# MGI-tech-bioinformatics/SuperPlus

Hardware: AMD Instinct MI355X
Metric: k-mers/s (DF createDict stage: trim + canonical k-mer count + solid filter + spectrum + adjacency) (higher is better)
Workload: dtype u64

## Files before the change

include/dfk.h:

```cpp
#ifndef DFK_H
#define DFK_H
#include <stddef.h>
#include <stdint.h>
#ifdef __cplusplus
extern "C" {
#endif

#define DFK_ABI_VERSION 3
#define DFK_MAX_MIN_BC 8u

enum {
    DFK_OK            = 0,
    DFK_E_ARG         = -1,
    DFK_E_NODEVICE    = -2,
    DFK_E_HIP         = -3,
    DFK_E_NOMEM       = -4,
    DFK_E_INPUT       = -5,
    DFK_E_STATE       = -6,
    DFK_E_NOGOOD      = -7
};

typedef struct dfk_config {
    uint32_t abi_version;
    uint32_t K;
    uint32_t min_qual;
    uint32_t min_freq;
    uint32_t min_bc;
    int32_t  device;
    int64_t  ign_bc_below;
    uint64_t hbm_budget_bytes;
    uint32_t minimizer_len;
    uint32_t flags;
    uint64_t inst_per_item;
    uint64_t reserved[4];
} dfk_config;

#define DFK_F_KEEP_PRE_ADJ   1u
#define DFK_F_KEEP_INPUTS    2u
#define DFK_F_MARK_BADS 4u

typedef struct dfk_entry32 {
    uint64_t w0, w1;
    uint32_t edge_id;
    uint32_t count_ctx;
    int32_t  bc;
    uint32_t pad;
} dfk_entry32;

typedef struct dfk_stats {
    uint64_t n_reads;
    uint64_t n_inst;
    uint64_t n_records;
    uint64_t n_buckets;
    uint64_t n_items;
    uint64_t n_overflow_items;
    uint64_t n_distinct;
    uint64_t n_solid;
    uint64_t adj_probes;
    float ms_upload, ms_trim, ms_part_count, ms_part_scatter, ms_count, ms_fallback, ms_adjacency, ms_total;
    uint64_t hbm_bytes_peak;
    uint64_t reserved[8];
} dfk_stats;

typedef struct dfk_ctx dfk_ctx;

int         dfk_create(const dfk_config* cfg, dfk_ctx** out);
void        dfk_destroy(dfk_ctx* ctx);
const char* dfk_last_error(void);
int         dfk_abi_version(void);

int dfk_qual_hist(dfk_ctx* ctx, uint32_t max_len, int64_t* hist);

int dfk_hint_file_range(dfk_ctx* ctx, const void* base, uint64_t bytes, int fd, uint64_t file_off);

int dfk_count(dfk_ctx* ctx,
              const uint8_t* packed_bases, const uint64_t* base_off, const uint32_t* read_len,
              const uint8_t* pq_bytes, const uint64_t* pq_off, const int32_t* bc,
              uint64_t n_reads);
int dfk_count_bci(dfk_ctx* ctx,
              const uint8_t* packed_bases, const uint64_t* base_off, const uint32_t* read_len,
              const uint8_t* pq_bytes, const uint64_t* pq_off, const int64_t* bci, uint64_t n_bci,
              uint64_t n_reads);

int dfk_count_device(dfk_ctx* ctx,
              const void* d_packed_bases, uint64_t packed_bytes, const void* d_base_off,
              const void* d_read_len, const void* d_pq_bytes, uint64_t pq_nbytes,
              const void* d_pq_off, const void* d_bc, uint64_t n_reads);

int dfk_good_lens(dfk_ctx* ctx, uint32_t* out, uint64_t cap);

int dfk_spectrum(dfk_ctx* ctx, const int64_t** hist, uint64_t* nbins);
int dfk_spectrum_json(dfk_ctx* ctx, char* out, uint64_t cap, uint64_t* need);

int dfk_solid_count(dfk_ctx* ctx, uint64_t* n);
int dfk_solid_fetch(dfk_ctx* ctx, dfk_entry32* out, uint64_t cap, int pre_adjacency);
int dfk_solid_fetch_unsorted(dfk_ctx* ctx, dfk_entry32* out, uint64_t cap, int pre_adjacency);

int dfk_solid_digest(dfk_ctx* ctx, int pre_adjacency, uint64_t* digest );

#define DFK_KVEC_PRE_ADJ 1
#define DFK_KVEC_SORTED  2
int dfk_write_kvec(dfk_ctx* ctx, const char* path, int flags);
int dfk_write_kvec_part(dfk_ctx* ctx, const char* path, int flags, uint64_t first_entry, uint64_t total_entries);

int dfk_get_stats(dfk_ctx* ctx, dfk_stats* out);

int dfk_graph_build(dfk_ctx* ctx);
int dfk_graph_stats(dfk_ctx* ctx, uint64_t* n_canonical_edges, uint64_t* n_vertices, uint64_t* n_edges);
int dfk_graph_write(dfk_ctx* ctx, const char* dir);

int dfk_paths_sink(dfk_ctx* ctx, const char* path);

int dfk_paths_build(dfk_ctx* ctx, const uint8_t* packed_bases, const uint64_t* base_off, const uint32_t* read_len,
              const uint8_t* pq_bytes, const uint64_t* pq_off, uint64_t n_reads);
int dfk_paths_build_device(dfk_ctx* ctx, const void* d_packed_bases, uint64_t packed_bytes, const void* d_base_off,
              const void* d_read_len, const void* d_pq_bytes, uint64_t pq_nbytes, const void* d_pq_off, uint64_t n_reads);
int dfk_paths_stats(dfk_ctx* ctx, uint64_t* n_reads, uint64_t* n_placed, uint64_t* n_path_edges);
int dfk_paths_write(dfk_ctx* ctx, const char* path);
int dfk_paths_fetch(dfk_ctx* ctx, int32_t* offsets, uint64_t* first_edge, int32_t* edges, uint64_t edges_cap);

int dfk_paths_index_write(dfk_ctx* ctx, const char* dir);
int dfk_dups_write(dfk_ctx* ctx, const char* path, uint64_t* n_marked_pairs);
int dfk_paths_index_dups_write(dfk_ctx* ctx, const char* dir, const char* dup_path, uint64_t* n_marked_pairs);

int dfk_bads_sums(dfk_ctx* ctx, uint16_t* out, uint64_t cap);
int dfk_bads_write(dfk_ctx* ctx, const char* path, uint64_t* n_marked_pairs, uint64_t* digest );
int dfk_bads_write_part(dfk_ctx* ctx, const char* path, uint64_t first_pair, uint64_t total_pairs, uint64_t* n_marked, uint64_t* digest );

#define DFK_HOPS_WORDS 16
#define DFK_HOPS_M1 0
#define DFK_HOPS_M2 1
#define DFK_HOPS_M3 2
#define DFK_HOPS_PAIRS 3
#define DFK_HOPS_SEARCHED 4
#define DFK_HOPS_EXTENDED 5
#define DFK_HOPS_HOST_EDGES 6
#define DFK_HOPS_MOST_ROUNDS 7
#define DFK_HOPS_US 8
#define DFK_HOPS_US_INDEX 9
#define DFK_HOPS_US_M12 10
#define DFK_HOPS_US_M3 11
#define DFK_HOPS_US_HOST 12
#define DFK_HOPS_LARGEST_X 13
#define DFK_HOPS_RANGES 14
int dfk_hops_build(dfk_ctx* ctx, const int32_t* bc , int one_good);
int dfk_hops_build_bci(dfk_ctx* ctx, const int64_t* bci, uint64_t n_bci, int one_good);
int dfk_hops_build_arrays(dfk_ctx* ctx, uint64_t n_edges, uint64_t n_vertices, const int32_t* kmers, const int32_t* inv, const int32_t* to_left, const int32_t* to_right,
                          uint64_t n_reads, const uint64_t* first , const int32_t* edges, const int32_t* bc, const uint16_t* sums, int one_good,
                          uint64_t reads_per_batch);
int dfk_hops_stats(dfk_ctx* ctx, uint64_t* out );
int dfk_hops_fetch(dfk_ctx* ctx, int32_t* pairs , uint64_t cap, uint64_t* n_pairs);
int dfk_hops_write(dfk_ctx* ctx, const char* path , uint64_t* n_pairs, uint64_t* digest );

#define DFK_SUBSET_WORDS 16
#define DFK_SUBSET_N_EOI 0
#define DFK_SUBSET_N_IDS 1
#define DFK_SUBSET_PATH_ENTRIES 2
#define DFK_SUBSET_INDEX_ENTRIES 3
#define DFK_SUBSET_RANGES 4
#define DFK_SUBSET_ONE_READ_ONLY 5
#define DFK_SUBSET_US 6
#define DFK_SUBSET_US_SWEEP 7
#define DFK_SUBSET_US_GATHER 8
#define DFK_SUBSET_US_INDEX 9
#define DFK_SUBSET_IDS_SUM 10
#define DFK_SUBSET_IDS_XOR 11
#define DFK_SUBSET_EOI_SUM 12
#define DFK_SUBSET_EOI_XOR 13
int dfk_subset_build(dfk_ctx* ctx, const int32_t* pairs , uint64_t n_pairs);
int dfk_subset_build_arrays(dfk_ctx* ctx, uint64_t n_edges, const int32_t* inv, uint64_t n_reads, const uint64_t* first , const int32_t* edges,
                            const int32_t* pairs, uint64_t n_pairs, uint64_t reads_per_batch, const char* dir );
int dfk_subset_stats(dfk_ctx* ctx, uint64_t* out );
int dfk_subset_fetch(dfk_ctx* ctx, uint64_t* ids, uint64_t ids_cap, uint64_t* n_ids, uint64_t* eoi, uint64_t eoi_cap, uint64_t* n_eoi);
int dfk_subset_write(dfk_ctx* ctx, const char* dir);

#define DFK_CHECK_WORDS 20
enum { DFK_CK_PATHS_SUM = 0, DFK_CK_PATHS_XOR = 1, DFK_CK_N_READS = 2, DFK_CK_N_PLACED = 3, DFK_CK_N_PATH_EDGES = 4,
       DFK_CK_INV_SUM = 5, DFK_CK_INV_XOR = 6, DFK_CK_INV_STARTS = 7, DFK_CK_INV_ENTRIES = 8,
       DFK_CK_COUNTSB_DIGEST = 9, DFK_CK_COUNTSB_SUM = 10, DFK_CK_SELF_INVERSE = 11,
       DFK_CK_DUP_DIGEST = 12, DFK_CK_DUP_MARKED = 13,
       DFK_CK_EDGE_KMERS = 14, DFK_CK_N_SOLID = 15, DFK_CK_INV_VIOLATIONS = 16, DFK_CK_N_EDGES = 17, DFK_CK_VALID = 18 };
#define DFK_CK_HAS_PATHS 1u
#define DFK_CK_HAS_INDEX 2u
#define DFK_CK_HAS_DUPS  4u
int dfk_paths_digest(dfk_ctx* ctx, uint64_t* out );
int dfk_paths_verify(dfk_ctx* ctx, const uint8_t* packed_bases, const uint64_t* base_off, const uint32_t* read_len, uint64_t n_reads,
              uint64_t* out );
int dfk_paths_verify_device(dfk_ctx* ctx, const void* d_packed_bases, uint64_t packed_bytes, const void* d_base_off, const void* d_read_len,
              uint64_t n_reads, uint64_t* out );

#define DFK_PBF_DROP 0xFFFFFFFFu
typedef struct dfk_pbf_input {
    const uint8_t*  seq[2];
    const uint8_t*  qual[2];
    const uint64_t* off[2];
    const uint32_t* rank;
    uint64_t m;
} dfk_pbf_input;
typedef struct dfk_pbf_output {
    uint64_t n_pairs;
    const uint32_t* order;
    const uint32_t* read_len;
    const uint8_t*  fastb_var;  const uint64_t* fastb_off;
    const uint8_t*  qualp_var;  const uint64_t* qualp_off;
    float ms_sort, ms_encode, ms_total;
} dfk_pbf_output;
typedef struct dfk_pbf dfk_pbf;
int  dfk_pbf_run(dfk_ctx* ctx, const dfk_pbf_input* in, dfk_pbf** out);
int  dfk_pbf_result(const dfk_pbf* r, dfk_pbf_output* o);
void dfk_pbf_free(dfk_pbf* r);

int dfk_shard_begin(dfk_ctx* ctx,
              const void* d_packed_bases, uint64_t packed_bytes, const void* d_base_off,
              const void* d_read_len, const void* d_pq_bytes, uint64_t pq_nbytes,
              const void* d_pq_off, const void* d_bc, uint64_t n_reads,
              int64_t global_read_offset ,
              uint64_t* n_inst_local);
int dfk_shard_begin_host(dfk_ctx* ctx,
              const uint8_t* packed_bases, const uint64_t* base_off , const uint32_t* read_len,
              const uint8_t* pq_bytes, const uint64_t* pq_off , const int32_t* bc, uint64_t n_reads,
              int64_t global_read_offset, uint64_t* n_inst_local);
int dfk_shard_plan(dfk_ctx* ctx, uint32_t world, uint64_t n_inst_global, uint32_t* log2_passes);
int dfk_shard_partition(dfk_ctx* ctx, uint32_t world, uint64_t n_inst_global, uint32_t log2_passes, uint32_t pass,
              const void** d_records, uint64_t* send_counts );
int dfk_shard_partition_begin(dfk_ctx* ctx, uint32_t world, uint64_t n_inst_global, uint32_t log2_passes, uint32_t pass, int defer,
              const void** d_records, uint64_t* send_counts );
int dfk_shard_partition_end(dfk_ctx* ctx, uint32_t pass);
int dfk_shard_recv_buffer(dfk_ctx* ctx, uint64_t n_records, void** d_buf);
int dfk_shard_count(dfk_ctx* ctx, const void* d_records, uint64_t n_records, uint32_t pass);
int dfk_shard_adj_queries(dfk_ctx* ctx, const void** d_keys,
              uint64_t* send_counts );
int dfk_shard_adj_answer(dfk_ctx* ctx, const void* d_keys, uint64_t n_keys, void* d_present );
int dfk_shard_adj_apply(dfk_ctx* ctx, const void* d_present, uint64_t n_keys);
int dfk_shard_dict_share(dfk_ctx* ctx, const void** d_entries, uint64_t* n_entries);
int dfk_shard_dict_adopt(dfk_ctx* ctx, uint64_t n_entries, void** d_room);
int dfk_shard_dict_whole(dfk_ctx* ctx);

int dfk_paths_var_bytes(dfk_ctx* ctx, uint64_t* bytes);
int dfk_paths_write_part(dfk_ctx* ctx, const char* path, uint64_t first_read, uint64_t total_reads, uint64_t var_before, uint64_t var_total);
int dfk_shard_pidx_pairs(dfk_ctx* ctx, uint32_t world, const void** d_pairs, uint64_t* send_counts , uint64_t* counts_host );
int dfk_shard_pidx_write(dfk_ctx* ctx, uint32_t world, uint32_t rank, const void* d_pairs_in, uint64_t n_in, const uint64_t* counts_global , const char* dir);
int dfk_shard_dup_keys(dfk_ctx* ctx, uint32_t world, const void** d_items, uint64_t* send_counts );
int dfk_shard_dup_answer(dfk_ctx* ctx, const void* d_items_in, uint64_t n_in, void* d_answers );
int dfk_shard_dup_write(dfk_ctx* ctx, const void* d_answers_back, uint64_t n, const char* path, uint64_t first_pair, uint64_t total_pairs, uint64_t* n_marked);

#ifdef __cplusplus
}
#endif
#endif
```

superplus_amd/csrc/dfk.hip:

```cpp
#include "../../include/dfk.h"
#include "dfk_kernels.h"
#include "dfk_arena.h"

#include <algorithm>
#include <chrono>
#include <cstdarg>
#include <cstdio>
#include <cstdlib>
#include <cstring>
#include <atomic>
#include <fcntl.h>
#include <functional>
#include <new>
#include <string>
#include <sys/mman.h>
#include <sys/stat.h>
#include <unistd.h>
#include <condition_variable>
#include <memory>
#include <mutex>
#include <numeric>
#include <thread>
#include <vector>

using namespace dfk;

namespace {

thread_local std::string g_err;

int fail(int code, const char* fmt, ...)
{
    char buf[512];
    va_list ap; va_start(ap, fmt); vsnprintf(buf, sizeof buf, fmt, ap); va_end(ap);
    g_err = buf;
    return code;
}

#define HIP_TRY(expr) do { hipError_t e_ = (expr); if (e_ != hipSuccess) \
    return fail(DFK_E_HIP, "%s failed: %s (%s:%d)", #expr, hipGetErrorString(e_), __FILE__, __LINE__); } while (0)

template <class F> int guarded(F&& f)
{
    try { return f(); }
    catch (const std::bad_alloc&) { return fail(DFK_E_NOMEM, "out of host memory"); }
    catch (const std::exception& e) { return fail(DFK_E_HIP, "internal error: %s", e.what()); }
    catch (...) { return fail(DFK_E_HIP, "internal error"); }
}

void* dev_get(uint64_t bytes, const char** why)
{
    void* p = nullptr;
    const hipError_t e = hipMalloc(&p, bytes);
    if (e == hipSuccess) return p;
    (void)hipGetLastError();
    *why = hipGetErrorString(e);
    return nullptr;
}
void dev_give(void* p) { (void)hipFree(p); }

bool g_trace = getenv("DFK_TRACE") != nullptr;
#define TRACE(...) do { if (g_trace) { fprintf(stderr, "[dfk] " __VA_ARGS__); fputc('\n', stderr); fflush(stderr); } } while (0)
inline uint32_t env_u32(const char* name, uint32_t dflt) { const char* e = getenv(name); return e ? (uint32_t)atoi(e) : dflt; }
inline double wall_now() { return std::chrono::duration<double>(std::chrono::steady_clock::now().time_since_epoch()).count(); }

template <int K> struct CountCfg;
#ifndef DFK_LOG2S
#define DFK_LOG2S 11
#endif
#ifndef DFK_NWAVES
#define DFK_NWAVES 8
#endif
template <> struct CountCfg<40> { static constexpr int LOG2S = DFK_LOG2S, NWAVES = DFK_NWAVES; };
template <> struct CountCfg<48> { static constexpr int LOG2S = DFK_LOG2S, NWAVES = DFK_NWAVES; };
template <> struct CountCfg<60> { static constexpr int LOG2S = DFK_LOG2S, NWAVES = DFK_NWAVES; };

struct Inputs {
    const uint8_t* packed; uint64_t packed_bytes;
    const uint64_t* base_off; const uint32_t* read_len;
    const uint8_t* pq; uint64_t pq_bytes; const uint64_t* pq_off;
    const int32_t* bc; uint64_t n_reads;
};

}

struct dfk_ctx {
    dfk_config cfg{};
    int device = 0;
    hipStream_t stream = nullptr;
    hipStream_t stream2 = nullptr;
    hipDeviceProp_t prop{};
    dfk::Arena arena{dev_get, dev_give};
    uint64_t &budget = arena.budget, &held = arena.held, &peak = arena.peak, &alloc_seq = arena.alloc_seq, &first_chunk_hint = arena.first_chunk_hint;
    int alloc(DevBuf& b, size_t bytes, const char* what, Place where = Place::High) { return arena.alloc(b, bytes, what, where) ? fail(DFK_E_NOMEM, "%s", arena.err.c_str()) : 0; }
    void release(DevBuf& b) { arena.release(b); }
    void shrink(DevBuf& b, size_t keep) { arena.shrink(b, keep); }
    void release_since(uint64_t mark, const DevBuf* keep = nullptr) { arena.release_since(mark, keep); }
    uint64_t largest_allocatable() const { return arena.largest_allocatable(); }
    void drop_empty_chunks() { arena.drop_empty_chunks(); }
    void drop_pool() { arena.drop_pool(); }
    bool have = false;
    uint64_t n_reads = 0;
    struct FileRange { const char* base; uint64_t bytes; int fd; uint64_t off; };
    std::vector<FileRange> file_ranges;
    DevBuf good_len;
    struct Part { DevBuf buf, pre; uint64_t n = 0; uint64_t blist = 0, n_blist = 0; bool listed = false; };
    bool want_blist = false;
    int pending_blist = -1;
    std::function<int()> after_count_launch;
    std::vector<Part> parts;
    uint64_t n_solid = 0, n_boundary = 0;
    unsigned seg_attempt = 0;
    double distinct_per_inst = 0.0;
    double plan_derate = 0.95;
    std::vector<int64_t> hist;
    std::vector<dfk_entry32> sorted, sorted_pre;
    bool sorted_ok = false, sorted_pre_ok = false;
    dfk_stats st{};
    bool shard_open = false, shard_use_bc = false;
    const void* sh_in[7] = {};
    uint64_t sh_packed_bytes = 0, sh_pq_bytes = 0, sh_n_reads = 0, sh_n_inst_local = 0;
    int64_t sh_read_id0 = 0;
    DevBuf shard_send[2];
    uint32_t shard_send_pass[2] = {~0u, ~0u};
    DevBuf shard_recv[2];
    unsigned shard_recv_seq = 0;
    uint64_t budget_taken = 0;
    void* sh_staged[6] = {};
    uint64_t sh_b0 = 0, sh_b1 = 0, sh_q0 = 0, sh_q1 = 0, sh_staged_reads = 0;
    DevBuf adj_keys, adj_src; uint64_t adj_n = 0;
    DevBuf set; uint64_t set_mask = 0;
    double t_upload_done = 0;
    uint32_t shard_world = 1, shard_log2_nb = 0;
    void* shard_state = nullptr;
    void (*shard_state_free)(void*) = nullptr;
    void* lane_pool = nullptr; void (*lane_pool_free)(void*) = nullptr;
    std::mutex lane_mu;
    void* graph_state = nullptr;
    void (*graph_state_free)(void*) = nullptr;
    unsigned int* d_resident = nullptr;
    unsigned int resident_target = 0;
    unsigned int last_wg_idle = 0;
    void* kept[6] = {};
    uint64_t kept_packed_bytes = 0, kept_pq_bytes = 0, kept_n_reads = 0, kept_budget = 0;

    void release_all()
    {
        after_count_launch = nullptr;
        if (stream2) (void)hipStreamSynchronize(stream2);
        DevBuf* live[] = {&good_len, &shard_send[0], &shard_send[1], &shard_recv[0], &shard_recv[1], &adj_keys, &adj_src, &set};
        for (DevBuf* d : live) release(*d);
        for (Part& pt : parts) { release(pt.buf); release(pt.pre); }
        parts.clear();
        arena.reset();
        good_len = shard_send[0] = shard_send[1] = shard_recv[0] = shard_recv[1] = adj_keys = adj_src = set = DevBuf{};
        shard_send_pass[0] = shard_send_pass[1] = ~0u;
        have = false; sorted_ok = sorted_pre_ok = false; sorted.clear(); sorted_pre.clear(); hist.clear();
        n_solid = 0; adj_n = 0; shard_open = false;
        if (shard_state) { shard_state_free(shard_state); shard_state = nullptr; }
        for (void*& p : sh_staged) if (p) { (void)hipFree(p); p = nullptr; }
        budget += budget_taken; budget_taken = 0;
        if (graph_state) { graph_state_free(graph_state); graph_state = nullptr; }
    }
    void drop_kept()
    {
        for (void*& p : kept) if (p) { (void)hipFree(p); p = nullptr; }
        budget += kept_budget; kept_budget = 0; kept_n_reads = 0;
    }
    void adopt_kept()
    {
        const uint64_t bytes[6] = {kept_packed_bytes + 64, (kept_n_reads + 1) * 8 + 64, kept_n_reads * 4 + 64, kept_pq_bytes + 64, (kept_n_reads + 1) * 8 + 64, 0};
        for (int i = 0; i < 6; ++i) {
            if (!kept[i]) continue;
            const uint64_t b = bytes[i] & ~(uint64_t)0xFFF;
            if (i < 5 && b >= (64ull << 20) && ((uintptr_t)kept[i] & 0xFFF) == 0) arena.adopt(kept[i], b);
            else (void)hipFree(kept[i]);
            kept[i] = nullptr;
        }
        budget += kept_budget; kept_budget = 0; kept_n_reads = 0;
    }
};

namespace {

struct Timer {
    hipEvent_t a{}, b{}; hipStream_t s;
    explicit Timer(hipStream_t st) : s(st) { (void)hipEventCreate(&a); (void)hipEventCreate(&b); }
    ~Timer() { (void)hipEventDestroy(a); (void)hipEventDestroy(b); }
    void start() { (void)hipEventRecord(a, s); }
    float stop() { (void)hipEventRecord(b, s); (void)hipEventSynchronize(b); float ms = 0; (void)hipEventElapsedTime(&ms, a, b); return ms; }
};

template <int K>
int stage_trim(dfk_ctx* c, const Inputs& in, uint64_t* n_inst)
{
    DevBuf ctr; int rc = c->alloc(ctr, 32, "trim counters"); if (rc) return rc;
    HIP_TRY(hipMemsetAsync(ctr.p, 0, 32, c->stream));
    rc = c->alloc(c->good_len, sizeof(uint32_t) * in.n_reads, "goodLens", Place::Low); if (rc) return rc;
    if (in.n_reads) {
        unsigned grid = (unsigned)std::min<uint64_t>((in.n_reads + 255) / 256, 8192);
        hipLaunchKernelGGL(HIP_KERNEL_NAME(k_trim<K>), dim3(grid), dim3(256), 0, c->stream,
                           in.pq, in.pq_off, in.pq_bytes, in.base_off, in.packed_bytes, in.read_len, in.n_reads, c->cfg.min_qual, (uint32_t*)c->good_len.p,
                           (unsigned long long*)ctr.p, (unsigned int*)((char*)ctr.p + 8),
                           (unsigned long long*)((char*)ctr.p + 16));
        HIP_TRY(hipGetLastError());
    }
    uint64_t h[3] = {0, 0, 0};
    HIP_TRY(hipMemcpyAsync(h, ctr.p, 24, hipMemcpyDeviceToHost, c->stream));
    HIP_TRY(hipStreamSynchronize(c->stream));
    c->release(ctr);
    if ((uint32_t)h[1]) return fail(DFK_E_INPUT, "malformed input: an offset table is not monotone or runs past its array, a PQVec stream is broken, or its length differs from read_len");
    if (h[2] == 0) return fail(DFK_E_NOGOOD, "Looks like your input data have almost no good bases.");
    *n_inst = h[0];
    return 0;
}

int device_scan(dfk_ctx* c, const uint64_t* in, uint64_t* out, uint64_t n)
{
    constexpr uint64_t PER = (uint64_t)SCAN_THREADS * SCAN_ITEMS;
    if (n == 0) return 0;
    const uint64_t nblk = (n + PER - 1) / PER;
    if (nblk == 1) {
        hipLaunchKernelGGL(k_scan_blocks, dim3(1), dim3(SCAN_THREADS), 0, c->stream, in, out, n, (uint64_t*)nullptr);
        HIP_TRY(hipGetLastError());
        return 0;
    }
    DevBuf sums; int rc = c->alloc(sums, nblk * 8, "scan block sums"); if (rc) return rc;
    hipLaunchKernelGGL(k_scan_blocks, dim3((unsigned)nblk), dim3(SCAN_THREADS), 0, c->stream, in, out, n, (uint64_t*)sums.p);
    HIP_TRY(hipGetLastError());
    rc = device_scan(c, (const uint64_t*)sums.p, (uint64_t*)sums.p, nblk); if (rc) return rc;
    hipLaunchKernelGGL(k_scan_add, dim3((unsigned)nblk), dim3(SCAN_THREADS), 0, c->stream, out, n, (const uint64_t*)sums.p);
    HIP_TRY(hipGetLastError());
    HIP_TRY(hipStreamSynchronize(c->stream));
    c->release(sums);
    return 0;
}

struct BucketTable {
    uint32_t log2_nb = 0;
    DevBuf acc;
    DevBuf summ;
    DevBuf classes;
    DevBuf ovf_list; uint64_t n_ovf = 0;
    DevBuf class_hist;
    std::vector<uint64_t> h_class;
    uint64_t n_records = 0, n_inst = 0;
};
struct Partition {
    DevBuf records, base, ipre, items;
    uint64_t n_records = 0, n_inst = 0, n_items = 0;
    uint64_t nb = 0;
};

template <int K>
PartParams part_params(const dfk_ctx* c, uint32_t log2_nb, uint32_t log2_world, int64_t read_id0, uint32_t sub_lo, uint32_t sub_n)
{
    const uint32_t M = c->cfg.minimizer_len;
    return PartParams{M, (uint32_t)K - M + 1, log2_nb, log2_world, read_id0, sub_lo, sub_n,
                      sweep_class_mask(sub_lo, sub_n, log2_nb - log2_world)};
}

int table_totals(dfk_ctx* c, const DevBuf& acc, uint64_t nb, uint64_t* n_records, uint64_t* n_inst)
{
    DevBuf tot; int rc = c->alloc(tot, 16, "bucket totals"); if (rc) return rc;
    HIP_TRY(hipMemsetAsync(tot.p, 0, 16, c->stream));
    hipLaunchKernelGGL(k_sum_acc, dim3(1024), dim3(256), 0, c->stream, (const unsigned long long*)acc.p, nb, (unsigned long long*)tot.p);
    HIP_TRY(hipGetLastError());
    uint64_t h[2];
    HIP_TRY(hipMemcpyAsync(h, tot.p, 16, hipMemcpyDeviceToHost, c->stream));
    HIP_TRY(hipStreamSynchronize(c->stream));
    c->release(tot);
    *n_records = h[0]; *n_inst = h[1];
    return 0;
}

struct ScanJob {
    PartParams pp; ScanPlan plan;
    DevBuf ovf_tmp, d_n;
    DevBuf keys, keys2, fill, sub;
    uint64_t n_pieces = 0; bool count_due = false;
    hipEvent_t ev_scan = nullptr, ev_count = nullptr, ev_part[2] = {nullptr, nullptr};
    std::vector<std::pair<hipEvent_t, hipEvent_t>> ev;
    ~ScanJob()
    {
        for (auto& e : ev) { (void)hipEventDestroy(e.first); (void)hipEventDestroy(e.second); }
        for (hipEvent_t e : {ev_scan, ev_count, ev_part[0], ev_part[1]}) if (e) (void)hipEventDestroy(e);
    }
};

template <int K> bool scan_takes_ranges(const dfk_ctx* c) { return c->cfg.minimizer_len == 16; }

ScanSwitches scan_switches()
{
    static const uint32_t scan_blocks = getenv("DFK_SCAN_BLOCKS") ? (uint32_t)atoi(getenv("DFK_SCAN_BLOCKS")) : 0;
    ScanSwitches sw;
    sw.scan_blocks = scan_blocks;
    if (const char* e = getenv("DFK_SCAN_KEY_PIECE")) { sw.key_piece_set = true; sw.key_piece = strtoull(e, nullptr, 10); }
    if (const char* e = getenv("DFK_SCAN_KEY_TAIL")) sw.key_tail = strtoull(e, nullptr, 10);
    sw.no_overlap = getenv("DFK_NO_OVERLAP") != nullptr;
    return sw;
}

template <int K>
int scan_begin(dfk_ctx* c, const Inputs& in, uint32_t log2_world, int64_t read_id0, BucketTable* T, bool by_class, ScanJob* J)
{
    J->pp = part_params<K>(c, T->log2_nb, log2_world, read_id0, 0, 1u << (T->log2_nb - log2_world));
    J->plan = plan_scan(ScanInputs{K, J->pp.W, T->log2_nb, log2_world, in.n_reads, in.packed_bytes, by_class, scan_takes_ranges<K>(c), c->stream2 != nullptr, scan_switches()});
    ScanPlan& P = J->plan;
    int rc = 0;
    if (by_class) { rc = c->alloc(T->class_hist, P.n_bins * 8, "class counters", Place::Low); if (rc) return rc; HIP_TRY(hipMemsetAsync(T->class_hist.p, 0, P.n_bins * 8, c->stream)); }
    else { rc = c->alloc(T->acc, P.nb * 8, "bucket counters", Place::Low); if (rc) return rc; }
// ... 232 lines not shown
                           (unsigned long long*)J->cur.p, J->P.n_records, (uint4*)J->P.records.p);
    HIP_TRY(hipGetLastError());
    HIP_TRY(hipEventRecord(J->e1, J->st));
    return 0;
}

template <int K>
int scatter_begin(dfk_ctx* c, const Inputs& in, const BucketTable& T, uint32_t log2_world, int64_t read_id0,
                  uint32_t sub_lo, uint32_t sub_n, ScatterJob* J, bool launch_now = true)
{
    Partition* P = &J->P;
    J->st = c->stream; J->lo = sub_lo; J->n = sub_n;
    const PartParams pp = part_params<K>(c, T.log2_nb, log2_world, read_id0, sub_lo, sub_n);
    const uint64_t budget = item_budget<K>(c);
    int rc = pass_tables(c, T.acc, T.log2_nb - log2_world, 1u << log2_world, sub_lo, sub_n, budget, P); if (rc) return rc;
    const uint64_t nb = P->nb;
    rc = c->alloc(J->cur, nb * 8, "bucket cursors"); if (rc) return rc;
    rc = c->alloc(P->records, P->n_records * 32, "super-k-mer records"); if (rc) return rc;
    rc = c->alloc(J->d_bad, 16, "scatter check"); if (rc) return rc;
    HIP_TRY(hipMemcpyAsync(J->cur.p, P->base.p, nb * 8, hipMemcpyDeviceToDevice, c->stream));
    HIP_TRY(hipMemsetAsync(J->d_bad.p, 0, 16, c->stream));
    if (!J->e0) { HIP_TRY(hipEventCreate(&J->e0)); HIP_TRY(hipEventCreate(&J->e1)); }
    (void)pp;
    if (launch_now) return scatter_launch<K>(c, in, T, log2_world, read_id0, J);
    return 0;
}

template <int K>
int scatter_end(dfk_ctx* c, const Inputs& in, const BucketTable& T, uint32_t log2_world, int64_t read_id0, ScatterJob* J)
{
    HIP_TRY(hipEventSynchronize(J->e1));
    float ms = 0; (void)hipEventElapsedTime(&ms, J->e0, J->e1);
    c->st.ms_part_scatter += ms;
    {
        Partition* P = &J->P;
        const PartParams pp = part_params<K>(c, T.log2_nb, log2_world, read_id0, J->lo, J->n);
        const size_t lds_b = sizeof(uint32_t) * pp.W * PART_THREADS + sizeof(uint32_t) * 2 * PART_QCAP * PART_THREADS;
        Timer t(c->stream);
        t.start();
        if (T.n_ovf)
            hipLaunchKernelGGL(HIP_KERNEL_NAME(k_partition<K, true>), dim3((unsigned)((T.n_ovf + PART_THREADS - 1) / PART_THREADS)),
                               dim3(PART_THREADS), lds_b, c->stream,
                               in.packed, in.packed_bytes, in.base_off, (const uint32_t*)c->good_len.p, in.bc,
                               (int64_t)c->cfg.ign_bc_below, in.n_reads, pp, (unsigned long long*)nullptr, (unsigned long long*)nullptr,
                               (unsigned long long*)J->cur.p, P->n_records, (uint4*)P->records.p, (uint4*)nullptr,
                               (const uint32_t*)T.ovf_list.p, T.n_ovf, (const uint64_t*)nullptr, (uint32_t*)nullptr);
        HIP_TRY(hipGetLastError());
        hipLaunchKernelGGL(k_check_cursors, dim3((unsigned)std::min<uint64_t>((P->nb + 255) / 256, 4096)), dim3(256), 0, c->stream, (const unsigned long long*)J->cur.p,
                           (const uint64_t*)P->base.p, P->nb, (unsigned int*)J->d_bad.p);
        HIP_TRY(hipGetLastError());
        c->st.ms_part_scatter += t.stop();
    }
    unsigned int bad = 0;
    HIP_TRY(hipMemcpy(&bad, J->d_bad.p, 4, hipMemcpyDeviceToHost));
    c->release(J->d_bad); c->release(J->cur);
    if (bad) return fail(DFK_E_HIP, "scatter: %u buckets did not receive the records counted for them (run summaries and bucket counters disagree)", bad);
    TRACE("scatter of buckets [%u, %u) done (%llu records, %llu items)", J->lo, J->lo + J->n,
          (unsigned long long)J->P.n_records, (unsigned long long)J->P.n_items);
    return 0;
}

constexpr int E_SPLIT_NO_ROOM = -101;
constexpr int E_SEGMENT_FULL = -100;

struct CountRun {
    CountGlobals* g = nullptr; uint4* seg = nullptr; unsigned long long* hist = nullptr;
    CountParams cp{}; unsigned grid = 0;
    DevBuf big; uint64_t big_cap = 0;
    DevBuf d_hist, d_g;
    DevBuf d_snap;
    DevBuf d_part;
    DevBuf d_wg;
    uint64_t solid_seen = 0, inst_seen = 0;
    uint64_t boundary_seen = 0;
    uint64_t splits_seen = 0;
};

int count_run_begin(dfk_ctx* c, CountRun* R)
{
    int rc = c->alloc(R->d_hist, (uint64_t)HIST_GLOBAL_BINS * 8, "spectrum bins", Place::Low); if (rc) return rc;
    rc = c->alloc(R->d_g, sizeof(CountGlobals), "count globals", Place::Low); if (rc) return rc;
    HIP_TRY(hipMemsetAsync(R->d_hist.p, 0, (uint64_t)HIST_GLOBAL_BINS * 8, c->stream));
    HIP_TRY(hipMemsetAsync(R->d_g.p, 0, sizeof(CountGlobals), c->stream));
    R->g = (CountGlobals*)R->d_g.p; R->hist = (unsigned long long*)R->d_hist.p;
    return c->alloc(R->d_snap, (uint64_t)HIST_GLOBAL_BINS * 8 + 256, "spectrum snapshot", Place::Low);
}

int count_snapshot(dfk_ctx* c, CountRun* R, bool restore)
{
    char* snap = (char*)R->d_snap.p;
    const uint64_t hb = (uint64_t)HIST_GLOBAL_BINS * 8;
    if (!restore) {
        HIP_TRY(hipMemcpyAsync(snap, R->d_hist.p, hb, hipMemcpyDeviceToDevice, c->stream));
        HIP_TRY(hipMemcpyAsync(snap + hb, R->d_g.p, sizeof(CountGlobals), hipMemcpyDeviceToDevice, c->stream));
    } else {
        HIP_TRY(hipMemcpyAsync(R->d_hist.p, snap, hb, hipMemcpyDeviceToDevice, c->stream));
        HIP_TRY(hipMemcpyAsync(R->d_g.p, snap + hb, sizeof(CountGlobals), hipMemcpyDeviceToDevice, c->stream));
    }
    return 0;
}

int count_run_end(dfk_ctx* c, CountRun* R)
{
    CountGlobals hg{};
    HIP_TRY(hipMemcpy(&hg, R->d_g.p, sizeof hg, hipMemcpyDeviceToHost));
    c->st.n_distinct = hg.n_distinct; c->n_boundary = hg.n_boundary;
#ifdef DFK_PHASE_TIMES
    {
        unsigned long long ph[16] = {};
        (void)hipMemcpyFromSymbol(ph, HIP_SYMBOL(g_phase), sizeof ph);
        unsigned long long tot = 0; for (int i = 0; i < 12; ++i) tot += ph[i];
        static const char* nm[12] = {"item loop tail (thread 0 publishes)", "barrier: item start", "chunks (stage + insert)", "barrier: chunks done", "finish pass 1 (solidity)", "barrier", "finish pass 2 (adjacency look-ups)", "barrier", "finish pass 3 (emit)", "barrier", "clear + reduce", "drain"};
        fprintf(stderr, "[dfk] k_count wave cycles by phase (%.3e memtime ticks in all):\n", (double)tot);
        for (int i = 0; i < 12; ++i) fprintf(stderr, "[dfk]   %5.1f %%  %s\n", 100.0 * (double)ph[i] / (double)std::max(1ull, tot), nm[i]);
        unsigned long long z[16] = {};
        (void)hipMemcpyToSymbol(HIP_SYMBOL(g_phase), z, sizeof z);
    }
#endif
    DevBuf d_max; int rc = c->alloc(d_max, 16, "max bin"); if (rc) return rc;
    HIP_TRY(hipMemsetAsync(d_max.p, 0, 16, c->stream));
    hipLaunchKernelGGL(k_hist_max, dim3(1024), dim3(256), 0, c->stream, (const unsigned long long*)R->d_hist.p, HIST_GLOBAL_BINS,
                       (unsigned int*)d_max.p);
    uint32_t nb = 0;
    HIP_TRY(hipMemcpyAsync(&nb, d_max.p, 4, hipMemcpyDeviceToHost, c->stream));
    HIP_TRY(hipStreamSynchronize(c->stream));
    c->hist.assign(nb, 0);
    if (nb) HIP_TRY(hipMemcpy(c->hist.data(), R->d_hist.p, 8ull * nb, hipMemcpyDeviceToHost));
    TRACE("spectrum read back: %u bins, %llu solid", nb, (unsigned long long)c->n_solid);
    c->release(d_max); c->release(R->d_hist); c->release(R->d_g); c->release(R->d_snap);
    return 0;
}

template <int K> unsigned count_grid(const dfk_ctx* c, int nbc = 1)
{
    constexpr int LOG2S = CountCfg<K>::LOG2S, NW = CountCfg<K>::NWAVES;
    const size_t lds = count_lds_bytes<K, LOG2S, NW, 1>() + (size_t)(nbc > 1 ? nbc - 1 : 0) * sizeof(uint32_t) * (1u << LOG2S);
    const unsigned per_cu = (unsigned)std::max<size_t>(1, (size_t)(160 * 1024) / lds);
    return (unsigned)c->prop.multiProcessorCount * per_cu;
}

int launch_boundary_list(dfk_ctx* c)
{
    if (c->pending_blist < 0) return 0;
    const dfk_ctx::Part& part = c->parts[(size_t)c->pending_blist];
    c->pending_blist = -1;
    unsigned long long* ctl = (unsigned long long*)((char*)part.buf.p + part.blist);
    HIP_TRY(hipMemsetAsync(ctl, 0, 16, c->stream2));
    hipLaunchKernelGGL(k_boundary_list, dim3((unsigned)std::min<uint64_t>((part.n + 2047) / 2048, 4096)), dim3(256), 0, c->stream2,
                       (const uint4*)part.buf.p, part.n, (uint32_t*)(ctl + 2), part.n_blist, ctl);
    HIP_TRY(hipGetLastError());
    return 0;
}

template <int K, int NBC>
int launch_count(dfk_ctx* c, const Partition& P, const ItemRange* d_items, uint64_t n_items, const CountRun& R,
                 std::vector<ItemRange>* overflowed, float* kernel_ms, const uint32_t* d_sub = nullptr, bool single_kmer_records = false)
{
    constexpr int LOG2S = CountCfg<K>::LOG2S, NW = CountCfg<K>::NWAVES;
    if (n_items == 0) return 0;
    if (n_items >= (1ull << 32)) return fail(DFK_E_ARG, "too many work items in one pass");
    DevBuf d_ovf;
    int rc = c->alloc(d_ovf, n_items * sizeof(ItemRange), "overflow list"); if (rc) return rc;
    HIP_TRY(hipMemsetAsync(&R.g->next_item, 0, 8, c->stream));
    HIP_TRY(hipMemsetAsync(&R.g->n_wg_idle, 0, 4, c->stream));
    CountParams cp = R.cp; cp.n_items = (uint32_t)n_items; cp.single = single_kmer_records ? 1u : 0u;
    const size_t lds = count_lds_bytes<K, LOG2S, NW, NBC>();
    auto kern = d_sub ? k_count<K, LOG2S, NW, NBC, true> : k_count<K, LOG2S, NW, NBC, false>;
    HIP_TRY(hipFuncSetAttribute(reinterpret_cast<const void*>(kern), hipFuncAttributeMaxDynamicSharedMemorySize, (int)lds));
    TRACE("k_count: %llu items, grid %u, lds %zu, seg_cap %llu", (unsigned long long)n_items, R.grid, lds, (unsigned long long)R.cp.seg_cap);
    Timer tk(c->stream);
    tk.start();
    hipLaunchKernelGGL(kern, dim3(R.grid), dim3(NW * 64), lds, c->stream,
                       (const uint4*)P.records.p, d_items, (const uint64_t*)P.base.p, cp, R.g, R.seg, (WgOut*)R.d_wg.p, R.hist,
                       (ItemRange*)d_ovf.p, d_sub, c->d_resident);
    HIP_TRY(hipGetLastError());
    c->resident_target += R.grid;
    if (c->after_count_launch || c->pending_blist >= 0) {
        hipLaunchKernelGGL(k_gate, dim3(1), dim3(64), 0, c->stream2, (const unsigned int*)c->d_resident, c->resident_target, 200000ull, c->d_resident + 1);
    }
    if (c->after_count_launch) { std::function<int()> f; f.swap(c->after_count_launch); rc = f(); if (rc) return rc; }
    rc = launch_boundary_list(c); if (rc) return rc;
    *kernel_ms += tk.stop();
    CountGlobals g{};
    HIP_TRY(hipMemcpyAsync(&g, R.g, sizeof g, hipMemcpyDeviceToHost, c->stream));
    HIP_TRY(hipStreamSynchronize(c->stream));
    c->last_wg_idle = g.n_wg_idle;
    if (g.n_overflow) {
        const size_t at = overflowed->size();
        overflowed->resize(at + g.n_overflow);
        HIP_TRY(hipMemcpy(overflowed->data() + at, d_ovf.p, sizeof(ItemRange) * g.n_overflow, hipMemcpyDeviceToHost));
    }
    c->release(d_ovf);
    return 0;
}

int gather_diffs(dfk_ctx* c, const std::vector<ItemRange>& ranges, std::initializer_list<std::pair<const DevBuf*, std::vector<uint64_t>*>> tables)
{
    const uint32_t n = (uint32_t)ranges.size();
    DevBuf d_idx, d_val;
    int rc = c->alloc(d_idx, 8ull * n, "gather index"); if (!rc) rc = c->alloc(d_val, 16ull * n, "gather values"); if (rc) return rc;
    HIP_TRY(hipMemcpyAsync(d_idx.p, ranges.data(), 8ull * n, hipMemcpyHostToDevice, c->stream));
    std::vector<uint64_t> val(2 * n);
    for (const auto& t : tables) {
        hipLaunchKernelGGL(k_gather_u64, dim3((2 * n + 255) / 256), dim3(256), 0, c->stream, (const uint64_t*)t.first->p, (const uint32_t*)d_idx.p, 2 * n, (uint64_t*)d_val.p);
        HIP_TRY(hipGetLastError());
        HIP_TRY(hipMemcpyAsync(val.data(), d_val.p, 16ull * n, hipMemcpyDeviceToHost, c->stream));
        HIP_TRY(hipStreamSynchronize(c->stream));
        for (uint32_t i = 0; i < n; ++i) t.second->push_back(val[2 * i + 1] - val[2 * i]);
    }
    c->release(d_idx); c->release(d_val);
    return 0;
}

template <int K, int NBC>
int launch_count_big(dfk_ctx* c, const Partition& P, const std::vector<ItemRange>& singles, CountRun& R)
{
    constexpr int KW = KTraits<K>::KW, NW = 8;
    const uint32_t n = (uint32_t)singles.size();
    std::vector<uint64_t> inst, rec;
    int rc = gather_diffs(c, singles, {{&P.ipre, &inst}, {&P.base, &rec}}); if (rc) return rc;
    const uint64_t tot_inst = std::accumulate(inst.begin(), inst.end(), (uint64_t)0);
    const std::vector<uint64_t> chunk_pre = chunk_prefixes(rec);
    double per_inst = table_distinct_per_inst(c->distinct_per_inst);
    DevBuf d_items, d_fail, d_pre;
    {
        const uint64_t more = tot_inst / std::max<uint32_t>(1, c->cfg.min_freq) + 1;
        if (!R.big.p) { R.big_cap = more; rc = c->alloc(R.big, R.big_cap * 32, "fallback solid entries"); if (rc) return rc; }
        else {
            CountGlobals g0{};
            HIP_TRY(hipMemcpy(&g0, R.d_g.p, sizeof g0, hipMemcpyDeviceToHost));
            DevBuf grown;
            rc = c->alloc(grown, (g0.big_cursor + more) * 32, "fallback solid entries"); if (rc) return rc;
            if (g0.big_cursor) HIP_TRY(hipMemcpy(grown.p, R.big.p, g0.big_cursor * 32, hipMemcpyDeviceToDevice));
            c->release(R.big);
            R.big = grown; R.big_cap = g0.big_cursor + more;
        }
    }
    rc = c->alloc(d_items, (uint64_t)n * sizeof(BigItem), "fallback items"); if (rc) return rc;
    rc = c->alloc(d_pre, 16ull * (n + 1), "fallback prefixes"); if (rc) return rc;
    rc = c->alloc(d_fail, 16, "fallback flag"); if (rc) return rc;
    uint64_t* d_chunk_pre = (uint64_t*)d_pre.p; uint64_t* d_slot_pre = d_chunk_pre + (n + 1);
    HIP_TRY(hipMemcpyAsync(d_chunk_pre, chunk_pre.data(), 8ull * (n + 1), hipMemcpyHostToDevice, c->stream));
    CountParams cpb = R.cp; cpb.seg_cap = R.big_cap;
    const unsigned cus = (unsigned)c->prop.multiProcessorCount;
    for (;;) {
        const BigTables T = size_big_tables(singles, inst, per_inst, big_slot_words(KW, NBC));
        DevBuf pool;
        rc = c->alloc(pool, T.words * 4 + 8, "HBM fallback tables"); if (rc) return rc;
        hipLaunchKernelGGL(k_fill_u64, dim3(4096), dim3(256), 0, c->stream, (uint64_t*)pool.p, T.words / 2 + (T.words & 1), 0ull);
        HIP_TRY(hipGetLastError());
        HIP_TRY(hipMemsetAsync(d_fail.p, 0, 16, c->stream));
        HIP_TRY(hipMemcpyAsync(d_items.p, T.items.data(), T.items.size() * sizeof(BigItem), hipMemcpyHostToDevice, c->stream));
        HIP_TRY(hipMemcpyAsync(d_slot_pre, T.slot_pre.data(), 8ull * (n + 1), hipMemcpyHostToDevice, c->stream));
        const unsigned g_ins = (unsigned)std::max<uint64_t>(1, std::min<uint64_t>((chunk_pre[n] + NW * BIG_TICKET_CHUNKS - 1) / (NW * BIG_TICKET_CHUNKS), 4ull * cus));
        const unsigned g_slot = (unsigned)std::max<uint64_t>(1, std::min<uint64_t>((T.slot_pre[n] + 255) / 256, 16ull * cus));
        hipLaunchKernelGGL(HIP_KERNEL_NAME(k_big_insert<K, NW, NBC>), dim3(g_ins), dim3(NW * 64), 0, c->stream,
                           (const uint4*)P.records.p, (const BigItem*)d_items.p, (const uint64_t*)P.base.p, (const uint64_t*)d_chunk_pre, n,
                           (uint32_t*)pool.p, (unsigned long long*)d_fail.p + 1, (uint32_t*)d_fail.p);
        HIP_TRY(hipGetLastError());
        uint32_t failed = 0;
        HIP_TRY(hipMemcpyAsync(&failed, d_fail.p, 4, hipMemcpyDeviceToHost, c->stream));
        HIP_TRY(hipStreamSynchronize(c->stream));
        if (failed) {
            unsigned int info[4] = {};
            (void)hipMemcpyFromSymbol(info, HIP_SYMBOL(g_big_fail), sizeof info);
            const unsigned int zero[4] = {};
            (void)hipMemcpyToSymbol(HIP_SYMBOL(g_big_fail), zero, sizeof zero);
            c->release(pool);
            if (T.certain) {
                c->release(d_items); c->release(d_fail); c->release(d_pre);
                return fail(DFK_E_HIP, "an insert into an HBM fallback table gave up after %u probe steps and %u waits on a locked slot "
                                       "(table of 2^%u slots at load <= 0.5; %u tables, %llu instances in this pass's fallback)", info[1], info[2], info[3], n,
                            (unsigned long long)tot_inst);
            }
            per_inst = table_retry_per_inst(per_inst);
            TRACE("fallback: an HBM table filled up (2^%u slots): rebuilding the tables for %.2f distinct k-mers per instance", info[3], per_inst);
            continue;
        }
        hipLaunchKernelGGL(HIP_KERNEL_NAME(k_big_flags<K, NBC>), dim3(g_slot), dim3(256), 0, c->stream, (const BigItem*)d_items.p,
                           (const uint64_t*)d_slot_pre, n, (uint32_t*)pool.p, cpb, R.g);
        if (cpb.do_adj)
            hipLaunchKernelGGL(HIP_KERNEL_NAME(k_big_resolve<K>), dim3(g_slot), dim3(256), 0, c->stream, (const BigItem*)d_items.p,
                               (const uint64_t*)d_slot_pre, n, (uint32_t*)pool.p);
        hipLaunchKernelGGL(HIP_KERNEL_NAME(k_big_emit<K>), dim3(g_slot), dim3(256), 0, c->stream, (const BigItem*)d_items.p,
                           (const uint64_t*)d_slot_pre, n, (uint32_t*)pool.p, cpb, R.g, (uint4*)R.big.p, R.hist);
        HIP_TRY(hipGetLastError());
        HIP_TRY(hipStreamSynchronize(c->stream));
        c->release(pool);
        break;
    }
    c->release(d_items); c->release(d_fail); c->release(d_pre);
    return 0;
}

template <int K, int NBC>
int count_halved(dfk_ctx* c, const Partition& P, const CountRun& R, bool single_kmer_records, std::vector<ItemRange>& overflowed, std::vector<ItemRange>* singles)
{
    while (!overflowed.empty()) {
        const std::vector<ItemRange> next = halve_items(overflowed, singles);
        overflowed.clear();
        if (next.empty()) break;
        if (!single_kmer_records) TRACE("retrying %zu split items", next.size());
        DevBuf d_next; float ignored = 0;
        int rc = c->alloc(d_next, next.size() * sizeof(ItemRange), "split items"); if (rc) return rc;
        HIP_TRY(hipMemcpyAsync(d_next.p, next.data(), next.size() * sizeof(ItemRange), hipMemcpyHostToDevice, c->stream));
        rc = launch_count<K, NBC>(c, P, (const ItemRange*)d_next.p, next.size(), R, &overflowed, &ignored, nullptr, single_kmer_records);
        c->release(d_next); if (rc) return rc;
    }
    return 0;
}

template <int K, int NBC>
int count_split(dfk_ctx* c, const Partition& P, const std::vector<ItemRange>& hot, const std::vector<uint64_t>& inst, const SplitCandidates& sp, size_t i0, size_t i1, CountRun& R)
{
    constexpr int NW = 8;
    const uint32_t n = (uint32_t)(i1 - i0);
    std::vector<HotItem> items(n); std::vector<ItemRange> buckets(n);
    uint64_t ns = 0, tot = 0;
    for (uint32_t i = 0; i < n; ++i) { buckets[i] = hot[sp.at[i0 + i]]; items[i] = HotItem{buckets[i].b0, buckets[i].b1, (uint32_t)ns, sp.log2p[i0 + i]}; ns += 1ull << sp.log2p[i0 + i]; tot += inst[sp.at[i0 + i]]; }
    if (ns >= (1ull << 24)) { fail(DFK_E_NOMEM, "more than 2^24 sub-buckets in one pass"); return E_SPLIT_NO_ROOM; }
    const uint64_t mark = c->alloc_seq;
    bool started = false;
    auto undo = [&](int rc) {
        (void)hipStreamSynchronize(c->stream);
        if (!started) { c->release_since(mark); return rc == DFK_E_NOMEM ? E_SPLIT_NO_ROOM : rc; }
        return rc;
    };
    DevBuf d_items, d_pre, d_tk, acc; std::vector<uint64_t> rec;
    int rc = gather_diffs(c, buckets, {{&P.base, &rec}}); if (rc) return undo(rc);
    const std::vector<uint64_t> chunk_pre = chunk_prefixes(rec);
    rc = c->alloc(d_items, (uint64_t)n * sizeof(HotItem), "hot buckets"); if (rc) return undo(rc);
    rc = c->alloc(d_pre, 8ull * (n + 1), "hot bucket chunks"); if (rc) return undo(rc);
    rc = c->alloc(d_tk, 16, "hot bucket ticket"); if (rc) return undo(rc);
    rc = c->alloc(acc, 8ull * ns, "sub-bucket counters"); if (rc) return undo(rc);
// ... 44 lines not shown
}

int barcode_words(const dfk_ctx* c, bool have_bc)
{ return !have_bc ? 0 : (int)std::max<uint32_t>(1, std::min<uint32_t>(c->cfg.min_bc, DFK_MAX_MIN_BC) - (c->cfg.min_bc > 1 ? 1 : 0)); }

template <int K> constexpr uint64_t out_chunk() { return 2ull << CountCfg<K>::LOG2S; }

template <int K>
int count_prepare(dfk_ctx* c, const Partition& P, CountRun& R, int nbc)
{
    const unsigned attempt = c->seg_attempt;
    R.grid = (unsigned)std::max<uint64_t>(1, std::min<uint64_t>(P.n_items, count_grid<K>(c, nbc)));
    uint64_t res = part_entries(P.n_inst, c->cfg.min_freq, R.inst_seen, R.solid_seen);
    res = (res << attempt) + (uint64_t)R.grid * out_chunk<K>();
    const uint64_t room = c->budget > c->held ? (c->budget - c->held) : 0;
    if (res * 32 > room) res = room / 32;
    int rc = c->alloc(R.d_wg, sizeof(WgOut) * R.grid, "workgroup output state"); if (rc) return rc;
    std::vector<WgOut> init(R.grid, WgOut{~0ull, (unsigned int)out_chunk<K>(), 0u});
    HIP_TRY(hipMemcpy(R.d_wg.p, init.data(), sizeof(WgOut) * R.grid, hipMemcpyHostToDevice));
    HIP_TRY(hipMemsetAsync(&R.g->big_cursor, 0, 8, c->stream));
    HIP_TRY(hipMemsetAsync(&R.g->part_cursor, 0, 8, c->stream));
    R.cp = CountParams{c->cfg.min_freq, c->cfg.min_bc, 0, 0, res, c->cfg.min_freq > 1 ? 1u : 0u,
                       (c->cfg.flags & DFK_F_KEEP_PRE_ADJ) ? 1u : 0u};
    R.big_cap = 0;
    rc = c->alloc(R.d_part, std::max<uint64_t>(1, res) * 32, "solid k-mer entries", Place::Low); if (rc) return rc;
    R.seg = (uint4*)R.d_part.p;
    return 0;
}

template <int K>
int finish_part(dfk_ctx* c, const Partition& P, CountRun& R)
{
    CountGlobals hg{};
    std::vector<WgOut> wg(R.grid);
    HIP_TRY(hipMemcpy(&hg, R.d_g.p, sizeof hg, hipMemcpyDeviceToHost));
    HIP_TRY(hipMemcpy(wg.data(), R.d_wg.p, sizeof(WgOut) * R.grid, hipMemcpyDeviceToHost));
    c->release(R.d_wg);
    const uint64_t claimed = hg.part_cursor;
    const HoleMoves mv = plan_hole_moves(wg, out_chunk<K>(), claimed);
    const std::vector<uint64_t>&src = mv.src, &dst = mv.dst; const uint64_t n_lds = mv.n_lds;
    if (hg.solid_overflow || claimed > R.cp.seg_cap || hg.big_cursor > R.big_cap || n_lds + hg.big_cursor > R.cp.seg_cap) {
        c->release(R.big); c->release(R.d_part);
        fail(DFK_E_NOMEM, "the room reserved for a pass's solid k-mers (%llu entries) is full", (unsigned long long)R.cp.seg_cap);
        return E_SEGMENT_FULL;
    }
    if (src.size() != dst.size())
        return fail(DFK_E_HIP, "output compaction: %zu holes, %zu entries to move", dst.size(), src.size());
    dfk_ctx::Part part;
    part.n = n_lds + hg.big_cursor;
    part.buf = R.d_part; R.d_part = DevBuf{};
    if (!src.empty()) {
        DevBuf d_mv; int rc = c->alloc(d_mv, 16ull * src.size(), "hole moves"); if (rc) return rc;
        HIP_TRY(hipMemcpyAsync(d_mv.p, src.data(), 8ull * src.size(), hipMemcpyHostToDevice, c->stream));
        HIP_TRY(hipMemcpyAsync((uint64_t*)d_mv.p + src.size(), dst.data(), 8ull * src.size(), hipMemcpyHostToDevice, c->stream));
        hipLaunchKernelGGL(k_fill_holes, dim3((unsigned)((src.size() + 255) / 256)), dim3(256), 0, c->stream, (uint4*)part.buf.p,
                           (const uint64_t*)d_mv.p, (const uint64_t*)d_mv.p + src.size(), (uint64_t)src.size());
        HIP_TRY(hipGetLastError());
        HIP_TRY(hipStreamSynchronize(c->stream));
        c->release(d_mv);
    }
    if (hg.big_cursor)
        HIP_TRY(hipMemcpyAsync((char*)part.buf.p + 32 * n_lds, R.big.p, 32 * hg.big_cursor, hipMemcpyDeviceToDevice, c->stream));
    HIP_TRY(hipStreamSynchronize(c->stream));
    c->release(R.big);
    const uint64_t nb_part = hg.n_boundary - R.boundary_seen;
    R.boundary_seen = hg.n_boundary;
    c->st.n_overflow_items += hg.n_split - R.splits_seen;
    R.splits_seen = hg.n_split;
    uint64_t keep = part.n * 32;
    part.listed = c->want_blist && nb_part == 0;
    if (c->want_blist && nb_part && keep + 16 + 4 * nb_part <= part.buf.bytes && part.n < (1ull << 32)) {
        part.blist = keep; part.n_blist = nb_part; part.listed = true;
        keep += 16 + 4 * nb_part;
    }
    c->shrink(part.buf, keep);
    c->parts.push_back(part);
    if (part.blist) c->pending_blist = (int)c->parts.size() - 1;
    c->n_solid += part.n; c->st.n_solid = c->n_solid;
    R.solid_seen += part.n; R.inst_seen += P.n_inst;
    if (R.inst_seen) c->distinct_per_inst = (double)hg.n_distinct / (double)R.inst_seen;
    return 0;
}

template <int K, int NBC>
int count_run(dfk_ctx* c, const Partition& P, CountRun& R)
{
    Timer t(c->stream);
    std::vector<ItemRange> overflowed, singles;
    c->st.n_items += P.n_items;
    const float ms_before = c->st.ms_count;
    int rc = launch_count<K, NBC>(c, P, (const ItemRange*)P.items.p, P.n_items, R, &overflowed, &c->st.ms_count); if (rc) return rc;
    if (g_trace) {
        unsigned int gate[2] = {0, 0};
        (void)hipMemcpy(gate, c->d_resident, 8, hipMemcpyDeviceToHost);
        TRACE("k_count: %llu instances in %.1f ms (%.1f G instances/s), reservation %.2f GB, %u of %u workgroups idle, %u gate timeouts so far",
              (unsigned long long)P.n_inst, c->st.ms_count - ms_before, 1e-6 * (double)P.n_inst / (double)(c->st.ms_count - ms_before), R.d_part.bytes / 1e9,
              c->last_wg_idle, R.grid, gate[1]);
    }
    t.start();
    c->st.n_overflow_items += overflowed.size();
    rc = count_halved<K, NBC>(c, P, R, false, overflowed, &singles); if (rc) return rc;
    TRACE("fallback: %zu single-bucket items", singles.size());
    if (!singles.empty()) {
        const FallbackSwitches sw{env_u32("DFK_SPLIT_FROM_LOG2", 2), env_u32("DFK_MAX_SUBPASS_LOG2", 8)};
        const double dpi = route_distinct_per_inst(c->distinct_per_inst);
        std::vector<uint64_t> inst; std::vector<uint8_t> taken(singles.size(), 0);
        rc = gather_diffs(c, singles, {{&P.ipre, &inst}}); if (rc) return rc;
        const SplitCandidates sp = split_candidates(inst, dpi, sw);
        for (size_t i0 = 0; i0 < sp.at.size();) {
            const uint64_t can = c->largest_allocatable();
            const size_t i1 = split_group_end(inst, sp.at, i0, split_group_cap(can));
            if (i1 == i0) { TRACE("fallback: no room to split a hot bucket of %llu instances (%.2f GB free in one piece): sub-passes instead", (unsigned long long)inst[sp.at[i0]], can / 1e9); break; }
            rc = count_split<K, NBC>(c, P, singles, inst, sp, i0, i1, R);
            if (rc == E_SPLIT_NO_ROOM) { TRACE("fallback: no room to split %zu hot buckets (%s): sub-passes instead", i1 - i0, g_err.c_str()); break; }
            if (rc) return rc;
            for (; i0 < i1; ++i0) taken[sp.at[i0]] = 1;
        }
        SubpassPlan sub = plan_subpasses(singles, inst, taken, dpi, CountCfg<K>::LOG2S, sw);
        TRACE("fallback: %zu sub-passes over %zu buckets in LDS tables, %zu buckets in HBM tables", sub.items.size(), singles.size() - sub.huge.size(), sub.huge.size());
        while (!sub.items.empty()) {
            DevBuf d_it, d_sub;
            rc = c->alloc(d_it, sub.items.size() * sizeof(ItemRange), "sub-pass items"); if (!rc) rc = c->alloc(d_sub, sub.words.size() * 4, "sub-pass words"); if (rc) return rc;
            HIP_TRY(hipMemcpyAsync(d_it.p, sub.items.data(), sub.items.size() * sizeof(ItemRange), hipMemcpyHostToDevice, c->stream));
            HIP_TRY(hipMemcpyAsync(d_sub.p, sub.words.data(), sub.words.size() * 4, hipMemcpyHostToDevice, c->stream));
            std::vector<ItemRange> again; ItemRange bad{}; float ignored = 0;
            rc = launch_count<K, NBC>(c, P, (const ItemRange*)d_it.p, sub.items.size(), R, &again, &ignored, (const uint32_t*)d_sub.p);
            c->release(d_it); c->release(d_sub);
            if (rc) return rc;
            if (!refine_subpasses(again, &sub, &bad))
                return fail(DFK_E_HIP, "a sub-pass (%u of 2^%u) of bucket %u overflowed its table (it holds at most %llu instances)", bad.b1 & 0xFFu, (bad.b1 & 0x7FFFFFFFu) >> 8, bad.b0, 1ull << (CountCfg<K>::LOG2S - 1));
            if (!sub.items.empty()) TRACE("fallback: %zu sub-passes cut in two", again.size());
        }
        if (!sub.huge.empty()) { rc = launch_count_big<K, NBC>(c, P, sub.huge, R); if (rc) return rc; }
    }
    c->st.ms_fallback += t.stop();
    return finish_part<K>(c, P, R);
}


template <int K>
int count_run_nbc(dfk_ctx* c, const Partition& P, CountRun& R, int nbc)
{
    static int (*const run[8])(dfk_ctx*, const Partition&, CountRun&) = {count_run<K, 0>, count_run<K, 1>, count_run<K, 2>, count_run<K, 3>, count_run<K, 4>, count_run<K, 5>, count_run<K, 6>, count_run<K, 7>};
    return run[std::min(std::max(nbc, 0), 7)](c, P, R);
}

template <int K>
int stage_count(dfk_ctx* c, const Partition& P, CountRun& R, bool have_bc)
{
    const int rc = count_prepare<K>(c, P, R, barcode_words(c, have_bc));
    return rc ? rc : count_run_nbc<K>(c, P, R, barcode_words(c, have_bc));
}

int build_set(dfk_ctx* c)
{
    uint64_t slots = 1ull << std::max<uint32_t>(10, ceil_log2(2 * c->n_boundary + 2));
    int rc = c->alloc(c->set, slots * sizeof(SetSlot), "boundary k-mer set"); if (rc) return rc;
    c->set_mask = slots - 1;
    hipLaunchKernelGGL(k_fill_u64, dim3(2048), dim3(256), 0, c->stream, (uint64_t*)c->set.p, slots * 2, ~0ull);
    for (const dfk_ctx::Part& pt : c->parts)
        if (pt.n)
            hipLaunchKernelGGL(k_set_insert, dim3((unsigned)((pt.n + 255) / 256)), dim3(256), 0, c->stream,
                               (const uint4*)pt.buf.p, pt.n, (SetSlot*)c->set.p, c->set_mask);
    HIP_TRY(hipGetLastError());
    return 0;
}

int make_pre_view(dfk_ctx* c)
{
    if (!(c->cfg.flags & DFK_F_KEEP_PRE_ADJ)) return 0;
    for (dfk_ctx::Part& pt : c->parts) {
        int rc = c->alloc(pt.pre, pt.n * 32, "pre-adjacency copy"); if (rc) return rc;
        if (!pt.n) continue;
        if (c->cfg.min_freq > 1)
            hipLaunchKernelGGL(k_make_pre, dim3((unsigned)((pt.n + 255) / 256)), dim3(256), 0, c->stream,
                               (uint4*)pt.buf.p, (uint4*)pt.pre.p, pt.n);
        else
            HIP_TRY(hipMemcpyAsync(pt.pre.p, pt.buf.p, pt.n * 32, hipMemcpyDeviceToDevice, c->stream));
    }
    HIP_TRY(hipGetLastError());
    return 0;
}

template <int K>
int stage_adjacency(dfk_ctx* c)
{
    Timer t(c->stream);
    t.start();
    int rc = make_pre_view(c); if (rc) return rc;
    if (c->cfg.min_freq > 1 && c->n_solid && c->n_boundary) {
        bool listed = c->want_blist;
        for (const dfk_ctx::Part& pt : c->parts) listed = listed && pt.listed;
        if (c->want_blist) {
            rc = launch_boundary_list(c); if (rc) return rc;
            HIP_TRY(hipStreamSynchronize(c->stream2));
        }
        if (listed) {
            uint64_t total = 0;
            for (const dfk_ctx::Part& pt : c->parts) {
                if (!pt.blist) continue;
                unsigned long long ctl[2] = {0, 0};
                HIP_TRY(hipMemcpy(ctl, (const char*)pt.buf.p + pt.blist, 16, hipMemcpyDeviceToHost));
                if (ctl[1] || ctl[0] != pt.n_blist)
                    return fail(DFK_E_HIP, "boundary list: %llu entries listed, the count kernels reported %llu", ctl[0], (unsigned long long)pt.n_blist);
                total += pt.n_blist;
            }
            if (total != c->n_boundary) listed = false;
        }
        if (!listed) { rc = build_set(c); if (rc) return rc; }
        else {
            uint64_t slots = 1ull << std::max<uint32_t>(10, ceil_log2(2 * c->n_boundary + 2));
            rc = c->alloc(c->set, slots * sizeof(SetSlot), "boundary k-mer set"); if (rc) return rc;
            c->set_mask = slots - 1;
            hipLaunchKernelGGL(k_fill_u64, dim3(2048), dim3(256), 0, c->stream, (uint64_t*)c->set.p, slots * 2, ~0ull);
            for (const dfk_ctx::Part& pt : c->parts)
                if (pt.n_blist)
                    hipLaunchKernelGGL(k_set_insert_list, dim3((unsigned)((pt.n_blist + 255) / 256)), dim3(256), 0, c->stream, (const uint4*)pt.buf.p,
                                       (const uint32_t*)((const char*)pt.buf.p + pt.blist + 16), pt.n_blist, (SetSlot*)c->set.p, c->set_mask);
            HIP_TRY(hipGetLastError());
        }
        DevBuf d_n; rc = c->alloc(d_n, 16, "probe counter"); if (rc) return rc;
        HIP_TRY(hipMemsetAsync(d_n.p, 0, 16, c->stream));
        for (const dfk_ctx::Part& pt : c->parts) {
            if (!pt.n) continue;
            if (listed) {
                if (pt.n_blist)
                    hipLaunchKernelGGL(HIP_KERNEL_NAME(k_adjacency_list<K>), dim3((unsigned)std::min<uint64_t>((pt.n_blist + 255) / 256, 16384)), dim3(256), 0,
                                       c->stream, (uint4*)pt.buf.p, (const uint32_t*)((const char*)pt.buf.p + pt.blist + 16), pt.n_blist,
                                       (const SetSlot*)c->set.p, c->set_mask, (unsigned long long*)d_n.p);
            } else
                hipLaunchKernelGGL(HIP_KERNEL_NAME(k_adjacency<K>), dim3((unsigned)std::min<uint64_t>((pt.n + 255) / 256, 8192)), dim3(256), 0,
                                   c->stream, (uint4*)pt.buf.p, pt.n, (const SetSlot*)c->set.p, c->set_mask, (unsigned long long*)d_n.p);
        }
        HIP_TRY(hipGetLastError());
        uint64_t np = 0;
        HIP_TRY(hipMemcpyAsync(&np, d_n.p, 8, hipMemcpyDeviceToHost, c->stream));
        HIP_TRY(hipStreamSynchronize(c->stream));
        c->st.adj_probes = np;
        c->release(d_n); c->release(c->set);
    }
    c->st.ms_adjacency = t.stop();
    TRACE("adjacency done");
    return 0;
}

uint32_t pick_log2_nb(uint64_t n_inst, uint32_t log2_world)
{
    static const uint64_t per = getenv("DFK_INST_PER_BUCKET") ? (uint64_t)atoll(getenv("DFK_INST_PER_BUCKET")) : 850;
    return dfk::pick_log2_nb(n_inst, log2_world, per);
}

PlanInputs plan_inputs(const dfk_ctx* c, const BucketTable& T, const CountRun& R, uint32_t sub_nb, uint32_t lo, bool overlap)
{
    static const double first_div = getenv("DFK_PLAN_FIRST") ? atof(getenv("DFK_PLAN_FIRST")) : 10.0;
    static const double growth = getenv("DFK_PLAN_GROWTH") ? atof(getenv("DFK_PLAN_GROWTH")) : 1.1;
    return PlanInputs{c->budget > c->held ? (double)(c->budget - c->held) : 0.0, sub_nb, lo, T.n_inst, T.n_records, R.inst_seen, R.solid_seen,
                      c->cfg.min_freq, c->seg_attempt, c->plan_derate, overlap, first_div, growth, g_trace};
}

struct StreamSwap {
    dfk_ctx* c; hipStream_t keep;
    StreamSwap(dfk_ctx* ctx, hipStream_t s) : c(ctx), keep(ctx->stream) { c->stream = s; }
    ~StreamSwap() { c->stream = keep; }
};

struct Prescan { BucketTable T; uint64_t n_inst = 0; float ms_trim = 0; };

template <int K>
int run_typed(dfk_ctx* c, const Inputs& in, Prescan* pre = nullptr)
{
    Timer total(c->stream);
    total.start();
    Timer t(c->stream);
    uint64_t n_inst = 0;
    int rc = 0;
    BucketTable T;
    if (pre) { n_inst = pre->n_inst; c->st.ms_trim = pre->ms_trim; T = std::move(pre->T); }
    else {
        t.start();
        TRACE("trim: %llu reads", (unsigned long long)in.n_reads);
        rc = stage_trim<K>(c, in, &n_inst); if (rc) return rc;
        c->st.ms_trim = t.stop();
        TRACE("trim done: %llu instances", (unsigned long long)n_inst);
    }
    c->st.n_reads = in.n_reads; c->st.n_inst = n_inst; c->n_reads = in.n_reads;
    if (!pre) {
        T.log2_nb = pick_log2_nb(n_inst, 0);
        rc = partition_count<K>(c, in, n_inst, 0, 0, &T); if (rc) return rc;
    }
    CountRun R;
    rc = count_run_begin(c, &R); if (rc) return rc;
    c->want_blist = true; c->pending_blist = -1;
    const uint32_t sub_nb = 1u << T.log2_nb;
    const uint32_t forced = (uint32_t)c->cfg.reserved[0];
    const uint32_t per_forced = forced ? std::max<uint32_t>(1, (sub_nb + forced - 1) / forced) : 0;
    const bool overlap = getenv("DFK_NO_OVERLAP") == nullptr;
    uint32_t n_passes = 0, retries = 0;
    c->seg_attempt = 0; c->distinct_per_inst = 0.0;
    struct Job { ScatterJob sj; Arena::PassBlock blk; uint64_t mark = 0; bool valid = false; };
    Job cur, nxt;
    auto drop_events = [&](Job& j) { if (j.sj.e0) { (void)hipEventDestroy(j.sj.e0); (void)hipEventDestroy(j.sj.e1); j.sj.e0 = j.sj.e1 = nullptr; } };
    static const double defer_below = getenv("DFK_DEFER_SWEEP_BELOW") ? atof(getenv("DFK_DEFER_SWEEP_BELOW")) : 1.0;
    auto start = [&](Job& j, uint32_t lo, uint32_t n, bool may_defer = false) -> int {
        j.sj = ScatterJob{}; j.mark = c->alloc_seq; j.valid = false;
        const bool defer = may_defer && (double)n < defer_below * (double)sub_nb;
        TRACE("pass range [%u, %u) of %u (%.1f %%), %.2f GB held of %.2f", lo, lo + n, sub_nb, 100.0 * n / sub_nb, c->held / 1e9, c->budget / 1e9);
        j.blk = Arena::PassBlock{};
        int r = c->alloc(j.blk.block, pass_block_bytes(n, sub_nb, T.n_records), "pass block");
        if (!r) { Arena::Current in_blk(c->arena, j.blk); StreamSwap sw(c, c->stream2); r = scatter_begin<K>(c, in, T, 0, 0, lo, n, &j.sj, !defer); }
        if (r) { (void)hipStreamSynchronize(c->stream2); c->release_since(j.mark); drop_events(j); return r; }
        if (defer) { ScatterJob* sj = &j.sj; c->after_count_launch = [c, &in, &T, sj]() { return scatter_launch<K>(c, in, T, 0, 0, sj); }; TRACE("  (its sweep starts behind k_count)"); }
        j.valid = true;
        return 0;
    };
    auto start_alone = [&](Job& j, uint32_t lo) -> int {
        for (;;) {
            const uint32_t n = forced ? std::min(per_forced, sub_nb - lo) : plan_range(plan_inputs(c, T, R, sub_nb, lo, overlap), c->arena.free_blocks(), nullptr);
            if (!forced && n < sub_nb - lo && (uint64_t)n * 1024 < sub_nb)
                return fail(DFK_E_NOMEM, "HBM budget too small: %.2f GB free of %.2f GB allows passes of %u of %u buckets",
                            (c->budget - c->held) / 1e9, c->budget / 1e9, n, sub_nb);
            const int r = start(j, lo, n);
            if (r != DFK_E_NOMEM || forced || n <= 16 || ++retries > 12) return r;
            c->plan_derate *= 0.7;
            TRACE("out of HBM (%s): planning smaller passes", g_err.c_str());
        }
    };
    rc = start_alone(cur, 0); if (rc) return rc;
    while (cur.valid) {
        const uint32_t lo = cur.sj.lo, n = cur.sj.n, nlo = lo + n;
        rc = scatter_end<K>(c, in, T, 0, 0, &cur.sj); if (rc) return rc;
        const dfk_stats st0 = c->st;
        rc = count_snapshot(c, &R, false); if (rc) return rc;
        { Arena::Current in_blk(c->arena, cur.blk); rc = count_prepare<K>(c, cur.sj.P, R, barcode_words(c, in.bc != nullptr)); }
        nxt.valid = false;
        if (!rc && overlap && nlo < sub_nb) {
            const Partition& P = cur.sj.P;
            (void)P;
            const RunningPass rp{cur.blk.block.bytes, cur.sj.P.n_inst, n, c->arena.offset_of(cur.blk.block)};
            const uint32_t n2 = forced ? std::min(per_forced, sub_nb - nlo) : plan_range(plan_inputs(c, T, R, sub_nb, nlo, overlap), c->arena.free_blocks(), &rp);
            if (n2) {
                const int r2 = start(nxt, nlo, n2, true);
                if (r2 && r2 != DFK_E_NOMEM) return r2;
            }
        }
        if (!rc) rc = count_run_nbc<K>(c, cur.sj.P, R, barcode_words(c, in.bc != nullptr));
        if (c->after_count_launch) {
            std::function<int()> f; f.swap(c->after_count_launch);
            if (!rc) { const int r3 = f(); if (r3) return r3; } else nxt.valid = false;
        }
        if (rc == DFK_E_NOMEM || rc == E_SEGMENT_FULL) {
            HIP_TRY(hipStreamSynchronize(c->stream)); HIP_TRY(hipStreamSynchronize(c->stream2));
            c->release_since(cur.mark);
            R.d_wg = R.big = R.d_part = DevBuf{};
            drop_events(cur); drop_events(nxt); nxt.valid = false;
            int rc2 = count_snapshot(c, &R, true); if (rc2) return rc2;
            const float ms_scatter = c->st.ms_part_scatter, ms_count = c->st.ms_count, ms_fb = c->st.ms_fallback;
            c->st = st0;
            c->st.ms_part_scatter = ms_scatter; c->st.ms_count = ms_count; c->st.ms_fallback = ms_fb;
            if (++retries > 12) return DFK_E_NOMEM;
            if (rc == E_SEGMENT_FULL) { ++c->seg_attempt; TRACE("the room reserved for the pass's solid k-mers was too small: redoing the pass with twice as much"); }
            else if (forced || n <= 16) return rc;
            else { c->plan_derate *= 0.7; TRACE("out of HBM (%s): redoing the pass smaller", g_err.c_str()); }
            rc = start_alone(cur, lo); if (rc) return rc;
            continue;
        }
        if (rc) return rc;
        release_pass(c, &cur.sj.P);
        c->release(cur.blk.block);
        drop_events(cur);
        ++n_passes;
        c->seg_attempt = 0;
        if (nxt.valid) { cur = nxt; nxt = Job{}; }
        else { cur = Job{}; if (nlo < sub_nb) { rc = start_alone(cur, nlo); if (rc) return rc; } }
    }
    c->release(T.acc); c->release(T.summ); c->release(T.classes); c->release(T.ovf_list); c->release(T.class_hist);
    c->st.reserved[0] = n_passes;
    rc = count_run_end(c, &R); if (rc) return rc;
    rc = stage_adjacency<K>(c); if (rc) return rc;
    c->st.ms_total = total.stop() + (pre ? c->st.ms_trim + c->st.ms_part_count : 0.0f);
    c->st.hbm_bytes_peak = c->peak;
    c->have = true;
    return 0;
}

int run(dfk_ctx* c, const Inputs& in)
{
    int rc;
    switch (c->cfg.K) {
    case 40: rc = run_typed<40>(c, in); break;
    case 48: rc = run_typed<48>(c, in); break;
    case 60: rc = run_typed<60>(c, in); break;
    default: return fail(DFK_E_ARG, "K must be 40, 48 or 60");
    }
    return rc == E_SEGMENT_FULL ? DFK_E_NOMEM : rc;
}

int upload(dfk_ctx* c, void* d, const void* h, uint64_t bytes);

template <int K>
int run_under_upload(dfk_ctx* c, const Inputs& in, const uint8_t* h_packed)
{
    const uint64_t n = in.n_reads, pb = in.packed_bytes;
    const uint64_t seg_env = getenv("DFK_UPLOAD_SEGMENT") ? (uint64_t)atoll(getenv("DFK_UPLOAD_SEGMENT")) : 0;
    const uint64_t seg = upload_segment_bytes(pb, seg_env);
    const uint64_t stride = offset_sampling(n).stride, n_samp = offset_sampling(n).n_samp;
    std::vector<uint64_t> samp(n_samp);
    {
        DevBuf d; int rc = c->alloc(d, n_samp * 8, "offset samples", Place::Low); if (rc) return rc;
        hipLaunchKernelGGL(k_sample_u64, dim3((unsigned)((n_samp + 255) / 256)), dim3(256), 0, c->stream, in.base_off, stride, n, n_samp, (uint64_t*)d.p);
        HIP_TRY(hipGetLastError());
        HIP_TRY(hipMemcpyAsync(samp.data(), d.p, n_samp * 8, hipMemcpyDeviceToHost, c->stream));
        HIP_TRY(hipStreamSynchronize(c->stream));
        c->release(d);
    }
    Prescan pre;
    int trim_rc = 0; std::string trim_err;
    Timer tt(c->stream);
    std::thread trim([&] {
        (void)hipSetDevice(c->device);
        TRACE("trim: %llu reads (the bases are still arriving)", (unsigned long long)n);
        tt.start();
        trim_rc = stage_trim<K>(c, in, &pre.n_inst);
        if (trim_rc) trim_err = g_err; else pre.ms_trim = tt.stop();
    });
    struct JoinTrim { std::thread& t; ~JoinTrim() { if (t.joinable()) t.join(); } } join_trim{trim};
    uint64_t sent = std::min(seg, pb);
    int rc = upload(c, (void*)in.packed, h_packed, sent);
    if (sent >= pb) c->t_upload_done = wall_now();
    trim.join();
    if (trim_rc) return fail(trim_rc, "%s", trim_err.c_str());
    if (rc) return rc;
    TRACE("trim done: %llu instances", (unsigned long long)pre.n_inst);
    pre.T.log2_nb = pick_log2_nb(pre.n_inst, 0);
    ScanJob J;
    rc = scan_begin<K>(c, in, 0, 0, &pre.T, false, &J); if (rc) return rc;
    uint64_t scanned = 0;
    for (;;) {
        const uint64_t r1 = sent >= pb ? n : reads_within(samp, stride, n, sent);
        rc = scan_range<K>(c, in, &pre.T, &J, scanned, r1); if (rc) return rc;
        scanned = std::max(scanned, r1);
        if (sent >= pb) break;
        const uint64_t m = std::min(seg, pb - sent);
        rc = upload(c, (char*)in.packed + sent, h_packed + sent, m); if (rc) return rc;
        sent += m;
        if (sent >= pb) c->t_upload_done = wall_now();
    }
    rc = scan_end<K>(c, in, pre.n_inst, &pre.T, &J); if (rc) return rc;
    return run_typed<K>(c, in, &pre);
}

int run_from_host_bases(dfk_ctx* c, const Inputs& in, const uint8_t* h_packed)
{
    int rc;
    switch (c->cfg.K) {
    case 40: rc = run_under_upload<40>(c, in, h_packed); break;
    case 48: rc = run_under_upload<48>(c, in, h_packed); break;
    case 60: rc = run_under_upload<60>(c, in, h_packed); break;
    default: return fail(DFK_E_ARG, "K must be 40, 48 or 60");
    }
    return rc == E_SEGMENT_FULL ? DFK_E_NOMEM : rc;
}
bool scan_under_upload_applies(const dfk_ctx* c, uint64_t packed_bytes)
{
    const bool off = getenv("DFK_NO_SCAN_UNDER_UPLOAD") != nullptr;
    const uint64_t min_bytes = getenv("DFK_SCAN_UNDER_UPLOAD_MIN") ? (uint64_t)atoll(getenv("DFK_SCAN_UNDER_UPLOAD_MIN")) : (1ull << 30);
    if (off || packed_bytes < min_bytes) return false;
    switch (c->cfg.K) { case 40: return scan_takes_ranges<40>(c); case 48: return scan_takes_ranges<48>(c); case 60: return scan_takes_ranges<60>(c); }
    return false;
}

void host_sort_entries(std::vector<dfk_entry32>& v)
{
    const auto less = [](const dfk_entry32& a, const dfk_entry32& b) { return a.w0 != b.w0 ? a.w0 < b.w0 : a.w1 < b.w1; };
    const uint64_t n = v.size();
    const unsigned T = (unsigned)std::min<uint64_t>(std::max(1u, std::thread::hardware_concurrency()), std::max<uint64_t>(1, n >> 14));
    if (T <= 1) { std::sort(v.begin(), v.end(), less); return; }
    constexpr unsigned B = 4096, SH = 52;
    std::vector<dfk_entry32> tmp(n);
    std::vector<uint64_t> cnt((size_t)T * B, 0);
    auto slice = [&](unsigned t) { return std::pair<uint64_t, uint64_t>(n * t / T, n * (t + 1) / T); };
    auto run = [&](auto&& body) { std::vector<std::thread> th; for (unsigned t = 0; t < T; ++t) th.emplace_back(body, t); for (auto& x : th) x.join(); };
    run([&](unsigned t) { auto [a, b] = slice(t); uint64_t* c = &cnt[(size_t)t * B]; for (uint64_t i = a; i < b; ++i) ++c[v[i].w0 >> SH]; });
    std::vector<uint64_t> start(B + 1, 0);
    {
        uint64_t at = 0;
        for (unsigned b = 0; b < B; ++b) { start[b] = at; for (unsigned t = 0; t < T; ++t) { const uint64_t c = cnt[(size_t)t * B + b]; cnt[(size_t)t * B + b] = at; at += c; } }
        start[B] = at;
    }
    run([&](unsigned t) { auto [a, b] = slice(t); uint64_t* c = &cnt[(size_t)t * B]; for (uint64_t i = a; i < b; ++i) tmp[c[v[i].w0 >> SH]++] = v[i]; });
    std::atomic<unsigned> next{0};
    run([&](unsigned) { for (unsigned b; (b = next.fetch_add(1)) < B;) std::sort(tmp.begin() + start[b], tmp.begin() + start[b + 1], less); });
    v.swap(tmp);
}

const size_t XFER_CHUNK = [] { const char* e = getenv("DFK_XFER_CHUNK"); return e && atoll(e) >= 64 ? ((size_t)atoll(e) & ~(size_t)31) : (size_t)4 << 20; }();
unsigned xfer_threads()
{
    static const unsigned n = [] {
        if (const char* e = getenv("DFK_HOST_THREADS")) return (unsigned)std::max(1, atoi(e));
        return std::min(8u, std::max(1u, std::thread::hardware_concurrency()));
    }();
    return n;
}

struct XferLane { void* pin[2] = {nullptr, nullptr}; hipStream_t st = nullptr; hipEvent_t ev[2] = {nullptr, nullptr}; unsigned turn = 0; };
// ... 375 lines not shown
    return 0;
    });
}

int dfk_spectrum(dfk_ctx* c, const int64_t** hist, uint64_t* nbins)
{
    if (!c || !c->have) return fail(DFK_E_STATE, "no completed count");
    *hist = c->hist.data(); *nbins = c->hist.size();
    return 0;
}

int dfk_spectrum_json(dfk_ctx* c, char* out, uint64_t cap, uint64_t* need)
{
    return guarded([&]() -> int {
    if (!c || !c->have) return fail(DFK_E_STATE, "no completed count");
    std::string s = "{\n\t\"description\": \"kmer_count\",\n\t\"stage\": \"DF\",\n\t\"binsize\": 1,\n\t\"min\": 0,\n";
    s += "\t\"max\": " + std::to_string((long long)c->hist.size() - 1) + ",\n";
    s += "\t\"numbins\": " + std::to_string(c->hist.size()) + ",\n\t\"vals\": [";
    for (size_t i = 0; i < c->hist.size(); ++i) { s += std::to_string(c->hist[i]); if (i + 1 != c->hist.size()) s += ","; }
    s += "]\n}\n";
    if (need) *need = s.size();
    if (out && cap) { size_t n = std::min<size_t>(cap, s.size()); memcpy(out, s.data(), n); if (n < cap) out[n] = 0; }
    return 0;
    });
}

int dfk_solid_count(dfk_ctx* c, uint64_t* n)
{
    if (!c || !c->have) return fail(DFK_E_STATE, "no completed count");
    *n = c->n_solid;
    return 0;
}

int dfk_solid_fetch(dfk_ctx* c, dfk_entry32* out, uint64_t cap, int pre)
{
    return guarded([&]() -> int {
    if (!c || !c->have) return fail(DFK_E_STATE, "no completed count");
    if (cap < c->n_solid) return fail(DFK_E_ARG, "buffer too small: %llu < %llu", (unsigned long long)cap, (unsigned long long)c->n_solid);
    HIP_TRY(hipSetDevice(c->device));
    std::vector<dfk_entry32>* v = nullptr;
    int rc = fetch_sorted(c, pre != 0, &v); if (rc) return rc;
    if (!v->empty()) memcpy(out, v->data(), v->size() * 32);
    return 0;
    });
}

int dfk_solid_fetch_unsorted(dfk_ctx* c, dfk_entry32* out, uint64_t cap, int pre)
{
    return guarded([&]() -> int {
    if (!c || !c->have) return fail(DFK_E_STATE, "no completed count");
    if (cap < c->n_solid) return fail(DFK_E_ARG, "buffer too small: %llu < %llu", (unsigned long long)cap, (unsigned long long)c->n_solid);
    if (pre && !(c->cfg.flags & DFK_F_KEEP_PRE_ADJ)) return fail(DFK_E_STATE, "pre-adjacency view needs DFK_F_KEEP_PRE_ADJ");
    HIP_TRY(hipSetDevice(c->device));
    uint64_t at = 0;
    for (const dfk_ctx::Part& pt : c->parts) {
        const DevBuf& src = pre ? pt.pre : pt.buf;
        if (pt.n) HIP_TRY(hipMemcpy(out + at, src.p, pt.n * 32, hipMemcpyDeviceToHost));
        at += pt.n;
    }
    return 0;
    });
}

int dfk_solid_digest(dfk_ctx* c, int pre, uint64_t* digest)
{
    return guarded([&]() -> int {
    if (!c || !digest) return fail(DFK_E_ARG, "null argument");
    if (!c->have) return fail(DFK_E_STATE, "no completed count");
    if (pre && !(c->cfg.flags & DFK_F_KEEP_PRE_ADJ)) return fail(DFK_E_STATE, "pre-adjacency view needs DFK_F_KEEP_PRE_ADJ");
    HIP_TRY(hipSetDevice(c->device));
    DevBuf d; int rc = c->alloc(d, 16, "digest"); if (rc) return rc;
    HIP_TRY(hipMemsetAsync(d.p, 0, 16, c->stream));
    for (const dfk_ctx::Part& pt : c->parts) {
        const DevBuf& src = pre ? pt.pre : pt.buf;
        if (!pt.n) continue;
        const unsigned grid = (unsigned)std::min<uint64_t>((pt.n + 255) / 256, 8192);
        hipLaunchKernelGGL(k_digest, dim3(grid), dim3(256), 0, c->stream, (const uint4*)src.p, (uint64_t)pt.n, (unsigned long long*)d.p);
    }
    HIP_TRY(hipGetLastError());
    HIP_TRY(hipMemcpyAsync(digest, d.p, 16, hipMemcpyDeviceToHost, c->stream));
    HIP_TRY(hipStreamSynchronize(c->stream));
    c->release(d);
    return 0;
    });
}

int dfk_write_kvec(dfk_ctx* c, const char* path, int flags)
{
    return guarded([&]() -> int {
    if (!c || !c->have) return fail(DFK_E_STATE, "no completed count");
    if (!path) return fail(DFK_E_ARG, "null path");
    const int pre = flags & DFK_KVEC_PRE_ADJ;
    if (pre && !(c->cfg.flags & DFK_F_KEEP_PRE_ADJ)) return fail(DFK_E_STATE, "pre-adjacency view needs DFK_F_KEEP_PRE_ADJ");
    HIP_TRY(hipSetDevice(c->device));
    if (!(flags & DFK_KVEC_SORTED)) {
        const int fd = open(path, O_WRONLY | O_CREAT | O_TRUNC, 0666);
        if (fd < 0) return fail(DFK_E_ARG, "cannot open %s", path);
        const uint64_t n = c->n_solid;
        char head[16]; memcpy(head, "BINWRITE", 8); memcpy(head + 8, &n, 8);
        int rc = pwrite(fd, head, 16, 0) == 16 ? 0 : fail(DFK_E_ARG, "short write to %s", path);
        if (!rc && ftruncate(fd, (off_t)(16 + 32 * n)) != 0) rc = fail(DFK_E_ARG, "cannot size %s", path);
        if (!rc) rc = write_parts_unsorted(c, fd, pre != 0);
        if (close(fd) != 0 && !rc) rc = fail(DFK_E_ARG, "short write to %s", path);
        return rc;
    }
    std::vector<dfk_entry32>* v = nullptr;
    int rc = fetch_sorted(c, pre != 0, &v); if (rc) return rc;
    FILE* f = fopen(path, "wb");
    if (!f) return fail(DFK_E_ARG, "cannot open %s", path);
    uint64_t n = v->size();
    bool ok = fwrite("BINWRITE", 1, 8, f) == 8 && fwrite(&n, 8, 1, f) == 1 && (n == 0 || fwrite(v->data(), 32, n, f) == n);
    ok = (fclose(f) == 0) && ok;
    return ok ? 0 : fail(DFK_E_ARG, "short write to %s", path);
    });
}

int dfk_write_kvec_part(dfk_ctx* c, const char* path, int flags, uint64_t first_entry, uint64_t total_entries)
{
    return guarded([&]() -> int {
    if (!c || !c->have) return fail(DFK_E_STATE, "no completed count");
    if (!path) return fail(DFK_E_ARG, "null path");
    if (flags & DFK_KVEC_SORTED) return fail(DFK_E_ARG, "the shares of several ranks are written in device order");
    const int pre = flags & DFK_KVEC_PRE_ADJ;
    if (pre && !(c->cfg.flags & DFK_F_KEEP_PRE_ADJ)) return fail(DFK_E_STATE, "pre-adjacency view needs DFK_F_KEEP_PRE_ADJ");
    if (first_entry + c->n_solid > total_entries) return fail(DFK_E_ARG, "this rank's %llu entries from %llu on do not fit %llu", (unsigned long long)c->n_solid,
                                                              (unsigned long long)first_entry, (unsigned long long)total_entries);
    HIP_TRY(hipSetDevice(c->device));
    const int fd = open(path, O_WRONLY | O_CREAT, 0666);
    if (fd < 0) return fail(DFK_E_ARG, "cannot open %s", path);
    int rc = 0;
    if (first_entry == 0) {
        char head[16]; memcpy(head, "BINWRITE", 8); memcpy(head + 8, &total_entries, 8);
        if (pwrite(fd, head, 16, 0) != 16) rc = fail(DFK_E_ARG, "short write to %s", path);
    }
    if (!rc && ftruncate(fd, (off_t)(16 + 32 * total_entries)) != 0) rc = fail(DFK_E_ARG, "cannot size %s", path);
    if (!rc) rc = write_parts_unsorted(c, fd, pre != 0, 16 + 32 * first_entry);
    if (close(fd) != 0 && !rc) rc = fail(DFK_E_ARG, "short write to %s", path);
    return rc;
    });
}

int dfk_get_stats(dfk_ctx* c, dfk_stats* out)
{
    if (!c || !out) return fail(DFK_E_ARG, "null argument");
    if (c->d_resident && hipSetDevice(c->device) == hipSuccess) {
        unsigned int t = 0;
        if (hipMemcpy(&t, c->d_resident + 1, 4, hipMemcpyDeviceToHost) == hipSuccess) c->st.reserved[4] = t;
    }
    c->st.reserved[5] = c->held;
    *out = c->st;
    return 0;
}

}

#include "dfk_shard.inc"
#include "dfk_graph.inc"
#include "dfk_paths.inc"
#include "dfk_hops.inc"
#include "dfk_subset.inc"
#include "dfk_paths_shard.inc"
#include "dfk_pbf.inc"
```

superplus_amd/csrc/dfk_arena.h:

```cpp
#pragma once
#include <algorithm>
#include <cstdarg>
#include <cstdint>
#include <cstdio>
#include <string>
#include <vector>

namespace dfk {

struct DevBuf {
    void* p = nullptr; size_t bytes = 0;
    bool sub = false;
};

enum class Place {
    High,
    Low,
};

class Arena {
public:
    enum { E_BUDGET = 1, E_FRAGMENTED, E_BACKING };
    struct Free { uint64_t off, bytes; };
    struct PassBlock { DevBuf block; size_t used = 0; };
    struct Current {
        Arena& a;
        Current(Arena& ar, PassBlock& blk) : a(ar) { a.sub = &blk; }
        ~Current() { a.sub = nullptr; }
    };
    typedef void* (*GetFn)(uint64_t bytes, const char** why);
    typedef void (*GiveFn)(void* p);

    uint64_t budget = 0, held = 0, peak = 0;
    uint64_t reserved = 0;
    uint64_t alloc_seq = 0;
    uint64_t first_chunk_hint = 0;
    bool trace = false;
    std::string err;

    Arena(GetFn get_, GiveFn give_) : get(get_), give(give_) {}

    int alloc(DevBuf& b, size_t bytes, const char* what, Place where = Place::High)
    {
        bytes = bytes ? (bytes + 255) & ~(size_t)255 : 256;
        if (sub && where == Place::High && sub->used + bytes <= sub->block.bytes) {
            b.p = (char*)sub->block.p + sub->used; b.bytes = bytes; b.sub = true;
            sub->used += bytes;
            return 0;
        }
        if (held + bytes > budget)
            return fail(E_BUDGET, "HBM budget exceeded allocating %zu bytes for %s (held %llu, budget %llu)",
                        bytes, what, (unsigned long long)held, (unsigned long long)budget);
        bool ok = false;
        for (Chunk& k : chunks) if (carve(k, bytes, b, where)) { ok = true; break; }
        if (!ok) {
            uint64_t want = std::max<uint64_t>(2 * (uint64_t)bytes, 64ull << 20);
            if (chunks.empty()) want = std::max<uint64_t>(want, std::min<uint64_t>(first_chunk_hint, budget));
            if (reserved + want > budget) { drop_empty_chunks(); want = std::min<uint64_t>(want, budget > reserved ? budget - reserved : 0); }
            want &= ~(uint64_t)0xFFF;
            if (want < bytes) {
                if (trace) {
                    for (const Chunk& k : chunks) trace_free(k.free_list);
                    for (const Owned& o : owned) if (o.bytes >= (1ull << 28)) fprintf(stderr, "[dfk]   held %.2f GB at %.2f GB (#%llu)\n", o.bytes / 1e9, ((char*)o.p - chunks[0].p) / 1e9, (unsigned long long)o.seq);
                }
                return fail(E_FRAGMENTED, "HBM budget exhausted by fragmentation allocating %zu bytes for %s", bytes, what);
            }
            const char* why = "";
            void* p = get(want, &why);
            if (!p && want > bytes) { want = bytes; p = get(want, &why); }
            if (!p) return fail(E_BACKING, "hipMalloc(%llu) for %s: %s", (unsigned long long)want, what, why);
            chunks.push_back(Chunk{(char*)p, want, {Free{0, want}}});
            reserved += want;
            say("new device chunk %p, %.2f GB (reserved %.2f of %.2f GB)", p, want / 1e9, (reserved) / 1e9, budget / 1e9);
            carve(chunks.back(), bytes, b, where);
        }
        held += bytes; peak = std::max(peak, held);
        owned.push_back(Owned{b.p, (uint64_t)bytes, ++alloc_seq});
        if (bytes >= (1ull << 30)) say("alloc %-28s %8.2f GB at %p (%s), held %.2f GB", what, bytes / 1e9, b.p, where == Place::Low ? "low" : "high", held / 1e9);
        return 0;
    }
    uint64_t largest_allocatable() const
    {
        uint64_t best = budget > reserved ? (budget - reserved) & ~(uint64_t)0xFFF : 0;
        for (const Chunk& k : chunks) for (const Free& f : k.free_list) best = std::max<uint64_t>(best, f.bytes);
        return std::min<uint64_t>(best, budget > held ? budget - held : 0);
    }
    void release(DevBuf& b)
    {
        if (!b.p) return;
        if (b.sub) { b = DevBuf{}; return; }
        auto it = std::find_if(owned.begin(), owned.end(), [&](const Owned& o) { return o.p == b.p; });
        if (it != owned.end()) owned.erase(it);
        for (Chunk& k : chunks)
            if ((char*)b.p >= k.p && (char*)b.p < k.p + k.bytes) {
                std::vector<Free>& fl = k.free_list;
                const uint64_t off = (uint64_t)((char*)b.p - k.p);
                size_t i = 0;
                while (i < fl.size() && fl[i].off < off) ++i;
                fl.insert(fl.begin() + i, Free{off, b.bytes});
                if (i + 1 < fl.size() && fl[i].off + fl[i].bytes == fl[i + 1].off) { fl[i].bytes += fl[i + 1].bytes; fl.erase(fl.begin() + i + 1); }
                if (i > 0 && fl[i - 1].off + fl[i - 1].bytes == fl[i].off) { fl[i - 1].bytes += fl[i].bytes; fl.erase(fl.begin() + i); }
                break;
            }
        held -= b.bytes; b.p = nullptr; b.bytes = 0;
    }
    void shrink(DevBuf& b, size_t keep)
    {
        keep = keep ? (keep + 255) & ~(size_t)255 : 256;
        if (!b.p || keep >= b.bytes) return;
        auto it = std::find_if(owned.begin(), owned.end(), [&](const Owned& o) { return o.p == b.p; });
        DevBuf tail; tail.p = (char*)b.p + keep; tail.bytes = b.bytes - keep;
        b.bytes = keep;
        if (it != owned.end()) { it->bytes = keep; owned.push_back(Owned{tail.p, (uint64_t)tail.bytes, it->seq}); }
        else owned.push_back(Owned{tail.p, (uint64_t)tail.bytes, alloc_seq});
        release(tail);
    }
    void release_since(uint64_t mark, const DevBuf* keep = nullptr)
    {
        for (size_t i = owned.size(); i-- > 0;)
            if (owned[i].seq > mark && !(keep && owned[i].p == keep->p)) { DevBuf b; b.p = owned[i].p; b.bytes = owned[i].bytes; release(b); }
    }
    void drop_empty_chunks()
    {
        for (size_t i = 0; i < chunks.size();)
            if (chunks[i].free_list.size() == 1 && chunks[i].free_list[0].bytes == chunks[i].bytes) drop_chunk(i);
            else ++i;
    }
    void drop_pool() { while (!chunks.empty()) drop_chunk(chunks.size() - 1); }
    void adopt(void* p, uint64_t bytes) { chunks.push_back(Chunk{(char*)p, bytes, {Free{0, bytes}}, true}); reserved += bytes; }
    void reset()
    {
        owned.clear(); held = 0;
        for (size_t i = 0; i < chunks.size();) if (chunks[i].adopted) drop_chunk(i); else ++i;
        for (Chunk& k : chunks) k.free_list.assign(1, Free{0, k.bytes});
    }
    const std::vector<Free>* free_blocks() const { return chunks.size() == 1 ? &chunks[0].free_list : nullptr; }
    uint64_t offset_of(const DevBuf& b) const
    {
        for (const Chunk& k : chunks) if ((char*)b.p >= k.p && (char*)b.p < k.p + k.bytes) return (uint64_t)((char*)b.p - k.p);
        return 0;
    }
    static void trace_free(const std::vector<Free>& fl) { for (const Free& f : fl) fprintf(stderr, "[dfk]   free %.2f GB at %.2f GB\n", f.bytes / 1e9, f.off / 1e9); }

private:
    friend struct ArenaTest;
    struct Chunk { char* p; uint64_t bytes; std::vector<Free> free_list; bool adopted = false; };
    struct Owned { void* p; uint64_t bytes, seq; };
    GetFn get; GiveFn give;
    std::vector<Chunk> chunks;
    std::vector<Owned> owned;
    PassBlock* sub = nullptr;

    bool carve(Chunk& k, size_t bytes, DevBuf& b, Place where)
    {
        if (where == Place::High) {
            for (size_t i = k.free_list.size(); i-- > 0;)
                if (k.free_list[i].bytes >= bytes) {
                    k.free_list[i].bytes -= bytes;
                    b.p = k.p + k.free_list[i].off + k.free_list[i].bytes; b.bytes = bytes;
                    if (!k.free_list[i].bytes) k.free_list.erase(k.free_list.begin() + i);
                    return true;
                }
            return false;
        }
        for (size_t i = 0; i < k.free_list.size(); ++i)
            if (k.free_list[i].bytes >= bytes) {
                b.p = k.p + k.free_list[i].off; b.bytes = bytes;
                k.free_list[i].off += bytes; k.free_list[i].bytes -= bytes;
                if (!k.free_list[i].bytes) k.free_list.erase(k.free_list.begin() + i);
                return true;
            }
        return false;
    }
    void drop_chunk(size_t i) { give(chunks[i].p); reserved -= chunks[i].bytes; chunks.erase(chunks.begin() + i); }
    int fail(int code, const char* fmt, ...)
    {
        char buf[512];
        va_list ap; va_start(ap, fmt); vsnprintf(buf, sizeof buf, fmt, ap); va_end(ap);
        err = buf;
        return code;
    }
    void say(const char* fmt, ...) const
    {
        if (!trace) return;
        fputs("[dfk] ", stderr);
        va_list ap; va_start(ap, fmt); vfprintf(stderr, fmt, ap); va_end(ap);
        fputc('\n', stderr); fflush(stderr);
    }
};


inline uint64_t pass_block_bytes(uint32_t n, uint32_t sub_nb, uint64_t n_records)
{
    const double share = (double)n / sub_nb;
    return (uint64_t)(1.01 * (80.0 * n + 32.0 * share * (double)n_records)) + (16ull << 20);
}
inline uint64_t part_entries(uint64_t n_inst, uint32_t min_freq, uint64_t inst_seen, uint64_t solid_seen)
{
    const uint64_t cap = n_inst / std::max<uint32_t>(1, min_freq) + 1;
    if (inst_seen) return std::min<uint64_t>(cap, (uint64_t)(1.10 * (double)solid_seen / (double)inst_seen * (double)n_inst) + 65536);
    return std::min<uint64_t>(cap, n_inst / 10 + (1u << 20));
}

struct PlanInputs {
    double room;
    uint32_t sub_nb, lo;
    uint64_t n_inst, n_records;
    uint64_t inst_seen, solid_seen;
    uint32_t min_freq; unsigned seg_attempt;
    double plan_derate;
    bool overlap;
    double first_div, growth;
    bool trace;
};
struct RunningPass { uint64_t bytes_held; uint64_t n_inst; uint32_t n_buckets; uint64_t block_off; };

inline double fit_free_blocks(const std::vector<Arena::Free>* fl_, double per_block, double per_res, const RunningPass& run)
{
    if (!fl_ || fl_->empty()) return 1e300;
    const std::vector<Arena::Free>& fl = *fl_;
    auto feasible = [&](double n) {
        const uint64_t B = (uint64_t)(per_block * n / 0.98) + 1;
        size_t at = fl.size();
        for (size_t i = fl.size(); i-- > 0;) if (fl[i].bytes >= B) { at = i; break; }
        if (at == fl.size()) return false;
        std::vector<Arena::Free> h(fl.begin(), fl.end());
        h[at].bytes -= B;
        h.push_back(Arena::Free{run.block_off, run.bytes_held});
        std::sort(h.begin(), h.end(), [](const Arena::Free& a, const Arena::Free& b) { return a.off < b.off; });
        uint64_t low_off = 0, low_bytes = 0; bool have = false;
        for (const Arena::Free& f : h) {
            if (!f.bytes) continue;
            if (!have) { low_off = f.off; low_bytes = f.bytes; have = true; }
            else if (low_off + low_bytes == f.off) low_bytes += f.bytes;
            else break;
        }
        return per_res * n <= 0.98 * (double)low_bytes;
    };
    double lo = 0.0, hi = 0.0;
// ... 52 lines not shown
```

superplus_amd/csrc/dfk_kernels.h:

```cpp
#pragma once
#include <type_traits>
#include "dfk_device.h"
#include "dfk_fallback.h"
#include "dfk_scan_plan.h"

namespace dfk {

template <int K>
__global__ void __launch_bounds__(256)
k_trim(const uint8_t* __restrict__ pq, const uint64_t* __restrict__ pq_off, uint64_t pq_nbytes,
       const uint64_t* __restrict__ base_off, uint64_t packed_bytes, const uint32_t* __restrict__ read_len,
       uint64_t n_reads, uint32_t min_qual, uint32_t* __restrict__ good_len,
       unsigned long long* __restrict__ n_inst, unsigned int* __restrict__ bad,
       unsigned long long* __restrict__ sum_good)
{
    unsigned long long mine = 0, good = 0;
    bool any_bad = false;
    for (uint64_t r = (uint64_t)blockIdx.x * blockDim.x + threadIdx.x; r < n_reads; r += (uint64_t)gridDim.x * blockDim.x) {
        uint32_t gl = 0;
        uint64_t p = pq_off[r], end = pq_off[r + 1];
        uint32_t idx = 0, run = 0;
        const uint64_t b0 = base_off[r], b1 = base_off[r + 1];
        bool ok = p <= end && end <= pq_nbytes && b0 <= b1 && b1 <= packed_bytes && b1 - b0 >= ((uint64_t)read_len[r] + 3) / 4;
        if (!ok) end = p;
// ... 1560 lines not shown
    if (threadIdx.x == 0 && ovf) atomicOr(failed, 1u);
}

template <int K> struct BigView {
    uint32_t* keys; uint32_t* cnt; uint32_t* ctxs; uint32_t* wide; uint32_t* bcw; uint32_t S, slot;
    __device__ __forceinline__ uint32_t count() const { const uint32_t c = tld(&wide[slot]); return c < CNT_MASK ? c : CNT_MASK; }
};
template <int K>
__device__ __forceinline__ BigView<K> big_view(const BigItem* __restrict__ items, const uint64_t* __restrict__ slot_pre, uint32_t n_items,
                                               uint32_t* __restrict__ tab_pool, uint64_t x)
{
    const uint32_t it = big_find(slot_pre, n_items, x);
    const BigItem I = items[it];
    const uint32_t S = 1u << I.log2s;
    uint32_t* keys = tab_pool + I.tab_off;
    uint32_t* cnt = keys + (size_t)KTraits<K>::KW * S;
    return BigView<K>{keys, cnt, cnt + S, cnt + 2 * (size_t)S, cnt + 3 * (size_t)S, S, (uint32_t)(x - slot_pre[it])};
}

template <int K, int NBC>
__global__ void __launch_bounds__(256)
k_big_flags(const BigItem* __restrict__ items, const uint64_t* __restrict__ slot_pre, uint32_t n_items, uint32_t* __restrict__ tab_pool,
            CountParams cp, CountGlobals* __restrict__ g)
{
    const uint64_t total = slot_pre[n_items];
    uint32_t occ = 0;
    for (uint64_t x = (uint64_t)blockIdx.x * 256 + threadIdx.x; x < total; x += (uint64_t)gridDim.x * 256) {
        const BigView<K> v = big_view<K>(items, slot_pre, n_items, tab_pool, x);
        const uint32_t c = tld(&v.cnt[v.slot]);
        if (!c) continue;
        ++occ;
        const bool solid = v.count() >= cp.min_freq && bc_pass<(NBC > 0)>(NBC > 0 ? tld(&v.bcw[v.slot]) : 0u, cp.min_bc);
        if (solid && cp.do_adj && cp.keep_pre) { const uint32_t ctx = tld(&v.ctxs[v.slot]) & 0xFFu; tst(&v.ctxs[v.slot], ctx | (ctx << 8)); }
        tst(&v.bcw[v.slot], solid ? FLAG_SOLID : 0u);
    }
#pragma unroll
    for (int d = 32; d > 0; d >>= 1) occ += __shfl_down(occ, d, 64);
    if ((threadIdx.x & 63) == 0 && occ) atomicAdd(&g->n_distinct, (unsigned long long)occ);
}

template <int K>
__global__ void __launch_bounds__(256)
k_big_resolve(const BigItem* __restrict__ items, const uint64_t* __restrict__ slot_pre, uint32_t n_items, uint32_t* __restrict__ tab_pool)
{
    constexpr int KW = KTraits<K>::KW;
    const uint64_t total = slot_pre[n_items];
    const u128 m = KTraits<K>::mask();
    for (uint64_t x = (uint64_t)blockIdx.x * 256 + threadIdx.x; x < total; x += (uint64_t)gridDim.x * 256) {
        const BigView<K> v = big_view<K>(items, slot_pre, n_items, tab_pool, x);
        if (!tld(&v.cnt[v.slot]) || !(tld(&v.bcw[v.slot]) & FLAG_SOLID)) continue;
        const uint32_t S = v.S, slot = v.slot;
        const u128 F{(uint64_t)tld(&v.keys[slot]) | ((uint64_t)tld(&v.keys[S + slot]) << 32),
                     (uint64_t)tld(&v.keys[2 * (size_t)S + slot]) | (KW == 4 ? ((uint64_t)tld(&v.keys[3 * (size_t)S + slot]) << 32) : 0ull)};
        for (uint32_t ctx = tld(&v.ctxs[slot]) & 0xFFu; ctx; ctx &= ctx - 1) {
            const uint32_t bit = (uint32_t)__ffs(ctx) - 1u;
            u128 nb;
            if (bit < 4) { nb = shl128(F, 2); nb.lo &= m.lo; nb.hi &= m.hi; nb.lo |= bit; }
            else {
                nb = shr128(F, 2);
                constexpr int TOP = KTraits<K>::BITS - 2;
                if (TOP >= 64) nb.hi |= (uint64_t)(bit - 4) << (TOP - 64); else nb.lo |= (uint64_t)(bit - 4) << TOP;
            }
            const uint32_t f = table_find<KW>(v.keys, v.cnt, S, canon_value<K>(nb));
            if (f == ~0u) atomicOr(&v.bcw[slot], 1u << bit);
            else if (!(tld(&v.bcw[f]) & FLAG_SOLID)) atomicAnd(&v.ctxs[slot], ~(1u << bit));
        }
    }
}

template <int K>
__global__ void __launch_bounds__(256)
k_big_emit(const BigItem* __restrict__ items, const uint64_t* __restrict__ slot_pre, uint32_t n_items, uint32_t* __restrict__ tab_pool,
           CountParams cp, CountGlobals* __restrict__ g, uint4* __restrict__ out, unsigned long long* __restrict__ hist_global)
{
    constexpr int KW = KTraits<K>::KW;
    const uint64_t total = slot_pre[n_items];
    const int lane = threadIdx.x & 63;
    uint32_t boundary = 0;
    const uint64_t rounds = (total + (uint64_t)gridDim.x * 256 - 1) / ((uint64_t)gridDim.x * 256);
    for (uint64_t r = 0; r < rounds; ++r) {
        const uint64_t x = (r * gridDim.x + blockIdx.x) * 256 + threadIdx.x;
        bool solid = false; BigView<K> v{}; uint32_t c = 0, flags = 0;
        if (x < total) {
            v = big_view<K>(items, slot_pre, n_items, tab_pool, x);
            c = tld(&v.cnt[v.slot]);
            flags = c ? tld(&v.bcw[v.slot]) : 0u;
            solid = (flags & FLAG_SOLID) != 0;
        }
        const unsigned long long mk = __ballot(solid);
        if (!mk) continue;
        unsigned long long wbase = 0;
        if (lane == 0) wbase = atomicAdd(&g->big_cursor, (unsigned long long)__popcll(mk));
        wbase = uniform64((uint64_t)wbase);
        if (!solid) continue;
        const uint32_t S = v.S, slot = v.slot, count = v.count();
        const uint32_t cw = tld(&v.ctxs[slot]);
        const uint32_t pending = flags & 0xFFu & cw;
        boundary += pending != 0;
        const unsigned long long idx = wbase + __popcll(mk & ((1ull << lane) - 1ull));
        if (idx < cp.seg_cap) {
            const u128 kv{(uint64_t)tld(&v.keys[slot]) | ((uint64_t)tld(&v.keys[S + slot]) << 32),
                          (uint64_t)tld(&v.keys[2 * (size_t)S + slot]) | (KW == 4 ? ((uint64_t)tld(&v.keys[3 * (size_t)S + slot]) << 32) : 0ull)};
            const u128 kw = shl128(kv, 128 - KTraits<K>::BITS);
            out[2 * idx] = uint4{(uint32_t)kw.hi, (uint32_t)(kw.hi >> 32), (uint32_t)kw.lo, (uint32_t)(kw.lo >> 32)};
            out[2 * idx + 1] = uint4{0xFFFFFFFFu, count | ((cw & 0xFFu) << 24), 0xFFFFFFFFu, pending | (cw & 0xFF00u)};
        } else atomicOr(&g->solid_overflow, 1u);
        atomicAdd(&hist_global[count], 1ull);
    }
#pragma unroll
    for (int d = 32; d > 0; d >>= 1) boundary += __shfl_down(boundary, d, 64);
    if (lane == 0 && boundary) atomicAdd(&g->n_boundary, (unsigned long long)boundary);
}

__global__ void __launch_bounds__(256)
k_fill_holes(uint4* __restrict__ out, const uint64_t* __restrict__ src, const uint64_t* __restrict__ dst, uint64_t n)
{
    const uint64_t i = (uint64_t)blockIdx.x * blockDim.x + threadIdx.x;
    if (i >= n) return;
    out[2 * dst[i]] = out[2 * src[i]];
    out[2 * dst[i] + 1] = out[2 * src[i] + 1];
}

__device__ __forceinline__ uint64_t digest_mix(uint64_t x)
{
    x ^= x >> 30; x *= 0xBF58476D1CE4E5B9ull;
    x ^= x >> 27; x *= 0x94D049BB133111EBull;
    return x ^ (x >> 31);
}

__global__ void __launch_bounds__(256)
k_digest(const uint4* __restrict__ entries, uint64_t n, unsigned long long* __restrict__ digest)
{
    uint64_t sum = 0, xr = 0;
    for (uint64_t i = (uint64_t)blockIdx.x * blockDim.x + threadIdx.x; i < n; i += (uint64_t)gridDim.x * blockDim.x) {
        const uint4 a = entries[2 * i], b = entries[2 * i + 1];
        const uint64_t w0 = a.x | ((uint64_t)a.y << 32), w1 = a.z | ((uint64_t)a.w << 32);
        const uint64_t w2 = b.x | ((uint64_t)b.y << 32), w3 = b.z | ((uint64_t)b.w << 32);
        const uint64_t h = digest_mix(w0 ^ digest_mix(w1 ^ digest_mix(w2 ^ digest_mix(w3 + 0x9E3779B97F4A7C15ull))));
        sum += h; xr ^= digest_mix(h + 0xD1B54A32D192ED03ull);
    }
#pragma unroll
    for (int d = 32; d > 0; d >>= 1) { sum += __shfl_down(sum, d, 64); xr ^= __shfl_down(xr, d, 64); }
    if ((threadIdx.x & 63) == 0) { atomicAdd(&digest[0], sum); atomicXor(&digest[1], xr); }
}

struct SetSlot { uint64_t w0, w1; };

__device__ __forceinline__ uint64_t set_hash(uint64_t w0, uint64_t w1)
{
    uint64_t h = w0 * 0x9E3779B97F4A7C15ull ^ (w1 + 0x7F4A7C159E3779B9ull) * 0xC2B2AE3D27D4EB4Full;
    h ^= h >> 29;
    return h;
}

__global__ void __launch_bounds__(256)
k_set_insert(const uint4* __restrict__ entries, uint64_t n, SetSlot* __restrict__ set, uint64_t mask)
{
    uint64_t i = (uint64_t)blockIdx.x * blockDim.x + threadIdx.x;
    if (i >= n) return;
    if (!(entries[2 * i + 1].w & 0xFFu)) return;
    uint4 a = entries[2 * i];
    uint64_t w0 = (uint64_t)a.x | ((uint64_t)a.y << 32), w1 = (uint64_t)a.z | ((uint64_t)a.w << 32);
    uint64_t s = set_hash(w0, w1) & mask;
    for (;;) {
        unsigned long long old = atomicCAS(reinterpret_cast<unsigned long long*>(&set[s].w0), ~0ull, (unsigned long long)w0);
        if (old == ~0ull) { set[s].w1 = w1; return; }
        s = (s + 1) & mask;
    }
}

__device__ __forceinline__ bool set_has(const SetSlot* __restrict__ set, uint64_t mask, uint64_t w0, uint64_t w1)
{
    uint64_t s = set_hash(w0, w1) & mask;
    for (;;) {
        SetSlot v = set[s];
        if (v.w0 == ~0ull) return false;
        if (v.w0 == w0 && v.w1 == w1) return true;
        s = (s + 1) & mask;
    }
}

constexpr int BLIST_PER_THREAD = 8;
__global__ void __launch_bounds__(256)
k_boundary_list(const uint4* __restrict__ entries, uint64_t n, uint32_t* __restrict__ list, uint64_t cap,
                unsigned long long* __restrict__ ctl)
{
    __shared__ uint32_t found[256 * BLIST_PER_THREAD];
    __shared__ uint32_t n_found;
    __shared__ unsigned long long at;
    const int lane = threadIdx.x & 63;
    const uint64_t per_block = 256ull * BLIST_PER_THREAD;
    for (uint64_t b0 = (uint64_t)blockIdx.x * per_block; b0 < n; b0 += (uint64_t)gridDim.x * per_block) {
        if (threadIdx.x == 0) n_found = 0;
        __syncthreads();
#pragma unroll
        for (int j = 0; j < BLIST_PER_THREAD; ++j) {
            const uint64_t i = b0 + 256ull * j + threadIdx.x;
            const bool hit = i < n && (entries[2 * i + 1].w & 0xFFu) != 0u;
            const unsigned long long mk = __ballot(hit);
            uint32_t w = 0;
            if (lane == 0 && mk) w = atomicAdd(&n_found, (uint32_t)__popcll(mk));
            w = __builtin_amdgcn_readfirstlane(w);
            if (hit) found[w + __popcll(mk & ((1ull << lane) - 1ull))] = (uint32_t)i;
        }
        __syncthreads();
        const uint32_t m = n_found;
        if (threadIdx.x == 0) at = m ? atomicAdd(&ctl[0], (unsigned long long)m) : 0ull;
        __syncthreads();
        const unsigned long long base = at;
        if (base + m > cap) { if (threadIdx.x == 0) atomicOr(&ctl[1], 1ull); }
        else for (uint32_t t = threadIdx.x; t < m; t += 256) list[base + t] = found[t];
        __syncthreads();
    }
}

__global__ void __launch_bounds__(256)
k_set_insert_list(const uint4* __restrict__ entries, const uint32_t* __restrict__ list, uint64_t n, SetSlot* __restrict__ set, uint64_t mask)
{
    const uint64_t t = (uint64_t)blockIdx.x * blockDim.x + threadIdx.x;
    if (t >= n) return;
    const uint4 a = entries[2 * (uint64_t)list[t]];
    const uint64_t w0 = (uint64_t)a.x | ((uint64_t)a.y << 32), w1 = (uint64_t)a.z | ((uint64_t)a.w << 32);
    uint64_t s = set_hash(w0, w1) & mask;
    for (uint64_t step = 0; step <= mask; ++step) {
        unsigned long long old = atomicCAS(reinterpret_cast<unsigned long long*>(&set[s].w0), ~0ull, (unsigned long long)w0);
        if (old == ~0ull) { set[s].w1 = w1; return; }
        s = (s + 1) & mask;
    }
}

template <int K>
__device__ __forceinline__ void canon_words(u128 F, uint64_t* w0, uint64_t* w1)
{
    const u128 m = KTraits<K>::mask();
    u128 nf{~F.lo & m.lo, ~F.hi & m.hi};
    u128 top = shl128(nf, 128 - KTraits<K>::BITS);
    u128 R{rev2_64(top.hi), rev2_64(top.lo)};
    u128 c = lt128(R, F) ? R : F;
    u128 kw = shl128(c, 128 - KTraits<K>::BITS);
    *w0 = kw.hi; *w1 = kw.lo;
}

template <int K>
__device__ __forceinline__ uint32_t adjacency_entry(uint4* __restrict__ entries, uint64_t i, const SetSlot* __restrict__ set, uint64_t mask)
{
    const u128 m = KTraits<K>::mask();
    uint4 b = entries[2 * i + 1];
    const uint32_t pending = b.w & 0xFFu;
    if (!pending) return 0;
    uint4 a = entries[2 * i];
    u128 kw{(uint64_t)a.z | ((uint64_t)a.w << 32), (uint64_t)a.x | ((uint64_t)a.y << 32)};
    u128 F = shr128(kw, 128 - KTraits<K>::BITS);
    uint32_t ctx = b.y >> 24, probes = 0;
    for (uint32_t bit = 0; bit < 8; ++bit) if (pending & (1u << bit)) {
        u128 v;
        if (bit < 4) { v = shl128(F, 2); v.lo &= m.lo; v.hi &= m.hi; v.lo |= bit; }
        else {
            v = shr128(F, 2);
            constexpr int TOP = KTraits<K>::BITS - 2;
            if (TOP >= 64) v.hi |= (uint64_t)(bit - 4) << (TOP - 64); else v.lo |= (uint64_t)(bit - 4) << TOP;
        }
        uint64_t w0, w1; canon_words<K>(v, &w0, &w1);
        ++probes;
        if (!set_has(set, mask, w0, w1)) ctx &= ~(1u << bit);
    }
    b.y = (b.y & 0xFFFFFFu) | (ctx << 24);
    b.w = 0;
    entries[2 * i + 1] = b;
    return probes;
}

__device__ __forceinline__ void add_probes(unsigned long long probes, unsigned long long* __restrict__ n_probes)
{
    __shared__ unsigned long long sh[4];
#pragma unroll
    for (int d = 32; d > 0; d >>= 1) probes += __shfl_down(probes, d, 64);
    if ((threadIdx.x & 63) == 0) sh[threadIdx.x >> 6] = probes;
    __syncthreads();
    if (threadIdx.x == 0 && (sh[0] + sh[1] + sh[2] + sh[3])) atomicAdd(n_probes, sh[0] + sh[1] + sh[2] + sh[3]);
}

template <int K>
__global__ void __launch_bounds__(256)
k_adjacency(uint4* __restrict__ entries, uint64_t n, const SetSlot* __restrict__ set, uint64_t mask,
            unsigned long long* __restrict__ n_probes)
{
    unsigned long long probes = 0;
    for (uint64_t i = (uint64_t)blockIdx.x * blockDim.x + threadIdx.x; i < n; i += (uint64_t)gridDim.x * blockDim.x)
        probes += adjacency_entry<K>(entries, i, set, mask);
    add_probes(probes, n_probes);
}

template <int K>
__global__ void __launch_bounds__(256)
k_adjacency_list(uint4* __restrict__ entries, const uint32_t* __restrict__ list, uint64_t n, const SetSlot* __restrict__ set, uint64_t mask,
                 unsigned long long* __restrict__ n_probes)
{
    unsigned long long probes = 0;
    for (uint64_t t = (uint64_t)blockIdx.x * blockDim.x + threadIdx.x; t < n; t += (uint64_t)gridDim.x * blockDim.x)
        probes += adjacency_entry<K>(entries, (uint64_t)list[t], set, mask);
    add_probes(probes, n_probes);
}

__global__ void __launch_bounds__(256)
k_make_pre(uint4* __restrict__ entries, uint4* __restrict__ pre, uint64_t n)
{
    uint64_t i = (uint64_t)blockIdx.x * blockDim.x + threadIdx.x;
    if (i >= n) return;
    uint4 a = entries[2 * i], b = entries[2 * i + 1];
    pre[2 * i] = a;
    pre[2 * i + 1] = uint4{b.x, (b.y & 0xFFFFFFu) | (((b.w >> 8) & 0xFFu) << 24), b.z, 0u};
    b.w &= 0xFFu;
    entries[2 * i + 1] = b;
}

__global__ void __launch_bounds__(256)
k_clear_pad(uint4* __restrict__ entries, uint64_t n)
{
    uint64_t i = (uint64_t)blockIdx.x * blockDim.x + threadIdx.x;
    if (i >= n) return;
    uint32_t* w = reinterpret_cast<uint32_t*>(entries + 2 * i + 1) + 3;
    if (*w) *w = 0;
}

template <int K>
__device__ __forceinline__ uint32_t kmer_bucket(u128 F, const PartParams& pp)
{
    const uint32_t M = pp.M;
    const uint32_t mmask = M == 16 ? 0xFFFFFFFFu : ((1u << (2 * M)) - 1u);
    const uint32_t rsh = 2 * (M - 1);
    uint32_t f = 0, rc = 0, mv = 0xFFFFFFFFu;
    for (int i = 0; i < K; ++i) {
        const int sh = 2 * (K - 1 - i);
        const uint32_t b = (uint32_t)(sh >= 64 ? (F.hi >> (sh - 64)) : (F.lo >> sh)) & 3u;
        f = ((f << 2) | b) & mmask;
        rc = (rc >> 2) | ((3u - b) << rsh);
        if (i + 1 >= (int)M) { uint32_t h = mmer_hash(f < rc ? f : rc); mv = h < mv ? h : mv; }
    }
    uint32_t bucket = (mv * 0x9E3779B1u) >> (32 - pp.log2_nb);
    return bucket;
}

constexpr int ADJ_PER_THREAD = 8, ADJ_ROUND = 256 * ADJ_PER_THREAD;

__device__ __forceinline__ uint32_t block_excl_scan_256(uint32_t v, uint32_t* scratch, uint32_t* total)
{
    const int lane = threadIdx.x & 63, wave = threadIdx.x >> 6;
    const uint32_t incl = wave_incl_scan(v, lane);
    if (lane == 63) scratch[wave] = incl;
    __syncthreads();
    uint32_t off = 0;
    for (int w = 0; w < wave; ++w) off += scratch[w];
    *total = scratch[0] + scratch[1] + scratch[2] + scratch[3];
    __syncthreads();
    return off + incl - v;
}

constexpr uint32_t RG_LOG2_PARTS = 12, RG_PARTS = 1u << RG_LOG2_PARTS;
constexpr uint32_t RG_FINE = 4096;

__global__ void __launch_bounds__(256)
k_rg_hist(const uint4* __restrict__ in, uint64_t n, uint64_t chunk, uint32_t local_mask, uint32_t part_shift, uint32_t n_parts,
          uint64_t* __restrict__ h1)
{
    __shared__ uint32_t hist[RG_PARTS];
    for (uint32_t i = threadIdx.x; i < n_parts; i += 256) hist[i] = 0;
    __syncthreads();
    const uint64_t lo = (uint64_t)blockIdx.x * chunk, hi = lo + chunk < n ? lo + chunk : n;
    for (uint64_t i = lo + threadIdx.x; i < hi; i += 256)
        atomicAdd(&hist[((in[2 * i].x >> 8) & local_mask) >> part_shift], 1u);
    __syncthreads();
    for (uint32_t i = threadIdx.x; i < n_parts; i += 256) h1[(uint64_t)i * gridDim.x + blockIdx.x] = hist[i];
}

__global__ void __launch_bounds__(256)
k_rg_scatter(const uint4* __restrict__ in, uint64_t n, uint64_t chunk, uint32_t local_mask, uint32_t part_shift, uint32_t n_parts,
             const uint64_t* __restrict__ h1off, uint4* __restrict__ out)
{
    __shared__ unsigned long long cur[RG_PARTS];
    for (uint32_t i = threadIdx.x; i < n_parts; i += 256) cur[i] = h1off[(uint64_t)i * gridDim.x + blockIdx.x];
    __syncthreads();
    const uint64_t lo = (uint64_t)blockIdx.x * chunk, hi = lo + chunk < n ? lo + chunk : n;
    for (uint64_t i = lo + threadIdx.x; i < hi; i += 256) {
        const uint4 a = in[2 * i], b = in[2 * i + 1];
        const unsigned long long dst = atomicAdd(&cur[((a.x >> 8) & local_mask) >> part_shift], 1ull);
        out[2 * dst] = a; out[2 * dst + 1] = b;
    }
}

__global__ void __launch_bounds__(256)
k_rg_finish(const uint4* __restrict__ in, uint64_t n, uint32_t local_mask, uint32_t part_shift, uint32_t n_parts, uint32_t n_blocks1,
            const uint64_t* __restrict__ h1off, unsigned long long* __restrict__ bucket_acc, uint4* __restrict__ out)
{
    __shared__ uint32_t rec[RG_FINE], inst[RG_FINE];
    __shared__ uint32_t scratch[8];
    const uint32_t fine = 1u << part_shift, fmask = fine - 1u;
    for (uint32_t p = blockIdx.x; p < n_parts; p += gridDim.x) {
        const uint64_t s = h1off[(uint64_t)p * n_blocks1], e = p + 1 < n_parts ? h1off[(uint64_t)(p + 1) * n_blocks1] : n;
        for (uint32_t i = threadIdx.x; i < fine; i += 256) { rec[i] = 0; inst[i] = 0; }
        __syncthreads();
        for (uint64_t i = s + threadIdx.x; i < e; i += 256) {
            const uint32_t h = in[2 * i].x, f = (h >> 8) & fmask;
            atomicAdd(&rec[f], 1u); atomicAdd(&inst[f], h & 63u);
        }
        __syncthreads();
        uint32_t carry = 0;
        for (uint32_t f0 = 0; f0 < fine; f0 += 256) {
            const uint32_t f = f0 + threadIdx.x;
            const uint32_t r = f < fine ? rec[f] : 0u;
            if (f < fine) bucket_acc[(uint64_t)p * fine + f] = ((unsigned long long)r << 32) | inst[f];
            uint32_t total;
            const uint32_t ex = block_excl_scan_256(r, scratch, &total);
            if (f < fine) rec[f] = carry + ex;
            carry += total;
        }
        __syncthreads();
        for (uint64_t i = s + threadIdx.x; i < e; i += 256) {
            const uint4 a = in[2 * i], b = in[2 * i + 1];
            const uint64_t dst = s + atomicAdd(&rec[(a.x >> 8) & fmask], 1u);
            out[2 * dst] = a; out[2 * dst + 1] = b;
        }
        __syncthreads();
    }
}

__global__ void __launch_bounds__(256)
k_adj_list(const uint4* __restrict__ entries, uint64_t n, unsigned long long* __restrict__ n_items, uint64_t* __restrict__ list)
{
    __shared__ uint32_t scratch[8];
    __shared__ unsigned long long base;
    for (uint64_t i0 = (uint64_t)blockIdx.x * ADJ_ROUND; i0 < n; i0 += (uint64_t)gridDim.x * ADJ_ROUND) {
        uint32_t pend[ADJ_PER_THREAD], mine = 0;
#pragma unroll
        for (int k = 0; k < ADJ_PER_THREAD; ++k) {
            const uint64_t i = i0 + 256ull * k + threadIdx.x;
            pend[k] = i < n ? entries[2 * i + 1].w & 0xFFu : 0u;
            mine += __popc(pend[k]);
        }
        uint32_t total;
        uint32_t at = block_excl_scan_256(mine, scratch, &total);
        if (threadIdx.x == 0) base = total && list ? atomicAdd(n_items, (unsigned long long)total) : 0ull;
        if (!list) { if (threadIdx.x == 0 && total) atomicAdd(n_items, (unsigned long long)total); continue; }
        __syncthreads();
        const unsigned long long b = base;
#pragma unroll
        for (int k = 0; k < ADJ_PER_THREAD; ++k) {
            const uint64_t i = i0 + 256ull * k + threadIdx.x;
            for (uint32_t p = pend[k]; p; p &= p - 1) list[b + at++] = (i << 3) | (uint32_t)(__ffs(p) - 1);
        }
        __syncthreads();
    }
}

template <int K>
__global__ void __launch_bounds__(256)
k_adj_owner(const uint4* __restrict__ entries, const uint64_t* __restrict__ list, uint64_t n_items, PartParams pp,
            SetSlot* __restrict__ tmp_keys, uint8_t* __restrict__ owner, unsigned long long* __restrict__ per_owner)
{
    __shared__ unsigned int cnt[256];
    const uint32_t world = 1u << pp.log2_world;
    const u128 m = KTraits<K>::mask();
    if (threadIdx.x < world) cnt[threadIdx.x] = 0;
    __syncthreads();
    for (uint64_t j = (uint64_t)blockIdx.x * 256 + threadIdx.x; j < n_items; j += (uint64_t)gridDim.x * 256) {
        const uint64_t s = list[j];
        const uint32_t bit = (uint32_t)s & 7u;
        const uint4 a = entries[2 * (s >> 3)];
        const u128 kw{(uint64_t)a.z | ((uint64_t)a.w << 32), (uint64_t)a.x | ((uint64_t)a.y << 32)};
        const u128 F = shr128(kw, 128 - KTraits<K>::BITS);
        u128 v;
        if (bit < 4) { v = shl128(F, 2); v.lo &= m.lo; v.hi &= m.hi; v.lo |= bit; }
        else {
            v = shr128(F, 2);
            constexpr int TOP = KTraits<K>::BITS - 2;
            if (TOP >= 64) v.hi |= (uint64_t)(bit - 4) << (TOP - 64); else v.lo |= (uint64_t)(bit - 4) << TOP;
        }
        const uint32_t o = kmer_bucket<K>(v, pp) & (world - 1);
        uint64_t w0, w1; canon_words<K>(v, &w0, &w1);
        tmp_keys[j] = SetSlot{w0, w1};
        owner[j] = (uint8_t)o;
        atomicAdd(&cnt[o], 1u);
    }
    __syncthreads();
    if (threadIdx.x < world && cnt[threadIdx.x]) atomicAdd(&per_owner[threadIdx.x], (unsigned long long)cnt[threadIdx.x]);
}

__global__ void __launch_bounds__(256)
k_adj_place(const uint64_t* __restrict__ list, const SetSlot* __restrict__ tmp_keys, const uint8_t* __restrict__ owner, uint64_t n_items,
            uint32_t world, const uint64_t* __restrict__ base, unsigned long long* __restrict__ fill,
            SetSlot* __restrict__ keys, uint64_t* __restrict__ src)
{
    __shared__ unsigned int cnt[256];
    __shared__ unsigned long long start[256];
    for (uint64_t j0 = (uint64_t)blockIdx.x * ADJ_ROUND; j0 < n_items; j0 += (uint64_t)gridDim.x * ADJ_ROUND) {
        if (threadIdx.x < world) cnt[threadIdx.x] = 0;
        __syncthreads();
        uint32_t own[ADJ_PER_THREAD];
#pragma unroll
        for (int k = 0; k < ADJ_PER_THREAD; ++k) {
            const uint64_t j = j0 + 256ull * k + threadIdx.x;
            own[k] = j < n_items ? owner[j] : 0xFFFFFFFFu;
            if (own[k] != 0xFFFFFFFFu) atomicAdd(&cnt[own[k]], 1u);
        }
        __syncthreads();
        if (threadIdx.x < world) {
            const unsigned int c = cnt[threadIdx.x];
            start[threadIdx.x] = base[threadIdx.x] + (c ? atomicAdd(&fill[threadIdx.x], (unsigned long long)c) : 0ull);
            cnt[threadIdx.x] = 0;
        }
        __syncthreads();
#pragma unroll
        for (int k = 0; k < ADJ_PER_THREAD; ++k) {
            const uint64_t j = j0 + 256ull * k + threadIdx.x;
            if (own[k] == 0xFFFFFFFFu) continue;
            const uint64_t pos = start[own[k]] + atomicAdd(&cnt[own[k]], 1u);
            keys[pos] = tmp_keys[j];
            src[pos] = list[j];
        }
        __syncthreads();
    }
}

__global__ void __launch_bounds__(256)
k_adj_answer(const SetSlot* __restrict__ keys, uint64_t n, const SetSlot* __restrict__ set, uint64_t mask,
             uint8_t* __restrict__ present)
{
    const uint64_t i = (uint64_t)blockIdx.x * blockDim.x + threadIdx.x;
    if (i >= n) return;
    SetSlot k = keys[i];
    present[i] = set_has(set, mask, k.w0, k.w1) ? 1 : 0;
}

__global__ void __launch_bounds__(256)
k_adj_apply(uint4* __restrict__ entries, const uint64_t* __restrict__ src, const uint8_t* __restrict__ present, uint64_t n)
{
    const uint64_t i = (uint64_t)blockIdx.x * blockDim.x + threadIdx.x;
    if (i >= n || present[i]) return;
    const uint64_t s = src[i];
    uint32_t* word = reinterpret_cast<uint32_t*>(entries + 2 * (s >> 3) + 1) + 1;
    atomicAnd(word, ~(1u << (24 + (uint32_t)(s & 7))));
}

__global__ void __launch_bounds__(256)
k_select_overflow(const uint4* __restrict__ summaries, uint64_t n_reads, uint32_t* __restrict__ list,
                  unsigned long long* __restrict__ n_list)
{
    __shared__ unsigned long long base;
    __shared__ uint32_t wcnt[4];
    const uint32_t* first = reinterpret_cast<const uint32_t*>(summaries);
    const uint64_t per = (n_reads + gridDim.x - 1) / gridDim.x;
    const uint64_t lo = (uint64_t)blockIdx.x * per, hi = lo + per < n_reads ? lo + per : n_reads;
    const int lane = threadIdx.x & 63, wave = threadIdx.x >> 6;
    uint32_t mine = 0;
    for (uint64_t r = lo + threadIdx.x; r < hi; r += blockDim.x) mine += (first[4 * r] & 15u) == SUMMARY_OVERFLOW;
#pragma unroll
    for (int d = 32; d > 0; d >>= 1) mine += __shfl_down(mine, d, 64);
    if (lane == 0) wcnt[wave] = mine;
    __syncthreads();
    if (threadIdx.x == 0) { uint32_t t = wcnt[0] + wcnt[1] + wcnt[2] + wcnt[3]; base = t ? atomicAdd(n_list, (unsigned long long)t) : 0ull; }
    __syncthreads();
    if (wcnt[0] + wcnt[1] + wcnt[2] + wcnt[3] == 0) return;
    unsigned long long at = base;
    for (uint64_t r0 = lo; r0 < hi; r0 += blockDim.x) {
        const uint64_t r = r0 + threadIdx.x;
        const bool keep = r < hi && (first[4 * r] & 15u) == SUMMARY_OVERFLOW;
        const unsigned long long m = __ballot(keep);
        __syncthreads();
        if (lane == 0) wcnt[wave] = __popcll(m);
        __syncthreads();
        uint32_t off = 0;
        for (int w = 0; w < wave; ++w) off += wcnt[w];
        if (keep) list[at + off + __popcll(m & ((1ull << lane) - 1ull))] = (uint32_t)r;
        at += wcnt[0] + wcnt[1] + wcnt[2] + wcnt[3];
    }
}


constexpr int SCAN_THREADS = 256, SCAN_ITEMS = 8;
__global__ void __launch_bounds__(SCAN_THREADS)
k_scan_blocks(const uint64_t* __restrict__ in, uint64_t* __restrict__ out, uint64_t n, uint64_t* __restrict__ sums)
{
    __shared__ uint64_t wsum[SCAN_THREADS / 64];
    const uint64_t base = ((uint64_t)blockIdx.x * SCAN_THREADS + threadIdx.x) * SCAN_ITEMS;
    uint64_t v[SCAN_ITEMS], run = 0;
#pragma unroll
    for (int i = 0; i < SCAN_ITEMS; ++i) { v[i] = base + i < n ? in[base + i] : 0; run += v[i]; }
    const int lane = threadIdx.x & 63, wave = threadIdx.x >> 6;
    uint64_t incl = run;
#pragma unroll
    for (int d = 1; d < 64; d <<= 1) { uint64_t o = __shfl_up(incl, d, 64); if (lane >= d) incl += o; }
    if (lane == 63) wsum[wave] = incl;
    __syncthreads();
    uint64_t woff = 0;
    for (int w = 0; w < wave; ++w) woff += wsum[w];
    uint64_t ex = woff + incl - run;
#pragma unroll
    for (int i = 0; i < SCAN_ITEMS; ++i) { if (base + i < n) out[base + i] = ex; ex += v[i]; }
    if (threadIdx.x == SCAN_THREADS - 1 && sums) sums[blockIdx.x] = woff + incl;
}

__global__ void __launch_bounds__(SCAN_THREADS)
k_scan_add(uint64_t* __restrict__ out, uint64_t n, const uint64_t* __restrict__ sums)
{
    const uint64_t add = sums[blockIdx.x];
    const uint64_t base = ((uint64_t)blockIdx.x * SCAN_THREADS + threadIdx.x) * SCAN_ITEMS;
#pragma unroll
    for (int i = 0; i < SCAN_ITEMS; ++i) if (base + i < n) out[base + i] += add;
}

__global__ void __launch_bounds__(256)
k_check_cursors(const unsigned long long* __restrict__ cur, const uint64_t* __restrict__ base, uint64_t nb, unsigned int* __restrict__ bad)
{
    unsigned int wrong = 0;
    const uint64_t stride = (uint64_t)gridDim.x * blockDim.x;
    for (uint64_t b0 = (uint64_t)blockIdx.x * blockDim.x + threadIdx.x; b0 < nb; b0 += 4 * stride) {
        unsigned long long c[4]; uint64_t e[4];
#pragma unroll
        for (int k = 0; k < 4; ++k) { const uint64_t b = b0 + k * stride; c[k] = b < nb ? cur[b] : 0ull; e[k] = b < nb ? base[b + 1] : 0ull; }
#pragma unroll
        for (int k = 0; k < 4; ++k) wrong += c[k] != e[k];
    }
    if (wrong) atomicAdd(bad, wrong);
}

__global__ void __launch_bounds__(256)
k_slice(const unsigned long long* __restrict__ acc, uint32_t log2_sub, uint32_t sub_lo, uint32_t sub_n, uint64_t nb_local,
        uint64_t* __restrict__ rec, uint64_t* __restrict__ inst)
{
    const uint64_t j = (uint64_t)blockIdx.x * blockDim.x + threadIdx.x;
    if (j > nb_local) return;
    const uint64_t owner = j / sub_n, d = j - owner * sub_n;
    unsigned long long h = j < nb_local ? acc[(owner << log2_sub) + sub_lo + d] : 0ull;
    rec[j] = h >> 32; inst[j] = h & 0xFFFFFFFFull;
}

__global__ void __launch_bounds__(256)
k_item_flags(const uint64_t* __restrict__ ipre, uint64_t nb, uint64_t budget, uint64_t* __restrict__ flags)
{
    const uint64_t b = (uint64_t)blockIdx.x * blockDim.x + threadIdx.x;
    if (b > nb) return;
    flags[b] = b < nb && (b == 0 || ipre[b] / budget != ipre[b - 1] / budget) ? 1 : 0;
}

__global__ void __launch_bounds__(256)
k_item_pairs(const uint64_t* __restrict__ flags, const uint64_t* __restrict__ idx, uint64_t nb, ItemRange* __restrict__ items)
{
    const uint64_t b = (uint64_t)blockIdx.x * blockDim.x + threadIdx.x;
    if (b >= nb || !flags[b]) return;
    const uint64_t k = idx[b];
    items[k].b0 = (uint32_t)b;
    if (k) items[k - 1].b1 = (uint32_t)b;
    if (k + 1 == idx[nb]) items[k].b1 = (uint32_t)nb;
}

__global__ void __launch_bounds__(256)
k_sum_acc(const unsigned long long* __restrict__ acc, uint64_t nb, unsigned long long* __restrict__ out)
{
    unsigned long long r = 0, i = 0;
    for (uint64_t b = (uint64_t)blockIdx.x * blockDim.x + threadIdx.x; b < nb; b += (uint64_t)gridDim.x * blockDim.x)
    { r += acc[b] >> 32; i += acc[b] & 0xFFFFFFFFull; }
#pragma unroll
    for (int d = 32; d > 0; d >>= 1) { r += __shfl_down(r, d, 64); i += __shfl_down(i, d, 64); }
    if ((threadIdx.x & 63) == 0) { if (r) atomicAdd(&out[0], r); if (i) atomicAdd(&out[1], i); }
}

__global__ void __launch_bounds__(256)
k_gather_u64(const uint64_t* __restrict__ src, const uint32_t* __restrict__ idx, uint32_t n, uint64_t* __restrict__ out)
{
    uint32_t i = blockIdx.x * blockDim.x + threadIdx.x;
    if (i < n) out[i] = src[idx[i]];
}

__global__ void __launch_bounds__(256)
k_sample_u64(const uint64_t* __restrict__ src, uint64_t stride, uint64_t n, uint64_t n_out, uint64_t* __restrict__ out)
{
    const uint64_t i = (uint64_t)blockIdx.x * blockDim.x + threadIdx.x;
    if (i < n_out) out[i] = src[min(i * stride, n)];
}

__global__ void __launch_bounds__(256)
k_dense_sizes(const uint32_t* __restrict__ read_len, uint64_t n, uint64_t* __restrict__ out )
{
    for (uint64_t i = (uint64_t)blockIdx.x * 256 + threadIdx.x; i <= n; i += (uint64_t)gridDim.x * 256) out[i] = i < n ? ((uint64_t)read_len[i] + 3) >> 2 : 0;
// ... 30 lines not shown
```

superplus_amd/csrc/dfk_shard.inc:

```
namespace {

struct CallClock {
    dfk_ctx* c; float* also; std::chrono::steady_clock::time_point t0 = std::chrono::steady_clock::now();
    CallClock(dfk_ctx* ctx, float* stage) : c(ctx), also(stage) {}
    ~CallClock()
    {
        if (!c) return;
        (void)hipStreamSynchronize(c->stream);
        const float ms = std::chrono::duration<float, std::milli>(std::chrono::steady_clock::now() - t0).count();
        c->st.ms_total += ms;
        c->st.hbm_bytes_peak = c->peak;
        if (also) *also += ms;
    }
};

uint32_t log2_exact(uint32_t v) { uint32_t l = 0; while ((1u << l) < v) ++l; return l; }

struct PendingPartition {
    bool active = false, launched = false, last = false;
    uint32_t pass = 0, world = 0;
    DevBuf d_slice, d_fill;
    std::vector<uint64_t> expect;
    std::function<int()> launch;
    hipEvent_t e0 = nullptr, e1 = nullptr;
// ... 324 lines not shown
int dfk_shard_begin_host(dfk_ctx* c, const uint8_t* packed, const uint64_t* base_off, const uint32_t* read_len,
                         const uint8_t* pq, const uint64_t* pq_off, const int32_t* bc, uint64_t n_reads,
                         int64_t global_read_offset, uint64_t* n_inst_local)
{
    return guarded([&]() -> int {
    if (!c || !n_inst_local) return fail(DFK_E_ARG, "null argument");
    if (n_reads && (!packed || !base_off || !read_len || !pq || !pq_off)) return fail(DFK_E_ARG, "null input array");
    HIP_TRY(hipSetDevice(c->device));
    c->release_all();
    int rd = 0;
    auto at = [&](const void* tab, uint64_t i) { uint64_t v = 0; if (!rd) rd = host_read(c, &v, (const char*)tab + 8 * i, 8); return v; };
    const uint64_t b0 = n_reads ? at(base_off, 0) & ~(uint64_t)3 : 0, b1 = n_reads ? at(base_off, n_reads) : 0;
    const uint64_t q0 = n_reads ? at(pq_off, 0) : 0, q1 = n_reads ? at(pq_off, n_reads) : 0;
    if (rd) return rd;
    if (b1 < b0 || q1 < q0) return fail(DFK_E_INPUT, "offset tables are not ascending");
    int rc = 0;
    Timer t(c->stream);
    t.start();
    auto up = [&](int slot, const void* h, uint64_t bytes) {
        if (rc) return;
        if (hipMalloc(&c->sh_staged[slot], bytes + 64) != hipSuccess) { (void)hipGetLastError(); rc = fail(DFK_E_NOMEM, "no room on the device for %llu bytes of input", (unsigned long long)bytes); return; }
        rc = upload(c, c->sh_staged[slot], h, bytes);
    };
    up(0, packed + b0, b1 - b0);
    up(1, base_off, (n_reads + 1) * 8);
    up(2, read_len, n_reads * 4);
    up(3, pq + q0, q1 - q0);
    up(4, pq_off, (n_reads + 1) * 8);
    if (bc) up(5, bc, n_reads * 4);
    const float ms_up = t.stop();
    if (rc) { for (void*& p : c->sh_staged) if (p) { (void)hipFree(p); p = nullptr; } return rc; }
    const uint64_t staged = (b1 - b0) + (q1 - q0) + (n_reads + 1) * 16 + n_reads * 8 + 6 * 64;
    void* keep[6]; memcpy(keep, c->sh_staged, sizeof keep); memset(c->sh_staged, 0, sizeof keep);
    rc = dfk_shard_begin(c, (const char*)keep[0] - b0, b1, keep[1], keep[2], (const char*)keep[3] - q0, q1, keep[4], bc ? keep[5] : nullptr, n_reads,
                         global_read_offset, n_inst_local);
    memcpy(c->sh_staged, keep, sizeof keep);
    if (rc) { for (void*& p : c->sh_staged) if (p) { (void)hipFree(p); p = nullptr; } return rc; }
    c->sh_b0 = b0; c->sh_b1 = b1; c->sh_q0 = q0; c->sh_q1 = q1; c->sh_staged_reads = n_reads;
    c->budget_taken = std::min(c->budget, staged);
    c->budget -= c->budget_taken;
    c->st.ms_upload = ms_up;
    return 0;
    });
}

int dfk_shard_plan(dfk_ctx* c, uint32_t world, uint64_t n_inst_global, uint32_t* log2_passes)
{
    return guarded([&]() -> int {
    if (!c || !log2_passes) return fail(DFK_E_ARG, "null argument");
    if (!c->shard_open) return fail(DFK_E_STATE, "dfk_shard_begin has not been called");
    if (world == 0 || (world & (world - 1)) || world > 64) return fail(DFK_E_ARG, "world must be a power of two <= 64");
    HIP_TRY(hipSetDevice(c->device));
    CallClock clock(c, nullptr);
    switch (c->cfg.K) {
    case 40: return shard_plan_typed<40>(c, world, n_inst_global, log2_passes);
    case 48: return shard_plan_typed<48>(c, world, n_inst_global, log2_passes);
    default: return shard_plan_typed<60>(c, world, n_inst_global, log2_passes);
    }
    });
}

int dfk_shard_partition_begin(dfk_ctx* c, uint32_t world, uint64_t n_inst_global, uint32_t log2_passes, uint32_t pass, int defer,
                              const void** d_records, uint64_t* send_counts)
{
    return guarded([&]() -> int {
    if (!c || !d_records || !send_counts) return fail(DFK_E_ARG, "null argument");
    if (!c->shard_open) return fail(DFK_E_STATE, "dfk_shard_begin has not been called");
    if (world == 0 || (world & (world - 1)) || world > 64) return fail(DFK_E_ARG, "world must be a power of two <= 64");
    if (log2_passes > 8 || pass >= (1u << log2_passes)) return fail(DFK_E_ARG, "pass %u of 2^%u", pass, log2_passes);
    HIP_TRY(hipSetDevice(c->device));
    CallClock clock(c, nullptr);
    switch (c->cfg.K) {
    case 40: return shard_partition_begin_typed<40>(c, world, n_inst_global, log2_passes, pass, defer != 0, d_records, send_counts);
    case 48: return shard_partition_begin_typed<48>(c, world, n_inst_global, log2_passes, pass, defer != 0, d_records, send_counts);
    default: return shard_partition_begin_typed<60>(c, world, n_inst_global, log2_passes, pass, defer != 0, d_records, send_counts);
    }
    });
}

int dfk_shard_partition_end(dfk_ctx* c, uint32_t pass)
{
    return guarded([&]() -> int {
    if (!c) return fail(DFK_E_ARG, "null context");
    if (!c->shard_open || !c->shard_state) return fail(DFK_E_STATE, "dfk_shard_partition_begin has not been called");
    HIP_TRY(hipSetDevice(c->device));
    CallClock clock(c, nullptr);
    return shard_partition_end(c, pass);
    });
}

int dfk_shard_partition(dfk_ctx* c, uint32_t world, uint64_t n_inst_global, uint32_t log2_passes, uint32_t pass,
                        const void** d_records, uint64_t* send_counts)
{
    const int rc = dfk_shard_partition_begin(c, world, n_inst_global, log2_passes, pass, 0, d_records, send_counts);
    return rc ? rc : dfk_shard_partition_end(c, pass);
}

int dfk_shard_recv_buffer(dfk_ctx* c, uint64_t n_records, void** d_buf)
{
    return guarded([&]() -> int {
    if (!c || !d_buf) return fail(DFK_E_ARG, "null argument");
    if (!c->shard_open) return fail(DFK_E_STATE, "dfk_shard_begin has not been called");
    HIP_TRY(hipSetDevice(c->device));
    CallClock clock(c, nullptr);
    DevBuf& rb = c->shard_recv[c->shard_recv_seq++ & 1];
    c->release(rb);
    int rc = c->alloc(rb, std::max<uint64_t>(1, n_records) * 32, "received records"); if (rc) return rc;
    *d_buf = rb.p;
    return 0;
    });
}

int dfk_shard_count(dfk_ctx* c, const void* d_records, uint64_t n_records, uint32_t pass)
{
    return guarded([&]() -> int {
    if (!c) return fail(DFK_E_ARG, "null context");
    if (!c->shard_open || !c->shard_state) return fail(DFK_E_STATE, "dfk_shard_partition has not been called");
    if (n_records && !d_records) return fail(DFK_E_ARG, "null records");
    HIP_TRY(hipSetDevice(c->device));
    CallClock clock(c, nullptr);
    switch (c->cfg.K) {
    case 40: return shard_count_typed<40>(c, d_records, n_records, pass);
    case 48: return shard_count_typed<48>(c, d_records, n_records, pass);
    default: return shard_count_typed<60>(c, d_records, n_records, pass);
    }
    });
}

int dfk_shard_adj_queries(dfk_ctx* c, const void** d_keys, uint64_t* send_counts)
{
    return guarded([&]() -> int {
    if (!c || !d_keys || !send_counts) return fail(DFK_E_ARG, "null argument");
    if (!c->have) return fail(DFK_E_STATE, "dfk_shard_count has not completed");
    HIP_TRY(hipSetDevice(c->device));
    CallClock clock(c, &c->st.ms_adjacency);
    switch (c->cfg.K) {
    case 40: return shard_adj_queries_typed<40>(c, d_keys, send_counts);
    case 48: return shard_adj_queries_typed<48>(c, d_keys, send_counts);
    default: return shard_adj_queries_typed<60>(c, d_keys, send_counts);
    }
    });
}

int dfk_shard_adj_answer(dfk_ctx* c, const void* d_keys, uint64_t n_keys, void* d_present)
{
    return guarded([&]() -> int {
    if (!c) return fail(DFK_E_ARG, "null context");
    if (!c->have || !c->set.p) return fail(DFK_E_STATE, "dfk_shard_count has not completed");
    if (n_keys == 0) return 0;
    if (!d_keys || !d_present) return fail(DFK_E_ARG, "null argument");
    HIP_TRY(hipSetDevice(c->device));
    CallClock clock(c, &c->st.ms_adjacency);
    hipLaunchKernelGGL(k_adj_answer, dim3((unsigned)((n_keys + 255) / 256)), dim3(256), 0, c->stream, (const SetSlot*)d_keys, n_keys,
                       (const SetSlot*)c->set.p, c->set_mask, (uint8_t*)d_present);
    HIP_TRY(hipGetLastError());
    HIP_TRY(hipStreamSynchronize(c->stream));
    return 0;
    });
}

int dfk_shard_adj_apply(dfk_ctx* c, const void* d_present, uint64_t n_keys)
{
    return guarded([&]() -> int {
    if (!c) return fail(DFK_E_ARG, "null context");
    if (!c->have) return fail(DFK_E_STATE, "dfk_shard_count has not completed");
    if (n_keys != c->adj_n) return fail(DFK_E_ARG, "expected %llu answers, got %llu", (unsigned long long)c->adj_n, (unsigned long long)n_keys);
    HIP_TRY(hipSetDevice(c->device));
    CallClock clock(c, &c->st.ms_adjacency);
    if (n_keys) {
        if (!d_present) return fail(DFK_E_ARG, "null answers");
        hipLaunchKernelGGL(k_adj_apply, dim3((unsigned)((n_keys + 255) / 256)), dim3(256), 0, c->stream, (uint4*)c->parts[0].buf.p,
                           (const uint64_t*)c->adj_src.p, (const uint8_t*)d_present, n_keys);
        HIP_TRY(hipGetLastError());
        HIP_TRY(hipStreamSynchronize(c->stream));
    }
    if (c->n_solid) {
        hipLaunchKernelGGL(k_clear_pad, dim3((unsigned)((c->n_solid + 255) / 256)), dim3(256), 0, c->stream, (uint4*)c->parts[0].buf.p, c->n_solid);
        HIP_TRY(hipGetLastError());
        HIP_TRY(hipStreamSynchronize(c->stream));
    }
    c->release(c->adj_keys); c->release(c->adj_src); c->release(c->set);
    c->sorted_ok = false;
    return 0;
    });
}

int dfk_shard_dict_share(dfk_ctx* c, const void** d_entries, uint64_t* n_entries)
{
    if (!c || !d_entries || !n_entries) return fail(DFK_E_ARG, "null argument");
    if (!c->have) return fail(DFK_E_STATE, "no completed count");
    if (c->parts.size() > 1) return fail(DFK_E_STATE, "the dictionary is in %zu parts: a sharded run leaves one", c->parts.size());
    *d_entries = c->parts.empty() ? nullptr : c->parts[0].buf.p;
    *n_entries = c->parts.empty() ? 0 : c->parts[0].n;
    return 0;
}

int dfk_shard_dict_adopt(dfk_ctx* c, uint64_t n_entries, void** d_room)
{
    return guarded([&]() -> int {
    if (!c || !d_room) return fail(DFK_E_ARG, "null argument");
    if (!c->have) return fail(DFK_E_STATE, "no completed count");
    HIP_TRY(hipSetDevice(c->device));
    *d_room = nullptr;
    if (c->shard_state) {
        ShardState* S = shard_state(c);
        for (DevBuf* d : {&S->T.acc, &S->T.summ, &S->T.classes, &S->T.ovf_list, &S->T.class_hist}) c->release(*d);
        c->shard_state_free(c->shard_state); c->shard_state = nullptr;
    }
    if (!(c->cfg.flags & DFK_F_KEEP_INPUTS)) {
        for (void*& p : c->sh_staged) if (p) { (void)hipFree(p); p = nullptr; }
        c->budget += c->budget_taken; c->budget_taken = 0; c->sh_staged_reads = 0;
    } else if (c->sh_staged[5]) { (void)hipFree(c->sh_staged[5]); c->sh_staged[5] = nullptr; }
    for (DevBuf* d : {&c->shard_send[0], &c->shard_send[1], &c->shard_recv[0], &c->shard_recv[1], &c->adj_keys, &c->adj_src, &c->set}) c->release(*d);
    if (!n_entries) return 0;
    dfk_ctx::Part pt; pt.n = n_entries;
    int rc = c->alloc(pt.buf, n_entries * 32, "solid k-mer entries of the other ranks"); if (rc) return rc;
    *d_room = pt.buf.p;
    c->parts.push_back(pt);
    return 0;
    });
}

int dfk_shard_dict_whole(dfk_ctx* c)
{
    return guarded([&]() -> int {
    if (!c) return fail(DFK_E_ARG, "null context");
    if (!c->have) return fail(DFK_E_STATE, "no completed count");
    uint64_t n = 0;
    for (const dfk_ctx::Part& pt : c->parts) n += pt.n;
    c->n_solid = n; c->st.n_solid = n;
    if (c->shard_state) { c->shard_state_free(c->shard_state); c->shard_state = nullptr; }
    c->shard_world = 1; c->shard_open = false;
    c->sorted_ok = c->sorted_pre_ok = false;
    for (dfk_ctx::Part& pt : c->parts) c->release(pt.pre);
    return 0;
    });
}

}
```

superplus_amd/dfk.py:

```python
import ctypes as C
import os
import subprocess

import numpy as np

_HERE = os.path.dirname(os.path.abspath(__file__))
LIB_PATH = os.environ.get("DFK_LIB") or os.path.join(_HERE, "libdfk.so")
ABI_VERSION = 3
F_KEEP_PRE_ADJ = 1
F_KEEP_INPUTS = 2
F_MARK_BADS = 4

ENTRY_DTYPE = np.dtype([("w0", "<u8"), ("w1", "<u8"), ("edge_id", "<u4"), ("count_ctx", "<u4"),
                        ("bc", "<i4"), ("pad", "<u4")])

EXPORTS = [
    "dfk_create", "dfk_destroy", "dfk_last_error", "dfk_abi_version", "dfk_count", "dfk_count_bci", "dfk_count_device",
    "dfk_hint_file_range", "dfk_qual_hist", "dfk_paths_sink", "dfk_good_lens", "dfk_spectrum", "dfk_spectrum_json", "dfk_solid_count", "dfk_solid_fetch", "dfk_solid_fetch_unsorted", "dfk_solid_digest",
    "dfk_write_kvec", "dfk_write_kvec_part", "dfk_get_stats", "dfk_shard_begin", "dfk_shard_begin_host", "dfk_shard_plan", "dfk_shard_partition", "dfk_shard_partition_begin", "dfk_shard_partition_end", "dfk_shard_recv_buffer", "dfk_shard_count", "dfk_shard_adj_queries",
    "dfk_shard_adj_answer", "dfk_shard_adj_apply", "dfk_graph_build", "dfk_graph_stats", "dfk_graph_write",
    "dfk_shard_dict_share", "dfk_shard_dict_adopt", "dfk_shard_dict_whole",
    "dfk_paths_build", "dfk_paths_build_device", "dfk_paths_stats", "dfk_paths_write", "dfk_paths_fetch", "dfk_paths_index_write", "dfk_dups_write", "dfk_paths_index_dups_write",
    "dfk_paths_digest", "dfk_paths_verify", "dfk_paths_verify_device", "dfk_pbf_run", "dfk_pbf_result", "dfk_pbf_free",
    "dfk_paths_var_bytes", "dfk_paths_write_part", "dfk_shard_pidx_pairs", "dfk_shard_pidx_write", "dfk_shard_dup_keys", "dfk_shard_dup_answer", "dfk_shard_dup_write",
    "dfk_bads_sums", "dfk_bads_write", "dfk_bads_write_part",
    "dfk_hops_build", "dfk_hops_build_bci", "dfk_hops_build_arrays", "dfk_hops_stats", "dfk_hops_fetch", "dfk_hops_write",
    "dfk_subset_build", "dfk_subset_build_arrays", "dfk_subset_stats", "dfk_subset_fetch", "dfk_subset_write",
]

CHECK_WORDS = 20
CK = ["PATHS_SUM", "PATHS_XOR", "N_READS", "N_PLACED", "N_PATH_EDGES", "INV_SUM", "INV_XOR", "INV_STARTS", "INV_ENTRIES",
      "COUNTSB_DIGEST", "COUNTSB_SUM", "SELF_INVERSE", "DUP_DIGEST", "DUP_MARKED", "EDGE_KMERS", "N_SOLID", "INV_VIOLATIONS",
      "N_EDGES", "VALID"]
HOPS_WORDS = 16
HOPS = ["m1", "m2", "m3", "pairs", "searched", "extended", "host_edges", "most_rounds", "us", "us_index", "us_m12", "us_m3", "us_host", "largest_x", "ranges"]
SUBSET_WORDS = 16
SUBSET = ["eoi", "ids", "path_entries", "index_entries", "ranges", "one_read_only", "us", "us_sweep", "us_gather", "us_index",
          "ids_sum", "ids_xor", "eoi_sum", "eoi_xor"]
SUBSET_FILES = ("a.sub.ids", "a.sub.eoi", "a.sub.paths", "a.sub.paths.inv")
VERIFY = ["placed", "broken", "hits", "consistent", "no_anchor", "all_consistent", "dict_bad", "outside"]


class DfkError(RuntimeError):
    def __init__(self, code, msg):
        super().__init__(f"dfk error {code}: {msg}")
        self.code = code


class Config(C.Structure):
    _fields_ = [("abi_version", C.c_uint32), ("K", C.c_uint32), ("min_qual", C.c_uint32), ("min_freq", C.c_uint32),
                ("min_bc", C.c_uint32), ("device", C.c_int32), ("ign_bc_below", C.c_int64),
                ("hbm_budget_bytes", C.c_uint64), ("minimizer_len", C.c_uint32), ("flags", C.c_uint32),
                ("inst_per_item", C.c_uint64), ("reserved", C.c_uint64 * 4)]


class Stats(C.Structure):
    _fields_ = [("n_reads", C.c_uint64), ("n_inst", C.c_uint64), ("n_records", C.c_uint64), ("n_buckets", C.c_uint64),
                ("n_items", C.c_uint64), ("n_overflow_items", C.c_uint64), ("n_distinct", C.c_uint64),
                ("n_solid", C.c_uint64), ("adj_probes", C.c_uint64),
                ("ms_upload", C.c_float), ("ms_trim", C.c_float), ("ms_part_count", C.c_float),
                ("ms_part_scatter", C.c_float), ("ms_count", C.c_float), ("ms_fallback", C.c_float),
                ("ms_adjacency", C.c_float), ("ms_total", C.c_float),
                ("hbm_bytes_peak", C.c_uint64), ("reserved", C.c_uint64 * 8)]

    def asdict(self):
        d = {k: getattr(self, k) for k, _ in self._fields_ if k != "reserved"}
        d["n_passes"] = int(self.reserved[0])
        d["us_graph_device"], d["us_graph_host"], d["us_paths"] = int(self.reserved[1]), int(self.reserved[2]), int(self.reserved[3])
        d["gate_timeouts"] = int(self.reserved[4])
        d["hbm_held"] = int(self.reserved[5])
        d["n_scan_launches"] = int(self.reserved[6])
        d["us_bad_sums"] = int(self.reserved[7])
        return d


_lib = None


def build():
    subprocess.check_call(["make", "-s", "-C", os.path.join(_HERE, "csrc")])


def lib():
    global _lib
    if _lib is None:
        if not os.path.exists(LIB_PATH):
            raise DfkError(-2, f"{LIB_PATH} is missing: run `make -C superplus_amd/csrc` (hipcc, gfx950). "
                               "There is no CPU fallback.")
        L = C.CDLL(LIB_PATH)
        L.dfk_last_error.restype = C.c_char_p
        _lib = L
    return _lib


def _check(rc):
    if rc != 0:
        raise DfkError(rc, lib().dfk_last_error().decode())


def _p(a):
    return None if a is None else a.ctypes.data_as(C.c_void_p)


class Dfk:

    def __init__(self, K=48, min_qual=7, min_freq=3, min_bc=2, ign_bc_below=0, device=0, hbm_budget_bytes=0,
                 minimizer_len=0, keep_pre_adjacency=False, inst_per_item=0, passes=0, keep_inputs=False, mark_bads=False):
        cfg = Config(abi_version=ABI_VERSION, K=K, min_qual=min_qual, min_freq=min_freq, min_bc=min_bc, device=device,
                     ign_bc_below=ign_bc_below, hbm_budget_bytes=hbm_budget_bytes, minimizer_len=minimizer_len,
                     flags=(F_KEEP_PRE_ADJ if keep_pre_adjacency else 0) | (F_KEEP_INPUTS if keep_inputs else 0) | (F_MARK_BADS if mark_bads else 0),
                     inst_per_item=inst_per_item)
        cfg.reserved[0] = passes
        self._ctx = C.c_void_p()
        _check(lib().dfk_create(C.byref(cfg), C.byref(self._ctx)))
        self.K = K

    def close(self):
        if self._ctx:
            lib().dfk_destroy(self._ctx)
            self._ctx = C.c_void_p()

    def __del__(self):
        try:
            self.close()
        except Exception:
            pass

    def count(self, packed, base_off, read_len, pq_bytes, pq_off, bc):
        packed = np.ascontiguousarray(packed, np.uint8); base_off = None if base_off is None else np.ascontiguousarray(base_off, np.uint64)
        read_len = np.ascontiguousarray(read_len, np.uint32); pq_bytes = np.ascontiguousarray(pq_bytes, np.uint8)
        pq_off = np.ascontiguousarray(pq_off, np.uint64)
        bc = None if bc is None else np.ascontiguousarray(bc, np.int32)
        _check(lib().dfk_count(self._ctx, _p(packed), _p(base_off), _p(read_len), _p(pq_bytes), _p(pq_off), _p(bc),
                               C.c_uint64(len(read_len))))

    def count_bci(self, packed, base_off, read_len, pq_bytes, pq_off, bci):
        packed = np.ascontiguousarray(packed, np.uint8); read_len = np.ascontiguousarray(read_len, np.uint32)
        base_off = None if base_off is None else np.ascontiguousarray(base_off, np.uint64)
        pq_bytes = np.ascontiguousarray(pq_bytes, np.uint8); pq_off = np.ascontiguousarray(pq_off, np.uint64)
        bci = np.ascontiguousarray(bci, np.int64)
        _check(lib().dfk_count_bci(self._ctx, _p(packed), _p(base_off), _p(read_len), _p(pq_bytes), _p(pq_off), _p(bci),
                                   C.c_uint64(len(bci)), C.c_uint64(len(read_len))))

    def count_device(self, packed, base_off, read_len, pq_bytes, pq_off, bc):
        def dp(t):
            return C.c_void_p(0 if t is None else t.data_ptr())
        for t in (packed, base_off, read_len, pq_bytes, pq_off):
            assert t.is_cuda and t.is_contiguous()
        _check(lib().dfk_count_device(self._ctx, dp(packed), C.c_uint64(packed.numel()), dp(base_off), dp(read_len),
                                      dp(pq_bytes), C.c_uint64(pq_bytes.numel()), dp(pq_off), dp(bc),
                                      C.c_uint64(read_len.numel())))

    def hint_file_range(self, array, fd, file_off=0):
        if array is None:
            _check(lib().dfk_hint_file_range(self._ctx, None, C.c_uint64(0), C.c_int(-1), C.c_uint64(0)))
        else:
            _check(lib().dfk_hint_file_range(self._ctx, C.c_void_p(array.ctypes.data), C.c_uint64(array.nbytes), C.c_int(fd), C.c_uint64(file_off)))

    def qual_hist(self, max_len):
        out = np.zeros((2, max_len, 256), np.int64)
        _check(lib().dfk_qual_hist(self._ctx, C.c_uint32(max_len), _p(out)))
        return out

    def good_lens(self):
        n = self.stats()["n_reads"]
        out = np.zeros(n, np.uint32)
        _check(lib().dfk_good_lens(self._ctx, _p(out), C.c_uint64(n)))
        return out

    def spectrum(self):
        h = C.POINTER(C.c_int64)(); n = C.c_uint64()
        _check(lib().dfk_spectrum(self._ctx, C.byref(h), C.byref(n)))
        return np.ctypeslib.as_array(h, shape=(n.value,)).copy() if n.value else np.zeros(0, np.int64)

    def spectrum_json(self):
        need = C.c_uint64()
        _check(lib().dfk_spectrum_json(self._ctx, None, C.c_uint64(0), C.byref(need)))
        buf = C.create_string_buffer(need.value + 1)
        _check(lib().dfk_spectrum_json(self._ctx, buf, C.c_uint64(need.value + 1), C.byref(need)))
        return buf.raw[: need.value].decode()

    def solid_count(self):
        n = C.c_uint64()
        _check(lib().dfk_solid_count(self._ctx, C.byref(n)))
        return n.value

    def solid(self, pre_adjacency=False):
        n = self.solid_count()
        out = np.zeros(n, dtype=ENTRY_DTYPE)
        _check(lib().dfk_solid_fetch(self._ctx, _p(out), C.c_uint64(n), C.c_int(1 if pre_adjacency else 0)))
        return out

# ... 26 lines not shown
        else:
            packed = np.ascontiguousarray(packed, np.uint8); base_off = np.ascontiguousarray(base_off, np.uint64)
            read_len = np.ascontiguousarray(read_len, np.uint32); pq_bytes = np.ascontiguousarray(pq_bytes, np.uint8)
            pq_off = np.ascontiguousarray(pq_off, np.uint64)
            _check(lib().dfk_paths_build(self._ctx, _p(packed), _p(base_off), _p(read_len), _p(pq_bytes), _p(pq_off), C.c_uint64(len(read_len))))
        return self.paths_stats()

    def paths_build_device(self, packed, base_off, read_len, pq_bytes, pq_off):
        def dp(t):
            return C.c_void_p(t.data_ptr())
        _check(lib().dfk_paths_build_device(self._ctx, dp(packed), C.c_uint64(packed.numel()), dp(base_off), dp(read_len),
                                            dp(pq_bytes), C.c_uint64(pq_bytes.numel()), dp(pq_off), C.c_uint64(read_len.numel())))
        return self.paths_stats()

    def paths_stats(self):
        a, b, c = C.c_uint64(), C.c_uint64(), C.c_uint64()
        _check(lib().dfk_paths_stats(self._ctx, C.byref(a), C.byref(b), C.byref(c)))
        return dict(n_reads=a.value, n_placed=b.value, n_path_edges=c.value)

    def paths_sink(self, path):
        _check(lib().dfk_paths_sink(self._ctx, None if path is None else path.encode()))

    def paths_write(self, path):
        _check(lib().dfk_paths_write(self._ctx, path.encode()))

    def paths_index_write(self, directory):
        _check(lib().dfk_paths_index_write(self._ctx, None if directory is None else directory.encode()))

    def dups_write(self, path):
        n = C.c_uint64()
        _check(lib().dfk_dups_write(self._ctx, None if path is None else path.encode(), C.byref(n)))
        return n.value

    def paths_index_dups_write(self, directory, path):
        n = C.c_uint64()
        _check(lib().dfk_paths_index_dups_write(self._ctx, None if directory is None else directory.encode(), None if path is None else path.encode(), C.byref(n)))
        return n.value

    def bads_sums(self):
        a = C.c_uint64()
        n = a.value if lib().dfk_paths_stats(self._ctx, C.byref(a), None, None) == 0 else 0
        out = np.zeros(n, np.uint16)
        _check(lib().dfk_bads_sums(self._ctx, _p(out), C.c_uint64(n)))
        return out

    def bads_write(self, path):
        n = C.c_uint64(); dg = (C.c_uint64 * 2)()
        _check(lib().dfk_bads_write(self._ctx, None if path is None else path.encode(), C.byref(n), dg))
        return n.value, (int(dg[0]), int(dg[1]))

    def hops_build(self, bc, one_good=False):
        bc = np.ascontiguousarray(bc, np.int32)
        _check(lib().dfk_hops_build(self._ctx, _p(bc), C.c_int(1 if one_good else 0)))
        return self.hops_stats()

    def hops_build_bci(self, bci, one_good=False):
        bci = np.ascontiguousarray(bci, np.int64)
        _check(lib().dfk_hops_build_bci(self._ctx, _p(bci), C.c_uint64(len(bci)), C.c_int(1 if one_good else 0)))
        return self.hops_stats()

    def hops_build_arrays(self, kmers, inv, to_left, to_right, n_vertices, paths, bc, sums, one_good=False, reads_per_batch=0):
        kmers, inv, to_left, to_right, bc = (np.ascontiguousarray(a, np.int32) for a in (kmers, inv, to_left, to_right, bc))
        sums = np.ascontiguousarray(sums, np.uint16)
        first = np.zeros(len(paths) + 1, np.uint64)
        first[1:] = np.cumsum([len(p) for p in paths], dtype=np.uint64)
        edges = np.ascontiguousarray([e for p in paths for e in p] or [0], np.int32)
        assert len(inv) == len(to_left) == len(to_right) == len(kmers) and len(bc) == len(sums) == len(paths)
        _check(lib().dfk_hops_build_arrays(self._ctx, C.c_uint64(len(kmers)), C.c_uint64(n_vertices), _p(kmers), _p(inv), _p(to_left), _p(to_right),
                                           C.c_uint64(len(paths)), _p(first), _p(edges), _p(bc), _p(sums), C.c_int(1 if one_good else 0),
                                           C.c_uint64(reads_per_batch)))
        return self.hops_stats()

    def hops_stats(self):
        out = (C.c_uint64 * HOPS_WORDS)()
        _check(lib().dfk_hops_stats(self._ctx, out))
        return {k: int(out[i]) for i, k in enumerate(HOPS)}

    def hops_fetch(self):
        n = C.c_uint64()
        _check(lib().dfk_hops_fetch(self._ctx, None, C.c_uint64(0), C.byref(n)))
        out = np.zeros((n.value, 2), np.int32)
        _check(lib().dfk_hops_fetch(self._ctx, _p(out), C.c_uint64(n.value), C.byref(n)))
        return out

    def hops_write(self, path):
        n = C.c_uint64(); dg = (C.c_uint64 * 2)()
        _check(lib().dfk_hops_write(self._ctx, None if path is None else path.encode(), C.byref(n), dg))
        return n.value, (int(dg[0]), int(dg[1]))

    def subset_build(self, pairs=None):
        if pairs is None:
            _check(lib().dfk_subset_build(self._ctx, None, C.c_uint64(0)))
        else:
            pairs = np.ascontiguousarray(pairs, np.int32).reshape(-1, 2)
            room = pairs if len(pairs) else np.zeros((1, 2), np.int32)
            _check(lib().dfk_subset_build(self._ctx, _p(room), C.c_uint64(len(pairs))))
        return self.subset_stats()

    def subset_build_arrays(self, inv, paths, pairs, reads_per_batch=0, directory=None):
        inv = np.ascontiguousarray(inv, np.int32)
        first = np.zeros(len(paths) + 1, np.uint64)
        first[1:] = np.cumsum([len(p) for p in paths], dtype=np.uint64)
        edges = np.ascontiguousarray([e for p in paths for e in p] or [0], np.int32)
        pr = np.ascontiguousarray(list(pairs) or [(0, 0)], np.int32).reshape(-1, 2)
        _check(lib().dfk_subset_build_arrays(self._ctx, C.c_uint64(len(inv)), _p(inv), C.c_uint64(len(paths)), _p(first), _p(edges), _p(pr),
                                             C.c_uint64(len(pairs)), C.c_uint64(reads_per_batch), None if directory is None else str(directory).encode()))
        return self.subset_stats()

    def subset_stats(self):
        out = (C.c_uint64 * SUBSET_WORDS)()
        _check(lib().dfk_subset_stats(self._ctx, out))
        return {k: int(out[i]) for i, k in enumerate(SUBSET)}

    def subset_fetch(self):
        ni, ne = C.c_uint64(), C.c_uint64()
        _check(lib().dfk_subset_fetch(self._ctx, None, C.c_uint64(0), C.byref(ni), None, C.c_uint64(0), C.byref(ne)))
        ids, eoi = np.zeros(ni.value, np.uint64), np.zeros(ne.value, np.uint64)
        _check(lib().dfk_subset_fetch(self._ctx, _p(ids), C.c_uint64(ni.value), C.byref(ni), _p(eoi), C.c_uint64(ne.value), C.byref(ne)))
        return ids, eoi

    def subset_write(self, directory):
        _check(lib().dfk_subset_write(self._ctx, None if directory is None else str(directory).encode()))

    def paths_digest(self):
        out = (C.c_uint64 * CHECK_WORDS)()
        _check(lib().dfk_paths_digest(self._ctx, out))
        return {k: int(out[i]) for i, k in enumerate(CK)}

    def paths_verify(self, packed, base_off, read_len):
        packed = np.ascontiguousarray(packed, np.uint8); base_off = np.ascontiguousarray(base_off, np.uint64)
        read_len = np.ascontiguousarray(read_len, np.uint32)
        out = (C.c_uint64 * 8)()
        _check(lib().dfk_paths_verify(self._ctx, _p(packed), _p(base_off), _p(read_len), C.c_uint64(len(read_len)), out))
        return {k: int(out[i]) for i, k in enumerate(VERIFY)}

    def paths_verify_device(self, packed, base_off, read_len):
        out = (C.c_uint64 * 8)()
        _check(lib().dfk_paths_verify_device(self._ctx, C.c_void_p(packed.data_ptr()), C.c_uint64(packed.numel()), C.c_void_p(base_off.data_ptr()),
                                             C.c_void_p(read_len.data_ptr()), C.c_uint64(read_len.numel()), out))
        return {k: int(out[i]) for i, k in enumerate(VERIFY)}

    def paths(self):
        st = self.paths_stats()
        off = np.zeros(st["n_reads"], np.int32); first = np.zeros(st["n_reads"] + 1, np.uint64)
        edges = np.zeros(max(1, st["n_path_edges"]), np.int32)
        _check(lib().dfk_paths_fetch(self._ctx, _p(off), _p(first), _p(edges), C.c_uint64(len(edges))))
        return off, first, edges[: st["n_path_edges"]]

    def stats(self):
        s = Stats()
        _check(lib().dfk_get_stats(self._ctx, C.byref(s)))
        return s.asdict()


def _mix(x):
    x = x ^ (x >> np.uint64(30)); x = x * np.uint64(0xBF58476D1CE4E5B9)
    x = x ^ (x >> np.uint64(27)); x = x * np.uint64(0x94D049BB133111EB)
    return x ^ (x >> np.uint64(31))


def digest_of(entries):
    w = np.ascontiguousarray(entries).view(np.uint64).reshape(-1, 4)
    with np.errstate(over="ignore"):
        h = _mix(w[:, 0] ^ _mix(w[:, 1] ^ _mix(w[:, 2] ^ _mix(w[:, 3] + np.uint64(0x9E3779B97F4A7C15)))))
        x = _mix(h + np.uint64(0xD1B54A32D192ED03))
        return int(h.sum(dtype=np.uint64)), int(np.bitwise_xor.reduce(x)) if len(x) else 0
```

Before: 64.73 billion.

## Build boundary k-mer set early on second stream, overlapping the last count pass

During the final count pass, the code estimates the boundary k-mer count from the parts already listed. It allocates a hash set sized to fit the free arena blocks and fills it with those parts' boundary k-mers on stream2, overlapping the last count kernel. Adjacency then inserts only the remaining parts. The set index moves from a power-of-two mask to multiply-high modulo over an arbitrary slot count, so the set can fit smaller free blocks. The risks are extra memory pressure during counting (the set is dropped if another allocation fails), a discarded set when the estimate is too low, and a slightly costlier hash-to-slot mapping.

```diff
diff --git a/include/dfk.h b/include/dfk.h
--- a/include/dfk.h
+++ b/include/dfk.h
@@ -104,6 +104,15 @@
 int dfk_write_kvec_part(dfk_ctx* ctx, const char* path, int flags, uint64_t first_entry, uint64_t total_entries);
 
 int dfk_get_stats(dfk_ctx* ctx, dfk_stats* out);
+
+#define DFK_ADJ_NOT_APPLICABLE    0u
+#define DFK_ADJ_USED              1u
+#define DFK_ADJ_DISCARDED_LOW     2u
+#define DFK_ADJ_DISCARDED_LIST    3u
+#define DFK_ADJ_NO_BLOCK          4u
+#define DFK_ADJ_DROPPED_FOR_ALLOC 5u
+#define DFK_ADJ_SWITCHED_OFF      6u
+int dfk_adj_outcome(dfk_ctx* ctx, uint32_t* outcome, uint64_t* slots);
 
 int dfk_graph_build(dfk_ctx* ctx);
 int dfk_graph_stats(dfk_ctx* ctx, uint64_t* n_canonical_edges, uint64_t* n_vertices, uint64_t* n_edges);
diff --git a/superplus_amd/csrc/dfk.hip b/superplus_amd/csrc/dfk.hip
--- a/superplus_amd/csrc/dfk.hip
+++ b/superplus_amd/csrc/dfk.hip
@@ -1,6 +1,7 @@
 #include "../../include/dfk.h"
 #include "dfk_kernels.h"
 #include "dfk_arena.h"
+#include "dfk_adj_plan.h"
 
 #include <algorithm>
 #include <chrono>
@@ -92,7 +93,12 @@
     hipDeviceProp_t prop{};
     dfk::Arena arena{dev_get, dev_give};
     uint64_t &budget = arena.budget, &held = arena.held, &peak = arena.peak, &alloc_seq = arena.alloc_seq, &first_chunk_hint = arena.first_chunk_hint;
-    int alloc(DevBuf& b, size_t bytes, const char* what, Place where = Place::High) { return arena.alloc(b, bytes, what, where) ? fail(DFK_E_NOMEM, "%s", arena.err.c_str()) : 0; }
+    int alloc(DevBuf& b, size_t bytes, const char* what, Place where = Place::High)
+    {
+        int e = arena.alloc(b, bytes, what, where);
+        if (e && (early_due || early_held)) { TRACE("no room for %s: the early boundary k-mer set goes", what); drop_early_set(dfk::ADJ_DROPPED_FOR_ALLOC); e = arena.alloc(b, bytes, what, where); }
+        return e ? fail(DFK_E_NOMEM, "%s", arena.err.c_str()) : 0;
+    }
     void release(DevBuf& b) { arena.release(b); }
     void shrink(DevBuf& b, size_t keep) { arena.shrink(b, keep); }
     void release_since(uint64_t mark, const DevBuf* keep = nullptr) { arena.release_since(mark, keep); }
@@ -129,7 +135,22 @@
     void* sh_staged[6] = {};
     uint64_t sh_b0 = 0, sh_b1 = 0, sh_q0 = 0, sh_q1 = 0, sh_staged_reads = 0;
     DevBuf adj_keys, adj_src; uint64_t adj_n = 0;
-    DevBuf set; uint64_t set_mask = 0;
+    DevBuf set; uint64_t set_slots = 0;
+    bool early_due = false, early_held = false;
+    size_t early_parts = 0;
+    uint32_t adj_outcome = dfk::ADJ_NOT_APPLICABLE; uint64_t adj_slots = 0;
+    void drop_early_set(uint32_t why)
+    {
+        if (!early_due && !early_held) return;
+        if (stream2) (void)hipStreamSynchronize(stream2);
+        release(set); set = DevBuf{}; set_slots = 0;
+        early_due = early_held = false; adj_outcome = why; adj_slots = 0;
+    }
+    void forget_early_set()
+    {
+        if (early_due || early_held) { set = DevBuf{}; set_slots = 0; adj_outcome = dfk::ADJ_NOT_APPLICABLE; adj_slots = 0; }
+        early_due = early_held = false;
+    }
     double t_upload_done = 0;
     uint32_t shard_world = 1, shard_log2_nb = 0;
     void* shard_state = nullptr;
@@ -157,6 +178,7 @@
         shard_send_pass[0] = shard_send_pass[1] = ~0u;
         have = false; sorted_ok = sorted_pre_ok = false; sorted.clear(); sorted_pre.clear(); hist.clear();
         n_solid = 0; adj_n = 0; shard_open = false;
+        early_due = early_held = false; set_slots = 0;
         if (shard_state) { shard_state_free(shard_state); shard_state = nullptr; }
         for (void*& p : sh_staged) if (p) { (void)hipFree(p); p = nullptr; }
         budget += budget_taken; budget_taken = 0;
@@ -695,6 +717,23 @@
     return 0;
 }
 
+int launch_early_set(dfk_ctx* c)
+{
+    c->early_due = false;
+    if (!c->set.p) return 0;
+    hipLaunchKernelGGL(k_fill_u64, dim3(2048), dim3(256), 0, c->stream2, (uint64_t*)c->set.p, c->set_slots * 2, ~0ull);
+    for (size_t i = 0; i < c->early_parts; ++i) {
+        const dfk_ctx::Part& pt = c->parts[i];
+        if (!pt.n_blist) continue;
+        const unsigned long long* ctl = (const unsigned long long*)((const char*)pt.buf.p + pt.blist);
+        hipLaunchKernelGGL(k_set_insert_list, dim3((unsigned)((pt.n_blist + 255) / 256)), dim3(256), 0, c->stream2, (const uint4*)pt.buf.p,
+                           (const uint32_t*)(ctl + 2), pt.n_blist, (SetSlot*)c->set.p, c->set_slots, ctl);
+    }
+    c->early_held = true;
+    HIP_TRY(hipGetLastError());
+    return 0;
+}
+
 template <int K, int NBC>
 int launch_count(dfk_ctx* c, const Partition& P, const ItemRange* d_items, uint64_t n_items, const CountRun& R,
                  std::vector<ItemRange>* overflowed, float* kernel_ms, const uint32_t* d_sub = nullptr, bool single_kmer_records = false)
@@ -718,11 +757,12 @@
                        (ItemRange*)d_ovf.p, d_sub, c->d_resident);
     HIP_TRY(hipGetLastError());
     c->resident_target += R.grid;
-    if (c->after_count_launch || c->pending_blist >= 0) {
+    if (c->after_count_launch || c->pending_blist >= 0 || c->early_due) {
         hipLaunchKernelGGL(k_gate, dim3(1), dim3(64), 0, c->stream2, (const unsigned int*)c->d_resident, c->resident_target, 200000ull, c->d_resident + 1);
     }
     if (c->after_count_launch) { std::function<int()> f; f.swap(c->after_count_launch); rc = f(); if (rc) return rc; }
     rc = launch_boundary_list(c); if (rc) return rc;
+    if (c->early_due) { rc = launch_early_set(c); if (rc) return rc; }
     *kernel_ms += tk.stop();
     CountGlobals g{};
     HIP_TRY(hipMemcpyAsync(&g, R.g, sizeof g, hipMemcpyDeviceToHost, c->stream));
@@ -1073,18 +1113,62 @@
     return rc ? rc : count_run_nbc<K>(c, P, R, barcode_words(c, have_bc));
 }
 
+static_assert(sizeof(SetSlot) == ADJ_SLOT_BYTES, "dfk_adj_plan.h sizes the set in SetSlots");
+
+int alloc_set(dfk_ctx* c, uint64_t keys)
+{
+    const std::vector<Arena::Free> blocks = c->arena.allocatable_blocks();
+    const uint64_t room = c->budget > c->held ? c->budget - c->held : 0;
+    const uint64_t slots = adj_set_slots(keys, blocks, room);
+    if (!slots) {
+        if (g_trace) Arena::trace_free(blocks);
+        return fail(DFK_E_NOMEM, "no free block of device memory holds the boundary k-mer set (%llu keys: %.2f GB at load 0.6; %.2f GB free of %.2f GB)",
+                    (unsigned long long)keys, adj_min_slots(keys) * (double)ADJ_SLOT_BYTES / 1e9, room / 1e9, c->budget / 1e9);
+    }
+    int rc = c->alloc(c->set, slots * sizeof(SetSlot), "boundary k-mer set"); if (rc) return rc;
+    c->set_slots = slots; c->adj_slots = slots;
+    return 0;
+}
+
 int build_set(dfk_ctx* c)
 {
-    uint64_t slots = 1ull << std::max<uint32_t>(10, ceil_log2(2 * c->n_boundary + 2));
-    int rc = c->alloc(c->set, slots * sizeof(SetSlot), "boundary k-mer set"); if (rc) return rc;
-    c->set_mask = slots - 1;
-    hipLaunchKernelGGL(k_fill_u64, dim3(2048), dim3(256), 0, c->stream, (uint64_t*)c->set.p, slots * 2, ~0ull);
+    int rc = alloc_set(c, c->n_boundary); if (rc) return rc;
+    hipLaunchKernelGGL(k_fill_u64, dim3(2048), dim3(256), 0, c->stream, (uint64_t*)c->set.p, c->set_slots * 2, ~0ull);
     for (const dfk_ctx::Part& pt : c->parts)
         if (pt.n)
             hipLaunchKernelGGL(k_set_insert, dim3((unsigned)((pt.n + 255) / 256)), dim3(256), 0, c->stream,
-                               (const uint4*)pt.buf.p, pt.n, (SetSlot*)c->set.p, c->set_mask);
+                               (const uint4*)pt.buf.p, pt.n, (SetSlot*)c->set.p, c->set_slots);
     HIP_TRY(hipGetLastError());
     return 0;
+}
+
+void plan_early_set(dfk_ctx* c, uint32_t sub_nb, uint32_t lo, uint64_t reserve)
+{
+    c->adj_outcome = ADJ_NOT_APPLICABLE; c->adj_slots = 0;
+    if (!c->want_blist || c->cfg.min_freq <= 1 || !c->stream2 || getenv("DFK_NO_OVERLAP") || !lo) return;
+    std::vector<uint64_t> n_blist;
+    bool listed = true;
+    for (const dfk_ctx::Part& pt : c->parts) { n_blist.push_back(pt.n_blist); listed = listed && pt.listed; }
+    const double scale = getenv("DFK_EARLY_SET_SCALE") ? atof(getenv("DFK_EARLY_SET_SCALE")) : 1.0;
+    const uint64_t est = adj_estimate_keys(n_blist, sub_nb, lo, scale);
+    if (!listed || !est) return;
+    if (getenv("DFK_NO_EARLY_SET")) { c->adj_outcome = ADJ_SWITCHED_OFF; return; }
+    const std::vector<Arena::Free> blocks = c->arena.allocatable_blocks();
+    const uint64_t free_now = c->budget > c->held ? c->budget - c->held : 0, room = free_now > reserve ? free_now - reserve : 0;
+    const uint64_t slots = adj_set_slots(est, blocks, room);
+    if (g_trace) {
+        TRACE("early set: estimate %llu keys from %zu parts (%u of %u buckets), %llu slots (%.2f GB, load %.3f), %.2f GB free (%.3f GB of it kept for the pass) in %zu blocks:",
+              (unsigned long long)est, n_blist.size(), lo, sub_nb, (unsigned long long)slots, slots * (double)ADJ_SLOT_BYTES / 1e9,
+              slots ? (double)est / (double)slots : 0.0, free_now / 1e9, reserve / 1e9, blocks.size());
+        Arena::trace_free(blocks);
+    }
+    c->adj_outcome = ADJ_NO_BLOCK;
+    if (!slots) return;
+    if (c->arena.alloc(c->set, slots * sizeof(SetSlot), "boundary k-mer set")) { c->set = DevBuf{}; return; }
+    c->set_slots = slots; c->adj_slots = slots;
+    c->early_parts = c->parts.size();
+    c->early_due = true;
+    c->adj_outcome = ADJ_USED;
 }
 
 int make_pre_view(dfk_ctx* c)
@@ -1117,28 +1201,47 @@
             HIP_TRY(hipStreamSynchronize(c->stream2));
         }
         if (listed) {
+            std::vector<unsigned long long> ctl(2 * c->parts.size(), 0);
+            for (size_t i = 0; i < c->parts.size(); ++i)
+                if (c->parts[i].blist) HIP_TRY(hipMemcpyAsync(&ctl[2 * i], (const char*)c->parts[i].buf.p + c->parts[i].blist, 16, hipMemcpyDeviceToHost, c->stream));
+            HIP_TRY(hipStreamSynchronize(c->stream));
             uint64_t total = 0;
-            for (const dfk_ctx::Part& pt : c->parts) {
+            for (size_t i = 0; i < c->parts.size(); ++i) {
+                const dfk_ctx::Part& pt = c->parts[i];
                 if (!pt.blist) continue;
-                unsigned long long ctl[2] = {0, 0};
-                HIP_TRY(hipMemcpy(ctl, (const char*)pt.buf.p + pt.blist, 16, hipMemcpyDeviceToHost));
-                if (ctl[1] || ctl[0] != pt.n_blist)
-                    return fail(DFK_E_HIP, "boundary list: %llu entries listed, the count kernels reported %llu", ctl[0], (unsigned long long)pt.n_blist);
+                if (ctl[2 * i + 1] || ctl[2 * i] != pt.n_blist) {
+                    c->drop_early_set(ADJ_DISCARDED_LIST);
+                    return fail(DFK_E_HIP, "boundary list: %llu entries listed, the count kernels reported %llu", ctl[2 * i], (unsigned long long)pt.n_blist);
+                }
                 total += pt.n_blist;
             }
             if (total != c->n_boundary) listed = false;
         }
+        if (c->early_held) {
+            if (!listed) c->drop_early_set(ADJ_DISCARDED_LIST);
+            else if (!adj_load_ok(c->n_boundary, c->set_slots)) {
+                TRACE("early set: %llu keys in %llu slots would be load %.3f: discarded", (unsigned long long)c->n_boundary, (unsigned long long)c->set_slots, (double)c->n_boundary / (double)c->set_slots);
+                c->drop_early_set(ADJ_DISCARDED_LOW);
+            }
+        }
+        const bool early = c->early_held;
+        c->early_held = false;
         if (!listed) { rc = build_set(c); if (rc) return rc; }
         else {
-            uint64_t slots = 1ull << std::max<uint32_t>(10, ceil_log2(2 * c->n_boundary + 2));
-            rc = c->alloc(c->set, slots * sizeof(SetSlot), "boundary k-mer set"); if (rc) return rc;
-            c->set_mask = slots - 1;
-            hipLaunchKernelGGL(k_fill_u64, dim3(2048), dim3(256), 0, c->stream, (uint64_t*)c->set.p, slots * 2, ~0ull);
-            for (const dfk_ctx::Part& pt : c->parts)
+            if (!early) {
+                rc = alloc_set(c, c->n_boundary); if (rc) return rc;
+                hipLaunchKernelGGL(k_fill_u64, dim3(2048), dim3(256), 0, c->stream, (uint64_t*)c->set.p, c->set_slots * 2, ~0ull);
+            }
+            for (size_t i = early ? c->early_parts : 0; i < c->parts.size(); ++i) {
+                const dfk_ctx::Part& pt = c->parts[i];
                 if (pt.n_blist)
                     hipLaunchKernelGGL(k_set_insert_list, dim3((unsigned)((pt.n_blist + 255) / 256)), dim3(256), 0, c->stream, (const uint4*)pt.buf.p,
-                                       (const uint32_t*)((const char*)pt.buf.p + pt.blist + 16), pt.n_blist, (SetSlot*)c->set.p, c->set_mask);
+                                       (const uint32_t*)((const char*)pt.buf.p + pt.blist + 16), pt.n_blist, (SetSlot*)c->set.p, c->set_slots,
+                                       (const unsigned long long*)nullptr);
+            }
             HIP_TRY(hipGetLastError());
+            TRACE("boundary k-mer set: %llu keys in %llu slots (load %.3f)%s", (unsigned long long)c->n_boundary, (unsigned long long)c->set_slots,
+                  (double)c->n_boundary / (double)c->set_slots, early ? ", filled under the last count but for the last part" : "");
         }
         DevBuf d_n; rc = c->alloc(d_n, 16, "probe counter"); if (rc) return rc;
         HIP_TRY(hipMemsetAsync(d_n.p, 0, 16, c->stream));
@@ -1148,10 +1251,10 @@
                 if (pt.n_blist)
                     hipLaunchKernelGGL(HIP_KERNEL_NAME(k_adjacency_list<K>), dim3((unsigned)std::min<uint64_t>((pt.n_blist + 255) / 256, 16384)), dim3(256), 0,
                                        c->stream, (uint4*)pt.buf.p, (const uint32_t*)((const char*)pt.buf.p + pt.blist + 16), pt.n_blist,
-                                       (const SetSlot*)c->set.p, c->set_mask, (unsigned long long*)d_n.p);
+                                       (const SetSlot*)c->set.p, c->set_slots, (unsigned long long*)d_n.p);
             } else
                 hipLaunchKernelGGL(HIP_KERNEL_NAME(k_adjacency<K>), dim3((unsigned)std::min<uint64_t>((pt.n + 255) / 256, 8192)), dim3(256), 0,
-                                   c->stream, (uint4*)pt.buf.p, pt.n, (const SetSlot*)c->set.p, c->set_mask, (unsigned long long*)d_n.p);
+                                   c->stream, (uint4*)pt.buf.p, pt.n, (const SetSlot*)c->set.p, c->set_slots, (unsigned long long*)d_n.p);
         }
         HIP_TRY(hipGetLastError());
         uint64_t np = 0;
@@ -1160,6 +1263,7 @@
         c->st.adj_probes = np;
         c->release(d_n); c->release(c->set);
     }
+    if (c->early_held) c->drop_early_set(ADJ_NOT_APPLICABLE);
     c->st.ms_adjacency = t.stop();
     TRACE("adjacency done");
     return 0;
@@ -1212,6 +1316,7 @@
     CountRun R;
     rc = count_run_begin(c, &R); if (rc) return rc;
     c->want_blist = true; c->pending_blist = -1;
+    c->adj_outcome = ADJ_NOT_APPLICABLE; c->adj_slots = 0;
     const uint32_t sub_nb = 1u << T.log2_nb;
     const uint32_t forced = (uint32_t)c->cfg.reserved[0];
     const uint32_t per_forced = forced ? std::max<uint32_t>(1, (sub_nb + forced - 1) / forced) : 0;
@@ -1264,7 +1369,9 @@
                 if (r2 && r2 != DFK_E_NOMEM) return r2;
             }
         }
+        if (!rc && nlo == sub_nb && overlap) plan_early_set(c, sub_nb, lo, cur.sj.P.n_items * sizeof(ItemRange) + 16ull * R.grid * out_chunk<K>() + 4096);
         if (!rc) rc = count_run_nbc<K>(c, cur.sj.P, R, barcode_words(c, in.bc != nullptr));
+        if (c->early_due) c->drop_early_set(ADJ_NOT_APPLICABLE);
         if (c->after_count_launch) {
             std::function<int()> f; f.swap(c->after_count_launch);
             if (!rc) { const int r3 = f(); if (r3) return r3; } else nxt.valid = false;
@@ -1272,6 +1379,7 @@
         if (rc == DFK_E_NOMEM || rc == E_SEGMENT_FULL) {
             HIP_TRY(hipStreamSynchronize(c->stream)); HIP_TRY(hipStreamSynchronize(c->stream2));
             c->release_since(cur.mark);
+            c->forget_early_set();
             R.d_wg = R.big = R.d_part = DevBuf{};
             drop_events(cur); drop_events(nxt); nxt.valid = false;
             int rc2 = count_snapshot(c, &R, true); if (rc2) return rc2;
@@ -1953,6 +2061,13 @@
     return 0;
 }
 
+int dfk_adj_outcome(dfk_ctx* c, uint32_t* outcome, uint64_t* slots)
+{
+    if (!c || !outcome || !slots) return fail(DFK_E_ARG, "null argument");
+    *outcome = c->adj_outcome; *slots = c->adj_slots;
+    return 0;
+}
+
 }
 
 #include "dfk_shard.inc"
diff --git a/superplus_amd/csrc/dfk_adj_plan.h b/superplus_amd/csrc/dfk_adj_plan.h
--- /dev/null
+++ b/superplus_amd/csrc/dfk_adj_plan.h
@@ -0,0 +1,54 @@
+#pragma once
+#include "dfk_arena.h"
+
+namespace dfk {
+
+constexpr uint64_t ADJ_SLOT_BYTES = 16;
+constexpr uint64_t ADJ_ALIGN = 256;
+constexpr uint64_t ADJ_LOAD_NUM = 3, ADJ_LOAD_DEN = 5;
+constexpr double ADJ_MARGIN = 1.05;
+
+enum AdjOutcome : uint32_t {
+    ADJ_NOT_APPLICABLE = 0,
+    ADJ_USED = 1,
+    ADJ_DISCARDED_LOW = 2,
+    ADJ_DISCARDED_LIST = 3,
+    ADJ_NO_BLOCK = 4,
+    ADJ_DROPPED_FOR_ALLOC = 5,
+    ADJ_SWITCHED_OFF = 6,
+};
+
+inline bool adj_load_ok(uint64_t keys, uint64_t slots) { return slots && (unsigned __int128)keys * ADJ_LOAD_DEN <= (unsigned __int128)slots * ADJ_LOAD_NUM; }
+
+inline uint64_t adj_min_slots(uint64_t keys) { return (uint64_t)(((unsigned __int128)keys * ADJ_LOAD_DEN + ADJ_LOAD_NUM - 1) / ADJ_LOAD_NUM) + (keys ? 0 : 1); }
+
+inline uint64_t adj_pow2_slots(uint64_t keys)
+{
+    uint32_t l = 10;
+    while (l < 63 && (1ull << l) < 2 * keys + 2) ++l;
+    return 1ull << l;
+}
+
+inline uint64_t adj_estimate_keys(const std::vector<uint64_t>& n_blist, uint32_t sub_nb, uint32_t buckets_done, double scale = 1.0)
+{
+    uint64_t sum = 0;
+    for (uint64_t n : n_blist) sum += n;
+    if (!buckets_done || !sum) return 0;
+    const double est = (double)sum * ((double)sub_nb / (double)buckets_done) * ADJ_MARGIN * scale;
+    return est >= 1.8e19 ? ~0ull : (uint64_t)est + 1;
+}
+
+inline uint64_t adj_set_slots(uint64_t keys, const std::vector<Arena::Free>& blocks, uint64_t room, size_t* block = nullptr)
+{
+    size_t at = blocks.size(); uint64_t best = 0;
+    for (size_t i = 0; i < blocks.size(); ++i) if (blocks[i].bytes > best) { best = blocks[i].bytes; at = i; }
+    if (block) *block = at;
+    const uint64_t bytes = std::min(best, room) & ~(ADJ_ALIGN - 1);
+    const uint64_t slots = std::min(bytes / ADJ_SLOT_BYTES, adj_pow2_slots(keys));
+    return adj_load_ok(keys, slots) ? slots : 0;
+}
+
+inline uint64_t adj_home(uint64_t hash, uint64_t slots) { return (uint64_t)(((unsigned __int128)hash * slots) >> 64); }
+inline uint64_t adj_next(uint64_t s, uint64_t slots) { return s + 1 == slots ? 0 : s + 1; }
+
+}
diff --git a/superplus_amd/csrc/dfk_arena.h b/superplus_amd/csrc/dfk_arena.h
--- a/superplus_amd/csrc/dfk_arena.h
+++ b/superplus_amd/csrc/dfk_arena.h
@@ -85,6 +85,14 @@
         for (const Chunk& k : chunks) for (const Free& f : k.free_list) best = std::max<uint64_t>(best, f.bytes);
         return std::min<uint64_t>(best, budget > held ? budget - held : 0);
     }
+    std::vector<Free> allocatable_blocks() const
+    {
+        std::vector<Free> all;
+        for (const Chunk& k : chunks) all.insert(all.end(), k.free_list.begin(), k.free_list.end());
+        const uint64_t grow = budget > reserved ? (budget - reserved) & ~(uint64_t)0xFFF : 0;
+        if (grow) all.push_back(Free{0, grow});
+        return all;
+    }
     void release(DevBuf& b)
     {
         if (!b.p) return;
diff --git a/superplus_amd/csrc/dfk_kernels.h b/superplus_amd/csrc/dfk_kernels.h
--- a/superplus_amd/csrc/dfk_kernels.h
+++ b/superplus_amd/csrc/dfk_kernels.h
@@ -1736,31 +1736,33 @@
     h ^= h >> 29;
     return h;
 }
-
-__global__ void __launch_bounds__(256)
-k_set_insert(const uint4* __restrict__ entries, uint64_t n, SetSlot* __restrict__ set, uint64_t mask)
+__device__ __forceinline__ uint64_t set_home(uint64_t w0, uint64_t w1, uint64_t slots) { return __umul64hi(set_hash(w0, w1), slots); }
+__device__ __forceinline__ uint64_t set_next(uint64_t s, uint64_t slots) { return s + 1 == slots ? 0 : s + 1; }
+
+__global__ void __launch_bounds__(256)
+k_set_insert(const uint4* __restrict__ entries, uint64_t n, SetSlot* __restrict__ set, uint64_t slots)
 {
     uint64_t i = (uint64_t)blockIdx.x * blockDim.x + threadIdx.x;
     if (i >= n) return;
     if (!(entries[2 * i + 1].w & 0xFFu)) return;
     uint4 a = entries[2 * i];
     uint64_t w0 = (uint64_t)a.x | ((uint64_t)a.y << 32), w1 = (uint64_t)a.z | ((uint64_t)a.w << 32);
-    uint64_t s = set_hash(w0, w1) & mask;
+    uint64_t s = set_home(w0, w1, slots);
     for (;;) {
         unsigned long long old = atomicCAS(reinterpret_cast<unsigned long long*>(&set[s].w0), ~0ull, (unsigned long long)w0);
         if (old == ~0ull) { set[s].w1 = w1; return; }
-        s = (s + 1) & mask;
-    }
-}
-
-__device__ __forceinline__ bool set_has(const SetSlot* __restrict__ set, uint64_t mask, uint64_t w0, uint64_t w1)
-{
-    uint64_t s = set_hash(w0, w1) & mask;
+        s = set_next(s, slots);
+    }
+}
+
+__device__ __forceinline__ bool set_has(const SetSlot* __restrict__ set, uint64_t slots, uint64_t w0, uint64_t w1)
+{
+    uint64_t s = set_home(w0, w1, slots);
     for (;;) {
         SetSlot v = set[s];
         if (v.w0 == ~0ull) return false;
         if (v.w0 == w0 && v.w1 == w1) return true;
-        s = (s + 1) & mask;
+        s = set_next(s, slots);
     }
 }
 
@@ -1799,17 +1801,19 @@
 }
 
 __global__ void __launch_bounds__(256)
-k_set_insert_list(const uint4* __restrict__ entries, const uint32_t* __restrict__ list, uint64_t n, SetSlot* __restrict__ set, uint64_t mask)
+k_set_insert_list(const uint4* __restrict__ entries, const uint32_t* __restrict__ list, uint64_t n, SetSlot* __restrict__ set, uint64_t slots,
+                  const unsigned long long* __restrict__ ctl)
 {
     const uint64_t t = (uint64_t)blockIdx.x * blockDim.x + threadIdx.x;
     if (t >= n) return;
+    if (ctl && (ctl[0] != n || ctl[1])) return;
     const uint4 a = entries[2 * (uint64_t)list[t]];
     const uint64_t w0 = (uint64_t)a.x | ((uint64_t)a.y << 32), w1 = (uint64_t)a.z | ((uint64_t)a.w << 32);
-    uint64_t s = set_hash(w0, w1) & mask;
-    for (uint64_t step = 0; step <= mask; ++step) {
+    uint64_t s = set_home(w0, w1, slots);
+    for (uint64_t step = 0; step < slots; ++step) {
         unsigned long long old = atomicCAS(reinterpret_cast<unsigned long long*>(&set[s].w0), ~0ull, (unsigned long long)w0);
         if (old == ~0ull) { set[s].w1 = w1; return; }
-        s = (s + 1) & mask;
+        s = set_next(s, slots);
     }
 }
 
@@ -1826,7 +1830,7 @@
 }
 
 template <int K>
-__device__ __forceinline__ uint32_t adjacency_entry(uint4* __restrict__ entries, uint64_t i, const SetSlot* __restrict__ set, uint64_t mask)
+__device__ __forceinline__ uint32_t adjacency_entry(uint4* __restrict__ entries, uint64_t i, const SetSlot* __restrict__ set, uint64_t slots)
 {
     const u128 m = KTraits<K>::mask();
     uint4 b = entries[2 * i + 1];
@@ -1846,7 +1850,7 @@
         }
         uint64_t w0, w1; canon_words<K>(v, &w0, &w1);
         ++probes;
-        if (!set_has(set, mask, w0, w1)) ctx &= ~(1u << bit);
+        if (!set_has(set, slots, w0, w1)) ctx &= ~(1u << bit);
     }
     b.y = (b.y & 0xFFFFFFu) | (ctx << 24);
     b.w = 0;
@@ -1866,23 +1870,23 @@
 
 template <int K>
 __global__ void __launch_bounds__(256)
-k_adjacency(uint4* __restrict__ entries, uint64_t n, const SetSlot* __restrict__ set, uint64_t mask,
+k_adjacency(uint4* __restrict__ entries, uint64_t n, const SetSlot* __restrict__ set, uint64_t slots,
             unsigned long long* __restrict__ n_probes)
 {
     unsigned long long probes = 0;
     for (uint64_t i = (uint64_t)blockIdx.x * blockDim.x + threadIdx.x; i < n; i += (uint64_t)gridDim.x * blockDim.x)
-        probes += adjacency_entry<K>(entries, i, set, mask);
+        probes += adjacency_entry<K>(entries, i, set, slots);
     add_probes(probes, n_probes);
 }
 
 template <int K>
 __global__ void __launch_bounds__(256)
-k_adjacency_list(uint4* __restrict__ entries, const uint32_t* __restrict__ list, uint64_t n, const SetSlot* __restrict__ set, uint64_t mask,
+k_adjacency_list(uint4* __restrict__ entries, const uint32_t* __restrict__ list, uint64_t n, const SetSlot* __restrict__ set, uint64_t slots,
                  unsigned long long* __restrict__ n_probes)
 {
     unsigned long long probes = 0;
     for (uint64_t t = (uint64_t)blockIdx.x * blockDim.x + threadIdx.x; t < n; t += (uint64_t)gridDim.x * blockDim.x)
-        probes += adjacency_entry<K>(entries, (uint64_t)list[t], set, mask);
+        probes += adjacency_entry<K>(entries, (uint64_t)list[t], set, slots);
     add_probes(probes, n_probes);
 }
 
@@ -2106,13 +2110,13 @@
 }
 
 __global__ void __launch_bounds__(256)
-k_adj_answer(const SetSlot* __restrict__ keys, uint64_t n, const SetSlot* __restrict__ set, uint64_t mask,
+k_adj_answer(const SetSlot* __restrict__ keys, uint64_t n, const SetSlot* __restrict__ set, uint64_t slots,
              uint8_t* __restrict__ present)
 {
     const uint64_t i = (uint64_t)blockIdx.x * blockDim.x + threadIdx.x;
     if (i >= n) return;
     SetSlot k = keys[i];
-    present[i] = set_has(set, mask, k.w0, k.w1) ? 1 : 0;
+    present[i] = set_has(set, slots, k.w0, k.w1) ? 1 : 0;
 }
 
 __global__ void __launch_bounds__(256)
diff --git a/superplus_amd/csrc/dfk_shard.inc b/superplus_amd/csrc/dfk_shard.inc
--- a/superplus_amd/csrc/dfk_shard.inc
+++ b/superplus_amd/csrc/dfk_shard.inc
@@ -500,7 +500,7 @@
     HIP_TRY(hipSetDevice(c->device));
     CallClock clock(c, &c->st.ms_adjacency);
     hipLaunchKernelGGL(k_adj_answer, dim3((unsigned)((n_keys + 255) / 256)), dim3(256), 0, c->stream, (const SetSlot*)d_keys, n_keys,
-                       (const SetSlot*)c->set.p, c->set_mask, (uint8_t*)d_present);
+                       (const SetSlot*)c->set.p, c->set_slots, (uint8_t*)d_present);
     HIP_TRY(hipGetLastError());
     HIP_TRY(hipStreamSynchronize(c->stream));
     return 0;
diff --git a/superplus_amd/dfk.py b/superplus_amd/dfk.py
--- a/superplus_amd/dfk.py
+++ b/superplus_amd/dfk.py
@@ -17,7 +17,7 @@
 EXPORTS = [
     "dfk_create", "dfk_destroy", "dfk_last_error", "dfk_abi_version", "dfk_count", "dfk_count_bci", "dfk_count_device",
     "dfk_hint_file_range", "dfk_qual_hist", "dfk_paths_sink", "dfk_good_lens", "dfk_spectrum", "dfk_spectrum_json", "dfk_solid_count", "dfk_solid_fetch", "dfk_solid_fetch_unsorted", "dfk_solid_digest",
-    "dfk_write_kvec", "dfk_write_kvec_part", "dfk_get_stats", "dfk_shard_begin", "dfk_shard_begin_host", "dfk_shard_plan", "dfk_shard_partition", "dfk_shard_partition_begin", "dfk_shard_partition_end", "dfk_shard_recv_buffer", "dfk_shard_count", "dfk_shard_adj_queries",
+    "dfk_write_kvec", "dfk_write_kvec_part", "dfk_get_stats", "dfk_adj_outcome", "dfk_shard_begin", "dfk_shard_begin_host", "dfk_shard_plan", "dfk_shard_partition", "dfk_shard_partition_begin", "dfk_shard_partition_end", "dfk_shard_recv_buffer", "dfk_shard_count", "dfk_shard_adj_queries",
     "dfk_shard_adj_answer", "dfk_shard_adj_apply", "dfk_graph_build", "dfk_graph_stats", "dfk_graph_write",
     "dfk_shard_dict_share", "dfk_shard_dict_adopt", "dfk_shard_dict_whole",
     "dfk_paths_build", "dfk_paths_build_device", "dfk_paths_stats", "dfk_paths_write", "dfk_paths_fetch", "dfk_paths_index_write", "dfk_dups_write", "dfk_paths_index_dups_write",
@@ -38,6 +38,8 @@
 SUBSET = ["eoi", "ids", "path_entries", "index_entries", "ranges", "one_read_only", "us", "us_sweep", "us_gather", "us_index",
           "ids_sum", "ids_xor", "eoi_sum", "eoi_xor"]
 SUBSET_FILES = ("a.sub.ids", "a.sub.eoi", "a.sub.paths", "a.sub.paths.inv")
+ADJ_OUTCOMES = ["not applicable", "used", "discarded: guess too low", "discarded: list problem", "no block", "dropped for an allocation",
+                "switched off"]
 VERIFY = ["placed", "broken", "hits", "consistent", "no_anchor", "all_consistent", "dict_bad", "outside"]
 
 
@@ -370,6 +372,11 @@
         _check(lib().dfk_get_stats(self._ctx, C.byref(s)))
         return s.asdict()
 
+    def adj_outcome(self):
+        code, slots = C.c_uint32(), C.c_uint64()
+        _check(lib().dfk_adj_outcome(self._ctx, C.byref(code), C.byref(slots)))
+        return ADJ_OUTCOMES[code.value], int(slots.value)
+
 
 def _mix(x):
     x = x ^ (x >> np.uint64(30)); x = x * np.uint64(0xBF58476D1CE4E5B9)
```

Result: faster. 65.74 billion (median of 6 runs) (+1.6%).
